# 666DZY666/micronet

Measured on NVIDIA H100. Metric: qat_step_images_per_sec, higher is better.
Workload: dtype f32 (bf16 tensor-core products of exact integer levels / exact bf16 pieces, fp32 accumulate)

## Files before the change

harness/step_profile.py:

```python
import argparse
import json
import os
import re
import subprocess
import sys

sys.path.insert(0, os.path.dirname(os.path.dirname(os.path.abspath(__file__))))

import torch

from harness import train as H

HEADLINE = "nin_gc_wbwtab_w3a2"


def card():
    try:
        return subprocess.run(["nvidia-smi", "--query-gpu=name,power.limit,clocks.max.sm", "--format=csv,noheader"],
                              capture_output=True, text=True, timeout=30).stdout.strip().splitlines()[0]
    except (OSError, subprocess.SubprocessError, IndexError) as e:
        return f"unknown ({type(e).__name__})"


def producer_bytes(rec, terms_dy):
    n, xb, pooled, plane_only, pk_conv = rec["n"], rec["xb"], rec["pool2"], rec["plane_only"], rec["pk_conv"]
    bits = n / 8
    out = {"channel_stats_kernel": n * xb}
    if pooled:
        out["bn_sign_pool_fwd_kernel"] = n * xb + n + n / 4 + bits
        out["bn_sign_pool_bwd_reduce_kernel"] = n * xb + n + n / 4 + bits
        if pk_conv:
            out["bn_sign_pool_bwd_pack_kernel"] = n * xb + n + n / 4 + bits + 2 * n * terms_dy
        else:
            out["bn_sign_pool_bwd_apply_kernel"] = n * xb + n + n / 4 + bits + 4 * n
    else:
        out["bn_sign_packed_fwd_kernel"] = n * xb + 2 * n + bits + (0 if plane_only else 4 * n)
        out["bn_sign_bwd_reduce_kernel"] = n * xb + 4 * n + bits
        if pk_conv:
            out["bn_sign_bwd_pack_kernel"] = n * xb + 4 * n + bits + 2 * n * terms_dy
        else:
            out["bn_sign_bwd_apply_kernel"] = n * xb + 4 * n + bits + 4 * n
    return out


def base_name(kernel):
    head = kernel.split("(")[0]
    head = re.sub(r"<.*$", "", head)
    return head.split("::")[-1].split(" ")[-1]


def main():
    ap = argparse.ArgumentParser()
    ap.add_argument("--out", required=True)
    ap.add_argument("--steps", type=int, default=5)
    ap.add_argument("--warmup", type=int, default=5)
    ap.add_argument("--batch", type=int, default=256)
    args = ap.parse_args()
    if not torch.cuda.is_available():
        raise SystemExit("step_profile: no CUDA device")
    os.makedirs(args.out, exist_ok=True)
    from micronet_b200 import _lib as L
    from micronet_b200.fused import BatchNormBinarize2d
    w = H.WORKLOADS[HEADLINE]
    dev = torch.device("cuda:0")
    model = H.prepare_engine(H.build_float_model(w["model"]), w["scheme"], **w["prepare"], **w.get("engine_extra", {})).to(dev)
    stepper = H.QatStepper(model, lr=0.01, wd=w["wd"], flat=True, graph=False)
    batches = [H.synthetic_batch(args.batch, w["hw"], seed=100 + i, device=dev) for i in range(2)]
    for i in range(args.warmup):
        stepper.step(*batches[i % 2])
    torch.cuda.synchronize()

    calls = []

    def hook(mod, inp):
        x = inp[0]
        calls.append({"n": x.numel(), "xb": 2 if getattr(x, "_mnb_codes", None) is not None else 4,
                      "pool2": bool(mod.pool2), "plane_only": bool(mod.plane_only) and not mod.pool2,
                      "pk_conv": getattr(x, "_mnb_pk_conv", None) is not None})

    handles = [m.register_forward_pre_hook(hook) for m in model.modules() if isinstance(m, BatchNormBinarize2d)]
    acts = [torch.profiler.ProfilerActivity.CPU, torch.profiler.ProfilerActivity.CUDA]
    with torch.profiler.profile(activities=acts) as prof:
        for i in range(args.steps):
            stepper.step(*batches[i % 2])
        torch.cuda.synchronize()
    for h in handles:
        h.remove()

    terms_dy = min(L.PK_TERMS, L.PK_TERMS_BWD)
    want = {}
    for rec in calls:
        for k, b in producer_bytes(rec, terms_dy).items():
            want[k] = want.get(k, 0.0) + b
    kern = {}
    for e in prof.events():
        if e.device_type != torch.autograd.DeviceType.CUDA:
            continue
        d = kern.setdefault(e.name, {"launches": 0, "us": 0.0})
        d["launches"] += 1
        d["us"] += e.device_time
    rows, total_us = [], sum(d["us"] for d in kern.values()) / args.steps
    for name, d in kern.items():
        row = {"kernel": name, "base": base_name(name), "launches_per_step": d["launches"] / args.steps,
               "us_per_step": d["us"] / args.steps}
        rows.append(row)
    by_base = {}
    for r in rows:
        by_base.setdefault(r["base"], []).append(r)
    for base, rs in by_base.items():
        if base not in want:
            continue
        launches = sum(r["launches_per_step"] for r in rs)
        bytes_step = want[base] / args.steps
        us = sum(r["us_per_step"] for r in rs)
        for r in rs:
            r["bytes_per_launch"] = bytes_step / launches
        rs[0]["group_bytes_per_step"] = bytes_step
        rs[0]["group_GBps"] = bytes_step / (us * 1e-6) / 1e9
    rows.sort(key=lambda r: -r["us_per_step"])
    res = {"card": card(), "workload": HEADLINE, "batch": args.batch, "steps": args.steps,
           "device_us_per_step": total_us, "kernels": rows}
    with open(os.path.join(args.out, "step_profile.json"), "w") as f:
        json.dump(res, f, indent=1)
    lines = [f"card: {res['card']}", f"{HEADLINE}, batch {args.batch}, eager step, {args.steps} profiled steps; "
             f"device time per step {total_us / 1e3:.3f} ms (sum of kernel times)", "",
             f"{'us/step':>9} {'share':>6} {'launch':>6} {'MB/launch':>9} {'GB/s':>7}  kernel"]
    for r in rows:
        mb = f"{r['bytes_per_launch'] / 1e6:9.1f}" if "bytes_per_launch" in r else " " * 9
        gbs = f"{r['group_GBps']:7.0f}" if "group_GBps" in r else " " * 7
        lines.append(f"{r['us_per_step']:9.1f} {r['us_per_step'] / total_us:6.1%} {r['launches_per_step']:6.1f} {mb} {gbs}  "
                     f"{r['kernel'][:110]}")
    txt = "\n".join(lines)
    with open(os.path.join(args.out, "step_profile.txt"), "w") as f:
        f.write(txt + "\n")
    print(txt)


if __name__ == "__main__":
    main()
```

include/micronet_b200.h:

```cpp
#ifndef MICRONET_B200_H
#define MICRONET_B200_H

#include <stdint.h>

#ifdef __cplusplus
extern "C" {
#endif

typedef void* mnb_stream_t;

#define MNB_E_ARG (-1)
#define MNB_E_UNSUPPORTED (-2)

int mnb_version(void);
const char* mnb_last_error(void);
int64_t mnb_launch_count(void);

typedef struct {
  int32_t batch, in_c, in_h, in_w;
  int32_t out_c, ker_h, ker_w;
  int32_t stride_h, stride_w, pad_h, pad_w, dil_h, dil_w, groups;
} mnb_conv_shape;

#define MNB_ACT_DOREFA 1
// ... 94 lines not shown
                          void* scratch, const int32_t* run_if_nonzero, mnb_stream_t stream);

int mnb_bn_batch_stats(const float* x, int32_t batch, int32_t channels, int32_t hw, double eps, double momentum,
                       float* running_mean, float* running_var, int64_t* num_batches_tracked, float* mean_invstd,
                       void* scratch, mnb_stream_t stream);
int mnb_bn_sign_fwd(const float* x, int32_t batch, int32_t channels, int32_t hw, const float* mean, const float* invstd,
                    const float* gamma, const float* beta, int32_t out_shuffle_groups, float* y, uint32_t* pass_bits,
                    mnb_stream_t stream);
int mnb_bn_sign_bwd(const float* g, const uint32_t* pass_bits, const float* x, int32_t batch, int32_t channels, int32_t hw,
                    const float* mean, const float* invstd, const float* gamma, int32_t training,
                    int32_t out_shuffle_groups, float* dx, float* dgamma, float* dbeta, float* dx_channel_sum,
                    void* scratch, mnb_stream_t stream);

int mnb_bn_sign_pool_fwd(const float* x, int32_t batch, int32_t channels, int32_t H, int32_t W, const float* mean,
                         const float* invstd, const float* gamma, const float* beta, int32_t out_shuffle_groups, float* y,
                         uint32_t* pass_bits, uint8_t* argmax, mnb_stream_t stream);
int mnb_bn_sign_pool_bwd(const float* g, const uint32_t* pass_bits, const uint8_t* argmax, const float* x, int32_t batch,
                         int32_t channels, int32_t H, int32_t W, const float* mean, const float* invstd, const float* gamma,
                         int32_t training, int32_t out_shuffle_groups, float* dx, float* dgamma, float* dbeta,
                         float* dx_channel_sum, void* scratch, mnb_stream_t stream);

int mnb_maxpool2d_fwd(const float* x, int32_t batch, int32_t channels, int32_t H, int32_t W, int32_t kernel, int32_t stride,
                      int32_t pad, int32_t out_shuffle_groups, float* y, uint8_t* argmax, mnb_stream_t stream);
int mnb_maxpool2d_bwd(const float* g, const uint8_t* argmax, int32_t batch, int32_t channels, int32_t H, int32_t W,
                      int32_t kernel, int32_t stride, int32_t pad, int32_t out_shuffle_groups, float* dx,
                      mnb_stream_t stream);

int mnb_bn_sign_fwd_packed(const float* x, int32_t batch, int32_t channels, int32_t hw, const float* mean,
                           const float* invstd, const float* gamma, const float* beta, int32_t out_shuffle_groups, float* y,
                           uint32_t* pass_bits, void* x_packed, mnb_stream_t stream);

int mnb_fconv2d_fwd_tc(const mnb_conv_shape* s, const float* x, const float* w, const float* bias, float* y,
                       int32_t* err_flag, mnb_stream_t stream);
int64_t mnb_fconv2d_wgrad_tc_scratch_bytes(const mnb_conv_shape* s);
int mnb_fconv2d_wgrad_tc(const mnb_conv_shape* s, const float* dy, const float* x, float* dw, void* scratch,
                         int32_t* err_flag, mnb_stream_t stream);

int64_t mnb_pk_act_bytes(int32_t batch, int32_t channels, int32_t h, int32_t w, int32_t terms);
int mnb_pk_pack_act(const float* x, int32_t batch, int32_t channels, int32_t h, int32_t w, const mnb_act_qparams* qp,
                    int32_t terms, const float* ch_scale, int32_t phase_split, void* out_pk, uint8_t* bits8,
                    mnb_stream_t stream);
int mnb_bn_relu_quant_pack_fwd(const float* x, int32_t batch, int32_t channels, int32_t hw, const float* mean,
                               const float* invstd, const float* gamma, const float* beta, const mnb_act_qparams* qp,
                               int32_t out_shuffle_groups, void* x_packed, uint32_t* pass_bits, mnb_stream_t stream);
int mnb_bn_sign_bwd_pack(const float* g, const uint32_t* pass_bits, const float* x, int32_t batch, int32_t channels, int32_t hw,
                         const float* mean, const float* invstd, const float* gamma, const float* dgamma, const float* dbeta,
                         int32_t out_shuffle_groups, const float* ch_scale, int32_t terms, float* dx, void* dy_packed,
                         mnb_stream_t stream);
int mnb_bn_sign_pool_bwd_pack(const float* g, const uint32_t* pass_bits, const uint8_t* argmax, const float* x, int32_t batch,
                              int32_t channels, int32_t H, int32_t W, const float* mean, const float* invstd,
                              const float* gamma, const float* dgamma, const float* dbeta, int32_t out_shuffle_groups,
                              const float* ch_scale, int32_t terms, void* dy_packed, mnb_stream_t stream);
int mnb_pk_conv_codes(const mnb_conv_shape* s, const void* a_pk, int32_t terms_a, const void* w_img, int32_t terms_w,
                      const float* n_scale, const float* a_scale, float a_scale_const, const float* bias, int32_t level_bound,
                      int16_t* codes, float* dec, int32_t* err_flag, mnb_stream_t stream);
int mnb_codes_decode(const int16_t* codes, const float* dec, int32_t batch, int32_t channels, int32_t hw, float* x,
                     mnb_stream_t stream);
int mnb_bn_batch_stats_codes(const int16_t* codes, const float* dec, int32_t batch, int32_t channels, int32_t hw, double eps,
                             double momentum, float* running_mean, float* running_var, int64_t* num_batches_tracked,
                             float* mean_invstd, void* scratch, mnb_stream_t stream);
int mnb_bn_sign_fwd_packed_codes(const int16_t* codes, const float* dec, int32_t batch, int32_t channels, int32_t hw,
                                 const float* mean, const float* invstd, const float* gamma, const float* beta,
                                 int32_t out_shuffle_groups, float* y, uint32_t* pass_bits, void* x_packed, mnb_stream_t stream);
int mnb_bn_sign_bwd_codes(const float* g, const uint32_t* pass_bits, const int16_t* codes, const float* dec, int32_t batch,
                          int32_t channels, int32_t hw, const float* mean, const float* invstd, const float* gamma,
                          int32_t training, int32_t out_shuffle_groups, float* dx, float* dgamma, float* dbeta,
                          float* dx_channel_sum, void* scratch, mnb_stream_t stream);
int mnb_bn_sign_pool_fwd_codes(const int16_t* codes, const float* dec, int32_t batch, int32_t channels, int32_t H, int32_t W,
                               const float* mean, const float* invstd, const float* gamma, const float* beta,
                               int32_t out_shuffle_groups, float* y, uint32_t* pass_bits, uint8_t* argmax, mnb_stream_t stream);
int mnb_bn_sign_pool_bwd_codes(const float* g, const uint32_t* pass_bits, const uint8_t* argmax, const int16_t* codes,
                               const float* dec, int32_t batch, int32_t channels, int32_t H, int32_t W, const float* mean,
                               const float* invstd, const float* gamma, int32_t training, int32_t out_shuffle_groups, float* dx,
                               float* dgamma, float* dbeta, float* dx_channel_sum, void* scratch, mnb_stream_t stream);
int mnb_bn_sign_bwd_pack_codes(const float* g, const uint32_t* pass_bits, const int16_t* codes, const float* dec, int32_t batch,
                               int32_t channels, int32_t hw, const float* mean, const float* invstd, const float* gamma,
                               const float* dgamma, const float* dbeta, int32_t out_shuffle_groups, const float* ch_scale,
                               int32_t terms, float* dx, void* dy_packed, mnb_stream_t stream);
int mnb_bn_sign_pool_bwd_pack_codes(const float* g, const uint32_t* pass_bits, const uint8_t* argmax, const int16_t* codes,
                                    const float* dec, int32_t batch, int32_t channels, int32_t H, int32_t W, const float* mean,
                                    const float* invstd, const float* gamma, const float* dgamma, const float* dbeta,
                                    int32_t out_shuffle_groups, const float* ch_scale, int32_t terms, void* dy_packed,
                                    mnb_stream_t stream);
int mnb_pk_pack_act_relu(const float* x, int32_t batch, int32_t channels, int32_t h, int32_t w, const mnb_act_qparams* qp,
                         int32_t terms, const float* ch_scale, int32_t phase_split, int32_t relu, void* out_pk,
                         uint8_t* bits8, mnb_stream_t stream);
int mnb_pk_conv_plan(const mnb_conv_shape* s, int32_t mode, int32_t terms_a, int32_t terms_w, int32_t* out16);
int mnb_pk_conv_plan_ex(const mnb_conv_shape* s, int32_t mode, int32_t terms_a, int32_t terms_w, int32_t* out, int32_t n);
int mnb_pk_wgrad_plan(const mnb_conv_shape* s, int32_t terms_dy, int32_t terms_x, int32_t* out, int32_t n);
int64_t mnb_pk_wimage_bytes(const mnb_conv_shape* s, int32_t mode, int32_t terms_a, int32_t terms_w);
int mnb_pk_pack_weight(const mnb_conv_shape* s, int32_t mode, int32_t terms_a, int32_t terms_w, const int16_t* w_int,
                       const float* w_f32, const float* kzero, void* w_img, mnb_stream_t stream);
int mnb_pk_conv(const mnb_conv_shape* s, int32_t mode, const void* a_pk, int32_t terms_a, const void* w_img, int32_t terms_w,
                const float* n_scale, const float* a_scale, float a_scale_const, const float* bias, const uint8_t* bits8,
                float gain, float* out, int32_t* err_flag, mnb_stream_t stream);
typedef struct mnb_pk_post {
  const mnb_act_qparams* q;
  int32_t relu;
  int32_t phase_split;
  void* out_pk;
  const float* bn_mean;
  const float* bn_invstd;
  const float* bn_gamma;
  const float* bn_beta;
  int32_t shuffle_groups;
} mnb_pk_post;
int mnb_pk_conv_post(const mnb_conv_shape* s, const void* a_pk, int32_t terms_a, const void* w_img, int32_t terms_w,
                     const float* n_scale, const float* a_scale, float a_scale_const, const float* bias, float* out,
                     const mnb_pk_post* post, int32_t* err_flag, mnb_stream_t stream);
int mnb_quant_add_pack_fwd(const float* a, const float* b, int32_t batch, int32_t channels, int32_t h, int32_t w,
                           const mnb_act_qparams* qp, int32_t relu, float* out, const mnb_pk_post* post, mnb_stream_t stream);
int64_t mnb_pk_i8_act_bytes(int32_t batch, int32_t channels, int32_t h, int32_t w);
int mnb_pk_i8_pack_act(const float* x, int32_t batch, int32_t channels, int32_t h, int32_t w, const mnb_act_qparams* qp,
                       int32_t phase_split, int32_t relu, void* out_pk, mnb_stream_t stream);
int mnb_pk_i8_conv_plan(const mnb_conv_shape* s, int32_t* out, int32_t n);
int64_t mnb_pk_i8_wimage_bytes(const mnb_conv_shape* s);
int mnb_pk_i8_pack_weight(const mnb_conv_shape* s, const int16_t* w_int, void* w_img, mnb_stream_t stream);
int mnb_pk_i8_conv(const mnb_conv_shape* s, const void* a_pk, const void* w_img, const float* n_scale, const float* a_scale,
                   float a_scale_const, const float* bias, float* out, const mnb_pk_post* post, int32_t* err_flag,
                   mnb_stream_t stream);
int mnb_quant_add_pack_i8_fwd(const float* a, const float* b, int32_t batch, int32_t channels, int32_t h, int32_t w,
                              const mnb_act_qparams* qp, int32_t relu, float* out, const mnb_pk_post* post, mnb_stream_t stream);
int mnb_bn_relu_quant_pack_i8_fwd(const float* x, int32_t batch, int32_t channels, int32_t hw, const float* mean,
                                  const float* invstd, const float* gamma, const float* beta, const mnb_act_qparams* qp,
                                  int32_t out_shuffle_groups, void* x_packed, mnb_stream_t stream);
int mnb_pk_plane_maxpool(const void* in_pk, int32_t batch, int32_t channels, int32_t h, int32_t w, int32_t k, int32_t s, int32_t p,
                         int32_t int8, void* out_pk, mnb_stream_t stream);
int64_t mnb_pk_wgrad_scratch_bytes(const mnb_conv_shape* s, int32_t terms_dy, int32_t terms_x);
int mnb_pk_wgrad(const mnb_conv_shape* s, const void* dy_pk, int32_t terms_dy, const void* x_pk, int32_t terms_x,
                 const float* a_scale, const float* kdiv, float* dw, void* scratch, int32_t* err_flag, mnb_stream_t stream);
int mnb_pk_wgrad_taps_plan(const mnb_conv_shape* s, int32_t terms_dy, int32_t terms_x, int32_t* out, int32_t n);
int mnb_pk_wgrad_taps(const mnb_conv_shape* s, const void* dy_pk, int32_t terms_dy, const void* x_pk, int32_t terms_x,
                      const float* a_scale, const float* kdiv, float* dw, void* scratch, int32_t* err_flag, mnb_stream_t stream);

int mnb_xnor_supported(const mnb_conv_shape* s);
int64_t mnb_xnor_act_bytes(int32_t batch, int32_t channels, int32_t h, int32_t w, int32_t groups);
int mnb_xnor_pack_act(const float* x, int32_t batch, int32_t channels, int32_t h, int32_t w, int32_t groups, void* out_bits,
                      mnb_stream_t stream);
int64_t mnb_xnor_wimage_bytes(const mnb_conv_shape* s);
int mnb_xnor_pack_weight(const mnb_conv_shape* s, const int16_t* w_int, void* w_img, mnb_stream_t stream);
int mnb_xnor_conv_fwd(const mnb_conv_shape* s, const void* a_bits, const void* w_img, const float* alpha, const float* bias,
                      float* y, mnb_stream_t stream);
#define MNB_XNOR_BITS 0
#define MNB_XNOR_PM1_BF16 1
typedef struct mnb_xnor_post {
  int32_t format;
  int32_t out_groups;
  int32_t shuffle_groups;
  int32_t pool2;
  const float* bn_mean;
  const float* bn_invstd;
  const float* bn_gamma;
  const float* bn_beta;
} mnb_xnor_post;
int64_t mnb_xnor_post_bytes(const mnb_conv_shape* s, const mnb_xnor_post* post);
int mnb_xnor_conv_post(const mnb_conv_shape* s, const void* a_bits, const void* w_img, const float* alpha, const float* bias,
                       const mnb_xnor_post* post, void* out, mnb_stream_t stream);
int mnb_xnor_pack_act_post(const float* x, int32_t batch, int32_t channels, int32_t h, int32_t w, const mnb_xnor_post* post,
                           void* out_bits, mnb_stream_t stream);

int mnb_adam_step(float* params, const float* grads, float* exp_avg, float* exp_avg_sq, int64_t n, float lr,
                  float beta1, float beta2, float eps, float weight_decay, int32_t step, mnb_stream_t stream);

void mnb_set_tc_profile_buffer(void* dev_int64x16);

int mnb_selftest_umma(const float* A, const float* B, float* D, int32_t N, int32_t K, int32_t int8,
// ... 12 lines not shown
```

micronet_b200/_lib.py:

```python
from __future__ import annotations

import ctypes as C
import os

import torch

_HERE = os.path.dirname(os.path.abspath(__file__))
LIB_PATH = os.path.join(_HERE, "lib", "libmicronet_b200.so")

ACT_DOREFA, ACT_IAO, ACT_SIGN = 1, 2, 3


class ConvShape(C.Structure):
    _fields_ = [(n, C.c_int32) for n in (
        "batch", "in_c", "in_h", "in_w", "out_c", "ker_h", "ker_w", "stride_h", "stride_w",
        "pad_h", "pad_w", "dil_h", "dil_w", "groups")]


class ActQParams(C.Structure):
    _fields_ = [("mode", C.c_int32), ("bits", C.c_int32), ("qmin", C.c_int32), ("qmax", C.c_int32),
                ("q_type", C.c_int32), ("scale", C.c_void_p), ("zero_point", C.c_void_p),
                ("obs_min", C.c_void_p), ("obs_max", C.c_void_p)]


# ... 6 lines not shown
XNOR_BITS, XNOR_PM1_BF16 = 0, 1


class XnorPost(C.Structure):
    _fields_ = [("format", C.c_int32), ("out_groups", C.c_int32), ("shuffle_groups", C.c_int32), ("pool2", C.c_int32),
                ("bn_mean", C.c_void_p), ("bn_invstd", C.c_void_p), ("bn_gamma", C.c_void_p), ("bn_beta", C.c_void_p)]


class ConvOperands(C.Structure):
    _fields_ = [("a_codes", C.c_void_p), ("a_f32", C.c_void_p), ("a_offset", C.c_int32),
                ("a_offset_zp", C.c_void_p), ("a_scale", C.c_void_p), ("w_int", C.c_void_p),
                ("w_scale", C.c_void_p), ("w_f32", C.c_void_p), ("bias", C.c_void_p)]


_P, _I, _L, _D = C.c_void_p, C.c_int32, C.c_int64, C.c_double
_SHAPE, _ACTQ, _OPS = C.POINTER(ConvShape), C.POINTER(ActQParams), C.POINTER(ConvOperands)

PROTOTYPES = {
    "mnb_version": (C.c_int, []),
    "mnb_last_error": (C.c_char_p, []),
    "mnb_launch_count": (_L, []),
    "mnb_act_quant_fwd": (C.c_int, [_P, _L, _ACTQ, _P, _P, _P, _P]),
    "mnb_act_quant_bwd": (C.c_int, [_P, _P, _L, _ACTQ, _P, _P]),
    "mnb_bn_fold_fwd": (C.c_int, [_P, _I, _I, _P, _P, _P, _P, _P, _D, _P, _P, _P]),
    "mnb_bn_fold_bwd": (C.c_int, [_P, _P, _P, _I, _I, _P, _P, _P, _P, _D, _P, _P, _P]),
    "mnb_bn_fold_running": (C.c_int, [_P, _P, _P, _P, _I, _D, _I, _P]),
    "mnb_quant_add_fwd": (C.c_int, [_P, _P, _L, _ACTQ, _P, _P, _P, _I, _P]),
    "mnb_quant_add_bwd": (C.c_int, [_P, _P, _P, _L, _ACTQ, _P, _P, _P]),
    "mnb_observe_scratch_bytes": (_L, [_L, _I]),
    "mnb_iao_observe": (C.c_int, [_P, _L, _I, _I, _I, _D, _D, _P, _P, _I, _I, _I, _I, _P, _P, _P, _P]),
    "mnb_iao_update_qparams": (C.c_int, [_P, _P, _I, _I, _I, _I, _P, _P, _P]),
    "mnb_dorefa_weight_fwd": (C.c_int, [_P, _L, _I, _I, _P, _P, _P, _P, _P, _P]),
    "mnb_dorefa_weight_bwd": (C.c_int, [_P, _P, _L, _I, _P, _P, _P]),
    "mnb_wb_weight_fwd": (C.c_int, [_P, _I, _I, _I, _I, _P, _P, _P, _P, _P]),
    "mnb_wb_weight_bwd": (C.c_int, [_P, _P, _P, _I, _I, _I, _I, _P, _P]),
    "mnb_iao_weight_fwd": (C.c_int, [_P, _L, _I, _I, _P, _P, _P, _P, _I, _I, _I, _P, _P, _P, _P, _P]),
    "mnb_iao_weight_bwd": (C.c_int, [_P, _P, _P, _L, _I, _I, _P, _P]),
    "mnb_conv2d_fwd": (C.c_int, [_SHAPE, _OPS, _P, _P]),
    "mnb_conv2d_dgrad": (C.c_int, [_SHAPE, _P, _P, _P, _ACTQ, _P, _P]),
    "mnb_wgrad_scratch_bytes": (_L, [_SHAPE]),
    "mnb_conv2d_wgrad": (C.c_int, [_SHAPE, _P, _OPS, _P, _P, _P]),
    "mnb_channel_stats": (C.c_int, [_P, _I, _I, _I, _I, _P, _P, _P]),
    "mnb_channel_stats_bwd": (C.c_int, [_P, _P, _P, _P, _I, _I, _I, _P, _P]),
    "mnb_fq_conv2d_fwd_tc": (C.c_int, [_SHAPE, _P, _ACTQ, _P, _P, _P, _P, _P, _P, _P, _P, _P]),
    "mnb_conv2d_dgrad_tc": (C.c_int, [_SHAPE, _P, _P, _P, _P, _ACTQ, _P, _P, _P, _P]),
    "mnb_wgrad_tc_scratch_bytes": (_L, [_SHAPE]),
    "mnb_conv2d_wgrad_tc": (C.c_int, [_SHAPE, _P, _P, _ACTQ, _P, _P, _P, _P, _P]),
    "mnb_conv2d_wgrad_cond": (C.c_int, [_SHAPE, _P, _OPS, _P, _P, _P, _P]),
    "mnb_bn_batch_stats": (C.c_int, [_P, _I, _I, _I, _D, _D, _P, _P, _P, _P, _P, _P]),
    "mnb_bn_sign_fwd": (C.c_int, [_P, _I, _I, _I, _P, _P, _P, _P, _I, _P, _P, _P]),
    "mnb_bn_sign_bwd": (C.c_int, [_P, _P, _P, _I, _I, _I, _P, _P, _P, _I, _I, _P, _P, _P, _P, _P, _P]),
    "mnb_bn_sign_pool_fwd": (C.c_int, [_P, _I, _I, _I, _I, _P, _P, _P, _P, _I, _P, _P, _P, _P]),
    "mnb_bn_sign_pool_bwd": (C.c_int, [_P, _P, _P, _P, _I, _I, _I, _I, _P, _P, _P, _I, _I, _P, _P, _P, _P, _P, _P]),
    "mnb_bn_sign_fwd_packed": (C.c_int, [_P, _I, _I, _I, _P, _P, _P, _P, _I, _P, _P, _P, _P]),
    "mnb_fconv2d_fwd_tc": (C.c_int, [_SHAPE, _P, _P, _P, _P, _P, _P]),
    "mnb_fconv2d_wgrad_tc_scratch_bytes": (_L, [_SHAPE]),
    "mnb_fconv2d_wgrad_tc": (C.c_int, [_SHAPE, _P, _P, _P, _P, _P, _P]),
    "mnb_maxpool2d_fwd": (C.c_int, [_P, _I, _I, _I, _I, _I, _I, _I, _I, _P, _P, _P]),
    "mnb_maxpool2d_bwd": (C.c_int, [_P, _P, _I, _I, _I, _I, _I, _I, _I, _I, _P, _P]),
    "mnb_adam_step": (C.c_int, [_P, _P, _P, _P, _L, C.c_float, C.c_float, C.c_float, C.c_float, C.c_float, _I, _P]),
    "mnb_pk_act_bytes": (_L, [_I, _I, _I, _I, _I]),
    "mnb_pk_pack_act": (C.c_int, [_P, _I, _I, _I, _I, _ACTQ, _I, _P, _I, _P, _P, _P]),
    "mnb_bn_relu_quant_pack_fwd": (C.c_int, [_P, _I, _I, _I, _P, _P, _P, _P, _ACTQ, _I, _P, _P, _P]),
    "mnb_pk_pack_act_relu": (C.c_int, [_P, _I, _I, _I, _I, _ACTQ, _I, _P, _I, _I, _P, _P, _P]),
    "mnb_pk_conv_plan": (C.c_int, [_SHAPE, _I, _I, _I, _P]),
    "mnb_pk_conv_plan_ex": (C.c_int, [_SHAPE, _I, _I, _I, _P, _I]),
    "mnb_pk_wgrad_plan": (C.c_int, [_SHAPE, _I, _I, _P, _I]),
    "mnb_pk_wimage_bytes": (_L, [_SHAPE, _I, _I, _I]),
    "mnb_pk_pack_weight": (C.c_int, [_SHAPE, _I, _I, _I, _P, _P, _P, _P, _P]),
    "mnb_pk_conv": (C.c_int, [_SHAPE, _I, _P, _I, _P, _I, _P, _P, C.c_float, _P, _P, C.c_float, _P, _P, _P]),
    "mnb_bn_sign_bwd_pack": (C.c_int, [_P, _P, _P, _I, _I, _I, _P, _P, _P, _P, _P, _I, _P, _I, _P, _P, _P]),
    "mnb_bn_sign_pool_bwd_pack": (C.c_int, [_P, _P, _P, _P, _I, _I, _I, _I, _P, _P, _P, _P, _P, _I, _P, _I, _P, _P]),
    "mnb_pk_conv_post": (C.c_int, [_SHAPE, _P, _I, _P, _I, _P, _P, C.c_float, _P, _P, C.POINTER(PkPost), _P, _P]),
    "mnb_pk_conv_codes": (C.c_int, [_SHAPE, _P, _I, _P, _I, _P, _P, C.c_float, _P, _I, _P, _P, _P, _P]),
    "mnb_codes_decode": (C.c_int, [_P, _P, _I, _I, _I, _P, _P]),
    "mnb_bn_batch_stats_codes": (C.c_int, [_P, _P, _I, _I, _I, _D, _D, _P, _P, _P, _P, _P, _P]),
    "mnb_bn_sign_fwd_packed_codes": (C.c_int, [_P, _P, _I, _I, _I, _P, _P, _P, _P, _I, _P, _P, _P, _P]),
    "mnb_bn_sign_bwd_codes": (C.c_int, [_P, _P, _P, _P, _I, _I, _I, _P, _P, _P, _I, _I, _P, _P, _P, _P, _P, _P]),
    "mnb_bn_sign_pool_fwd_codes": (C.c_int, [_P, _P, _I, _I, _I, _I, _P, _P, _P, _P, _I, _P, _P, _P, _P]),
    "mnb_bn_sign_pool_bwd_codes": (C.c_int, [_P, _P, _P, _P, _P, _I, _I, _I, _I, _P, _P, _P, _I, _I, _P, _P, _P, _P, _P, _P]),
    "mnb_bn_sign_bwd_pack_codes": (C.c_int, [_P, _P, _P, _P, _I, _I, _I, _P, _P, _P, _P, _P, _I, _P, _I, _P, _P, _P]),
    "mnb_bn_sign_pool_bwd_pack_codes": (C.c_int, [_P, _P, _P, _P, _P, _I, _I, _I, _I, _P, _P, _P, _P, _P, _I, _P, _I, _P,
                                                  _P]),
    "mnb_quant_add_pack_fwd": (C.c_int, [_P, _P, _I, _I, _I, _I, _ACTQ, _I, _P, C.POINTER(PkPost), _P]),
    "mnb_pk_i8_act_bytes": (_L, [_I, _I, _I, _I]),
    "mnb_pk_i8_pack_act": (C.c_int, [_P, _I, _I, _I, _I, _ACTQ, _I, _I, _P, _P]),
    "mnb_pk_i8_conv_plan": (C.c_int, [_SHAPE, _P, _I]),
    "mnb_pk_i8_wimage_bytes": (_L, [_SHAPE]),
    "mnb_pk_i8_pack_weight": (C.c_int, [_SHAPE, _P, _P, _P]),
    "mnb_pk_i8_conv": (C.c_int, [_SHAPE, _P, _P, _P, _P, C.c_float, _P, _P, C.POINTER(PkPost), _P, _P]),
    "mnb_quant_add_pack_i8_fwd": (C.c_int, [_P, _P, _I, _I, _I, _I, _ACTQ, _I, _P, C.POINTER(PkPost), _P]),
    "mnb_bn_relu_quant_pack_i8_fwd": (C.c_int, [_P, _I, _I, _I, _P, _P, _P, _P, _ACTQ, _I, _P, _P]),
    "mnb_pk_plane_maxpool": (C.c_int, [_P, _I, _I, _I, _I, _I, _I, _I, _I, _P, _P]),
    "mnb_pk_wgrad_scratch_bytes": (_L, [_SHAPE, _I, _I]),
    "mnb_pk_wgrad": (C.c_int, [_SHAPE, _P, _I, _P, _I, _P, _P, _P, _P, _P, _P]),
    "mnb_pk_wgrad_taps_plan": (C.c_int, [_SHAPE, _I, _I, _P, _I]),
    "mnb_pk_wgrad_taps": (C.c_int, [_SHAPE, _P, _I, _P, _I, _P, _P, _P, _P, _P, _P]),
    "mnb_xnor_supported": (C.c_int, [_SHAPE]),
    "mnb_xnor_act_bytes": (_L, [_I, _I, _I, _I, _I]),
    "mnb_xnor_pack_act": (C.c_int, [_P, _I, _I, _I, _I, _I, _P, _P]),
    "mnb_xnor_wimage_bytes": (_L, [_SHAPE]),
    "mnb_xnor_pack_weight": (C.c_int, [_SHAPE, _P, _P, _P]),
    "mnb_xnor_conv_fwd": (C.c_int, [_SHAPE, _P, _P, _P, _P, _P, _P]),
    "mnb_xnor_post_bytes": (_L, [_SHAPE, C.POINTER(XnorPost)]),
    "mnb_xnor_conv_post": (C.c_int, [_SHAPE, _P, _P, _P, _P, C.POINTER(XnorPost), _P, _P]),
    "mnb_xnor_pack_act_post": (C.c_int, [_P, _I, _I, _I, _I, C.POINTER(XnorPost), _P, _P]),
    "mnb_set_tc_profile_buffer": (None, [_P]),
    "mnb_selftest_mma_rate": (C.c_int, [_I, _I, _I, _I, _I, _P, _P, _P]),
    "mnb_selftest_umma": (C.c_int, [_P, _P, _P, _I, _I, _I, _P, _P]),
    "mnb_selftest_tma3d": (C.c_int, [_P, C.POINTER(C.c_int64), C.POINTER(C.c_int32), C.POINTER(C.c_int32), _P, _P, _P]),
}

_lib = None


def load():
    global _lib
    if _lib is not None:
        return _lib
    if not os.path.exists(LIB_PATH):
        raise RuntimeError(
            f"micronet_b200: {LIB_PATH} is missing - build it with `python -m micronet_b200.build` "
            "(there is no CPU / PyTorch fallback for the fake-quant hot path)")
    lib = C.CDLL(LIB_PATH)
    for name, (res, args) in PROTOTYPES.items():
        fn = getattr(lib, name)
        fn.restype, fn.argtypes = res, args
    _lib = lib
    return lib


def check(rc: int, what: str):
    if rc != 0:
        msg = load().mnb_last_error().decode(errors="replace")
        kind = ValueError if rc < 0 else RuntimeError
        raise kind(f"micronet_b200.{what} failed (code {rc}): {msg}")


def ptr(t):
    return None if t is None else t.data_ptr()


def stream():
    return torch.cuda.current_stream().cuda_stream


def require_cuda(*tensors):
    for t in tensors:
        if t is not None and not t.is_cuda:
            raise RuntimeError(
                "micronet_b200: the fake-quant engine runs on CUDA (sm_90a) tensors only; "
                "got a CPU tensor - there is deliberately no CPU fallback")


def require_f32(*tensors):
    for t in tensors:
        if t is not None and t.dtype != torch.float32:
            raise TypeError(f"micronet_b200: fp32 tensors only (the reference's QAT modules are fp32), got {t.dtype}")


def launch_count() -> int:
    return int(load().mnb_launch_count())


_errflags = {}

# ... 42 lines not shown
```

micronet_b200/csrc/mnb_common.cuh:

```cuda
#pragma once
#include <cuda_runtime.h>
#include <float.h>
#include <stdint.h>

#include "../../include/micronet_b200.h"

int mnb_fail(int code, const char* fmt, ...);
void mnb_count_launches(int n);

#define MNB_REQUIRE(cond, ...)                            \
  do {                                                    \
    if (!(cond)) return mnb_fail(MNB_E_ARG, __VA_ARGS__); \
  } while (0)

#define MNB_LAUNCHED(nlaunch)                                                        \
  do {                                                                               \
    mnb_count_launches(nlaunch);                                                     \
    cudaError_t e__ = cudaGetLastError();                                            \
    if (e__ != cudaSuccess) return mnb_fail((int)e__, "%s:%d launch failed: %s", __FILE__, __LINE__, \
                                            cudaGetErrorString(e__));                \
  } while (0)

static inline int mnb_ceil_div(int64_t a, int64_t b) { return (int)((a + b - 1) / b); }
constexpr int MNB_NUM_SMS = 132;


__device__ __forceinline__ float mnb_round_half_away(float v) {
  float r = floorf(__fadd_rn(fabsf(v), 0.5f));
  return v > 0.f ? r : (v < 0.f ? -r : 0.f);
}
__device__ __forceinline__ float mnb_sign0(float v) { return v > 0.f ? 1.f : (v < 0.f ? -1.f : 0.f); }

__device__ __forceinline__ uint32_t mnb_f2ord(float f) {
  uint32_t u = __float_as_uint(f);
  return (u & 0x80000000u) ? ~u : (u | 0x80000000u);
}
__device__ __forceinline__ float mnb_ord2f(uint32_t u) {
  return __uint_as_float((u & 0x80000000u) ? (u & 0x7fffffffu) : ~u);
}

template <typename T, typename Op>
__device__ __forceinline__ T mnb_warp_reduce(T v, Op op) {
#pragma unroll
  for (int o = 16; o > 0; o >>= 1) v = op(v, __shfl_xor_sync(0xffffffffu, v, o));
  return v;
}
template <typename T, typename Op>
__device__ __forceinline__ T mnb_block_reduce(T v, Op op, T identity, T* smem) {
  const int lane = threadIdx.x & 31, wid = threadIdx.x >> 5;
  v = mnb_warp_reduce(v, op);
  __syncthreads();
  if (lane == 0) smem[wid] = v;
  __syncthreads();
  const int nw = (blockDim.x + 31) >> 5;
  T r = (lane < nw) ? smem[lane] : identity;
  r = mnb_warp_reduce(r, op);
  return r;
}
struct MnbMin { template <typename T> __device__ T operator()(T a, T b) const { return a < b ? a : b; } };
struct MnbMax { template <typename T> __device__ T operator()(T a, T b) const { return a > b ? a : b; } };
struct MnbSum { template <typename T> __device__ T operator()(T a, T b) const { return a + b; } };

__device__ __forceinline__ float bn_bwd_centre(float g, float db, float xhat, float dg) {
  return fmaf(-xhat, dg, __fsub_rn(g, db));
}

struct XDec { float s, b; };
template <typename XT> struct XVec;
template <> struct XVec<float> { typedef float t1; typedef float2 t2; typedef float4 t4; };
template <> struct XVec<int16_t> { typedef short t1; typedef short2 t2; typedef short4 t4; };

template <typename XT>
__device__ __forceinline__ XDec x_dec(const float* dec, int channels, int c) {
  if constexpr (sizeof(XT) == 4) return XDec{1.f, 0.f};
  else return XDec{__ldg(dec + c), __ldg(dec + channels + c)};
}
template <typename XT>
__device__ __forceinline__ float x_val(XT q, XDec d) {
  if constexpr (sizeof(XT) == 4) return q;
  else return fmaf((float)q, d.s, d.b);
}
template <int VEC, typename XT>
__device__ __forceinline__ void x_load(const XT* p, XDec d, float (&v)[VEC]) {
  if constexpr (VEC == 1) {
    v[0] = x_val<XT>(__ldg(reinterpret_cast<const typename XVec<XT>::t1*>(p)), d);
  } else if constexpr (VEC == 2) {
    const typename XVec<XT>::t2 t = __ldg(reinterpret_cast<const typename XVec<XT>::t2*>(p));
    v[0] = x_val<XT>(t.x, d); v[1] = x_val<XT>(t.y, d);
  } else {
    static_assert(VEC == 4, "x_load: 1, 2 or 4 elements");
    const typename XVec<XT>::t4 t = __ldg(reinterpret_cast<const typename XVec<XT>::t4*>(p));
    v[0] = x_val<XT>(t.x, d); v[1] = x_val<XT>(t.y, d); v[2] = x_val<XT>(t.z, d); v[3] = x_val<XT>(t.w, d);
  }
}
template <typename XT>
__device__ __forceinline__ float4 x_load4(const XT* p, XDec d) {
  float v[4];
  x_load<4>(p, d, v);
  return make_float4(v[0], v[1], v[2], v[3]);
}

struct MnbActQ {
  int mode, qmin, qmax;
  float s, zp, lo, hi;
  float rinv;
};

__device__ __forceinline__ MnbActQ mnb_load_actq(const mnb_act_qparams& p) {
  MnbActQ q;
  q.mode = p.mode; q.qmin = p.qmin; q.qmax = p.qmax;
  q.s = 1.f; q.zp = 0.f; q.lo = 0.f; q.hi = 0.f; q.rinv = 1.f;
  if (p.mode == MNB_ACT_DOREFA) {
    q.s = (float)(1.0 / (double)((1 << p.bits) - 1));
  } else if (p.mode == MNB_ACT_IAO) {
    q.s = __ldg(p.scale);
    q.zp = __ldg(p.zero_point);
    float a = __fsub_rn(__fdiv_rn(__ldg(p.obs_min), q.s), q.zp);
    float b = __fsub_rn(__fdiv_rn(__ldg(p.obs_max), q.s), q.zp);
    if (p.q_type == 0) { q.hi = fmaxf(fabsf(a), fabsf(b)); q.lo = -q.hi; }
    else { q.lo = a; q.hi = b; }
  }
  q.rinv = __fdiv_rn(1.f, q.s);
  return q;
}

__device__ __forceinline__ int mnb_act_quantize_one(const MnbActQ& q, float x, bool& pass, float& xq) {
  if (q.mode == MNB_ACT_DOREFA) {
    float t = __fmul_rn(x, 0.1f);
    pass = (t >= 0.f) && (t <= 1.f);
    float c = fminf(fmaxf(t, 0.f), 1.f);
    float r = floorf(__fadd_rn(__fdiv_rn(c, q.s), 0.5f));
    xq = __fmul_rn(r, q.s);
    return (int)r;
  } else if (q.mode == MNB_ACT_IAO) {
    float v = __fsub_rn(__fdiv_rn(x, q.s), q.zp);
    float r = mnb_round_half_away(v);
    float c = fminf(fmaxf(r, (float)q.qmin), (float)q.qmax);
    pass = !(v > q.hi) && !(v < q.lo) && (r >= (float)q.qmin) && (r <= (float)q.qmax);
    xq = __fmul_rn(__fadd_rn(c, q.zp), q.s);
    return (int)c - q.qmin;
  } else {
    bool pos = !(x < 0.f);
    pass = !(x >= 1.0f) && !(x <= -1.0f);
    xq = pos ? 1.f : -1.f;
    return pos ? 2 : 0;
  }
}

__device__ __forceinline__ int mnb_act_code_certified(const MnbActQ& q, float x, bool& pass) {
  if (q.mode == MNB_ACT_DOREFA) {
    const float t = __fmul_rn(x, 0.1f);
    pass = (t >= 0.f) && (t <= 1.f);
    const float c = fminf(fmaxf(t, 0.f), 1.f);
    const float pa = c * q.rinv;
    const float f = pa + 0.5f;
    float r = floorf(f);
    const float d = f - r, delta = 4e-7f * (pa + 1.f);
    if (d < delta || d > 1.f - delta) r = floorf(__fadd_rn(__fdiv_rn(c, q.s), 0.5f));
    return (int)r;
  } else if (q.mode == MNB_ACT_IAO) {
    const float xa = x * q.rinv;
    float v = xa - q.zp;
    const float av = fabsf(v);
// ... 115 lines not shown
```

micronet_b200/csrc/mnb_conv_packed.cu:

```cuda
#include <cuda_bf16.h>

#include <algorithm>

#include "mnb_common.cuh"

namespace tcpacked {

template <int VEC> struct VecT;
template <> struct VecT<1> { typedef float type; };
template <> struct VecT<2> { typedef float2 type; };
template <> struct VecT<4> { typedef float4 type; };

template <int VEC>
__device__ __forceinline__ void store_vec(float* p, const float (&v)[VEC]) {
  typedef typename VecT<VEC>::type T;
  T t;
  float* f = reinterpret_cast<float*>(&t);
#pragma unroll
  for (int i = 0; i < VEC; ++i) f[i] = v[i];
  *reinterpret_cast<T*>(p) = t;
}

template <int VEC, typename XT>
__global__ void __launch_bounds__(256) bn_sign_packed_fwd_kernel(const XT* __restrict__ x, const float* __restrict__ dec,
// ... 11 lines not shown
    const int64_t t = w / chunks;
    const int oc8 = (int)(t % c8n), b = (int)(t / c8n);
    const int pos = (ch * 32 + lane) * VEC;
    float v[8][VEC];
    int cc[8];
#pragma unroll
    for (int j = 0; j < 8; ++j) {
      const int oc = oc8 * 8 + j;
      cc[j] = sg > 1 ? (oc % sg) * cpg + oc / sg : oc;
      x_load<VEC>(x + ((int64_t)b * channels + cc[j]) * hw + pos, x_dec<XT>(dec, channels, cc[j]), v[j]);
    }
    uint32_t h[VEC][8];
#pragma unroll
    for (int j = 0; j < 8; ++j) {
      const int c = cc[j];
      const float mu = __ldg(mean + c), k = __ldg(gamma + c) * __ldg(invstd + c), be = __ldg(beta + c);
      uint32_t pass = 0;
      float yv[VEC];
#pragma unroll
      for (int i = 0; i < VEC; ++i) {
        const float bn = fmaf(v[j][i] - mu, k, be);
        const bool neg = bn < 0.f;
        yv[i] = neg ? -1.f : 1.f;
        h[i][j] = neg ? 0xBF80u : 0x3F80u;
        pass |= (fabsf(bn) < 1.f ? 1u : 0u) << i;
      }
      if (y) store_vec<VEC>(y + ((int64_t)b * channels + oc8 * 8 + j) * hw + pos, yv);
      uint32_t word = pass << (VEC * (lane % LPW));
#pragma unroll
      for (int o = 1; o < LPW; o <<= 1) word |= __shfl_xor_sync(0xffffffffu, word, o);
      if (lane % LPW == 0) bits[(((int64_t)b * channels + c) * hw + pos) >> 5] = word;
    }
    uint4* dst = xp + ((int64_t)b * c8n + oc8) * hw + pos;
#pragma unroll
    for (int i = 0; i < VEC; ++i)
      dst[i] = make_uint4(h[i][0] | (h[i][1] << 16), h[i][2] | (h[i][3] << 16), h[i][4] | (h[i][5] << 16), h[i][6] | (h[i][7] << 16));
  }
}

}

template <typename XT>
static int bn_sign_fwd_packed(const XT* x, const float* dec, int32_t batch, int32_t channels, int32_t hw, const float* mean,
                              const float* invstd, const float* gamma, const float* beta, int32_t out_shuffle_groups, float* y,
                              uint32_t* pass_bits, void* x_packed, mnb_stream_t stream) {
  MNB_REQUIRE(x && mean && invstd && gamma && beta && pass_bits && x_packed, "NULL bn_sign_fwd_packed pointer");
  MNB_REQUIRE(batch > 0 && channels > 0 && hw > 0, "bad bn_sign_fwd_packed shape");
  MNB_REQUIRE(out_shuffle_groups >= 1 && channels % out_shuffle_groups == 0, "shuffle groups %d do not divide %d channels",
              out_shuffle_groups, channels);
  if (channels % 8 || hw % 32 || (reinterpret_cast<uintptr_t>(x_packed) & 15))
    return mnb_fail(MNB_E_UNSUPPORTED, "packed producer needs channels %% 8 == 0, H*W %% 32 == 0, 16-byte aligned output");
  constexpr uintptr_t xa4 = 4 * sizeof(XT) - 1, xa2 = 2 * sizeof(XT) - 1;
  const int vec = (hw % 128 == 0 && (reinterpret_cast<uintptr_t>(x) & xa4) == 0 && (!y || (reinterpret_cast<uintptr_t>(y) & 15) == 0)) ? 4
                  : ((hw % 64 == 0 && (reinterpret_cast<uintptr_t>(x) & xa2) == 0 && (!y || (reinterpret_cast<uintptr_t>(y) & 7) == 0)) ? 2 : 1);
  const int64_t warps = (int64_t)batch * (channels / 8) * (hw / (32 * vec));
  int blocks = (int)std::min<int64_t>(mnb_ceil_div(warps, 8), MNB_NUM_SMS * 8);
  uint4* xp = reinterpret_cast<uint4*>(x_packed);
  cudaStream_t st = (cudaStream_t)stream;
  if (vec == 4)
    tcpacked::bn_sign_packed_fwd_kernel<4, XT><<<blocks, 256, 0, st>>>(x, dec, batch, channels, hw, out_shuffle_groups, mean, invstd, gamma, beta, y, pass_bits, xp);
  else if (vec == 2)
    tcpacked::bn_sign_packed_fwd_kernel<2, XT><<<blocks, 256, 0, st>>>(x, dec, batch, channels, hw, out_shuffle_groups, mean, invstd, gamma, beta, y, pass_bits, xp);
  else
    tcpacked::bn_sign_packed_fwd_kernel<1, XT><<<blocks, 256, 0, st>>>(x, dec, batch, channels, hw, out_shuffle_groups, mean, invstd, gamma, beta, y, pass_bits, xp);
  MNB_LAUNCHED(1);
  return 0;
}

extern "C" int mnb_bn_sign_fwd_packed(const float* x, int32_t batch, int32_t channels, int32_t hw, const float* mean,
                                      const float* invstd, const float* gamma, const float* beta, int32_t out_shuffle_groups,
                                      float* y, uint32_t* pass_bits, void* x_packed, mnb_stream_t stream) {
  return bn_sign_fwd_packed<float>(x, nullptr, batch, channels, hw, mean, invstd, gamma, beta, out_shuffle_groups, y, pass_bits,
                                   x_packed, stream);
}

extern "C" int mnb_bn_sign_fwd_packed_codes(const int16_t* codes, const float* dec, int32_t batch, int32_t channels, int32_t hw,
                                            const float* mean, const float* invstd, const float* gamma, const float* beta,
                                            int32_t out_shuffle_groups, float* y, uint32_t* pass_bits, void* x_packed,
                                            mnb_stream_t stream) {
  MNB_REQUIRE(dec, "NULL decode pair");
  return bn_sign_fwd_packed<int16_t>(codes, dec, batch, channels, hw, mean, invstd, gamma, beta, out_shuffle_groups, y, pass_bits,
                                     x_packed, stream);
}
```

micronet_b200/csrc/mnb_fused.cu:

```cuda
#include <algorithm>

#include "mnb_common.cuh"

static inline cudaStream_t S(mnb_stream_t s) { return (cudaStream_t)s; }
constexpr int FUSED_SPLITS = 32;

__device__ __forceinline__ uint32_t shuffled_channel(uint32_t c, uint32_t sg, uint32_t cpg) {
  return sg > 1 ? (c % cpg) * sg + c / cpg : c;
}

__global__ void __launch_bounds__(256) bn_sign_fwd_v4_kernel(const float4* __restrict__ x, uint32_t n4, uint32_t channels,
                                                             uint32_t hw4, uint32_t sg, const float* __restrict__ mean,
                                                             const float* __restrict__ invstd, const float* __restrict__ gamma,
                                                             const float* __restrict__ beta, float4* __restrict__ y,
                                                             uint32_t* __restrict__ bits) {
  const uint32_t lane = threadIdx.x & 31;
  const uint32_t stride = gridDim.x * blockDim.x;
  const uint32_t n4_up = (n4 + 31u) & ~31u;
  const uint32_t cpg = channels / sg;
  for (uint32_t i = blockIdx.x * blockDim.x + threadIdx.x; i < n4_up; i += stride) {
    uint32_t nib = 0;
    if (i < n4) {
      const uint32_t plane = i / hw4, off = i - plane * hw4;
      const uint32_t b = plane / channels, c = plane - b * channels;
// ... 196 lines not shown

template <typename XT = float>
static bool planes_vectorizable(int64_t n, int hw, const void* a, const void* b, const void* c, const XT* x = nullptr) {
  return (hw & 3) == 0 && n < (1ll << 31) &&
         (((uintptr_t)a | (uintptr_t)b | (uintptr_t)c) & 15) == 0 && ((uintptr_t)x & (4 * sizeof(XT) - 1)) == 0;
}
static int plane_splits(int batch, int64_t per, int channels) {
  const int64_t want = (2 * 8 * MNB_NUM_SMS + channels - 1) / channels;
  return (int)std::max<int64_t>(1, std::min<int64_t>(std::min<int64_t>(std::min<int64_t>(FUSED_SPLITS, batch), per / 2048), want));
}

extern "C" int mnb_bn_sign_fwd(const float* x, int32_t batch, int32_t channels, int32_t hw, const float* mean,
                               const float* invstd, const float* gamma, const float* beta, int32_t out_shuffle_groups,
                               float* y, uint32_t* pass_bits, mnb_stream_t stream) {
  MNB_REQUIRE(x && mean && invstd && gamma && beta && y && pass_bits, "NULL bn_sign_fwd pointer");
  MNB_REQUIRE(batch > 0 && channels > 0 && hw > 0, "bad bn_sign_fwd shape");
  MNB_REQUIRE(out_shuffle_groups >= 1 && channels % out_shuffle_groups == 0, "shuffle groups %d do not divide %d channels",
              out_shuffle_groups, channels);
  const int64_t n = (int64_t)batch * channels * hw;
  int blocks = (int)std::min<int64_t>(mnb_ceil_div(n, 256 * 4), MNB_NUM_SMS * 8);
  if (planes_vectorizable(n, hw, x, y, nullptr))
    bn_sign_fwd_v4_kernel<<<blocks, 256, 0, S(stream)>>>(reinterpret_cast<const float4*>(x), (uint32_t)(n / 4),
                                                         (uint32_t)channels, (uint32_t)(hw / 4), (uint32_t)out_shuffle_groups,
                                                         mean, invstd, gamma, beta, reinterpret_cast<float4*>(y), pass_bits);
  else
    bn_sign_fwd_kernel<<<blocks, 256, 0, S(stream)>>>(x, n, channels, hw, out_shuffle_groups, mean, invstd, gamma, beta, y,
                                                      pass_bits);
  MNB_LAUNCHED(1);
  return 0;
}

template <typename XT>
static int bn_sign_bwd(const float* g, const uint32_t* pass_bits, const XT* x, const float* dec, int32_t batch, int32_t channels,
                       int32_t hw, const float* mean, const float* invstd, const float* gamma, int32_t training,
                       int32_t out_shuffle_groups, float* dx, float* dgamma, float* dbeta, float* dx_channel_sum, void* scratch,
                       mnb_stream_t stream) {
  MNB_REQUIRE(g && pass_bits && x && mean && invstd && gamma && dx && dgamma && dbeta && scratch, "NULL bn_sign_bwd pointer");
  MNB_REQUIRE(batch > 0 && channels > 0 && channels <= 8192 && hw > 0, "bad bn_sign_bwd shape");
  MNB_REQUIRE(out_shuffle_groups >= 1 && channels % out_shuffle_groups == 0, "shuffle groups %d do not divide %d channels",
              out_shuffle_groups, channels);
  const int64_t n = (int64_t)batch * channels * hw;
  const int64_t per = (int64_t)batch * hw;
  const int splits = plane_splits(batch, per, channels);
  uint32_t* counters = reinterpret_cast<uint32_t*>(reinterpret_cast<char*>(scratch) + 16384);
  double* partial = reinterpret_cast<double*>(reinterpret_cast<char*>(scratch) + 49152);
  const dim3 grid(channels, splits);
  const float inv_count = 1.f / (float)per;
  if (planes_vectorizable(n, hw, g, dx, nullptr, x)) {
    bn_sign_bwd_reduce_kernel<true, XT><<<grid, 256, 0, S(stream)>>>(g, pass_bits, x, dec, batch, channels, hw, out_shuffle_groups,
                                                                     mean, invstd, dgamma, dbeta, counters, partial);
    if (training == 2) { MNB_LAUNCHED(1); return 0; }
    bn_sign_bwd_apply_kernel<true, XT><<<grid, 256, 0, S(stream)>>>(g, pass_bits, x, dec, batch, channels, hw, out_shuffle_groups,
                                                                    inv_count, mean, invstd, gamma, dgamma, dbeta, training, dx,
                                                                    dx_channel_sum, counters, partial);
  } else {
    bn_sign_bwd_reduce_kernel<false, XT><<<grid, 256, 0, S(stream)>>>(g, pass_bits, x, dec, batch, channels, hw, out_shuffle_groups,
                                                                      mean, invstd, dgamma, dbeta, counters, partial);
    if (training == 2) { MNB_LAUNCHED(1); return 0; }
    bn_sign_bwd_apply_kernel<false, XT><<<grid, 256, 0, S(stream)>>>(g, pass_bits, x, dec, batch, channels, hw, out_shuffle_groups,
                                                                     inv_count, mean, invstd, gamma, dgamma, dbeta, training, dx,
                                                                     dx_channel_sum, counters, partial);
  }
  MNB_LAUNCHED(2);
  return 0;
}

extern "C" int mnb_bn_sign_bwd(const float* g, const uint32_t* pass_bits, const float* x, int32_t batch, int32_t channels,
                               int32_t hw, const float* mean, const float* invstd, const float* gamma, int32_t training,
                               int32_t out_shuffle_groups, float* dx, float* dgamma, float* dbeta, float* dx_channel_sum,
                               void* scratch, mnb_stream_t stream) {
  return bn_sign_bwd<float>(g, pass_bits, x, nullptr, batch, channels, hw, mean, invstd, gamma, training, out_shuffle_groups, dx,
                            dgamma, dbeta, dx_channel_sum, scratch, stream);
}

extern "C" int mnb_bn_sign_bwd_codes(const float* g, const uint32_t* pass_bits, const int16_t* codes, const float* dec,
                                     int32_t batch, int32_t channels, int32_t hw, const float* mean, const float* invstd,
                                     const float* gamma, int32_t training, int32_t out_shuffle_groups, float* dx, float* dgamma,
                                     float* dbeta, float* dx_channel_sum, void* scratch, mnb_stream_t stream) {
  MNB_REQUIRE(dec, "NULL decode pair");
  return bn_sign_bwd<int16_t>(g, pass_bits, codes, dec, batch, channels, hw, mean, invstd, gamma, training, out_shuffle_groups, dx,
                              dgamma, dbeta, dx_channel_sum, scratch, stream);
}

struct PoolGeom { uint32_t channels, H, W4, OH, OW2, sg; };

__device__ __forceinline__ uint32_t first_max_of_signs(bool p0, bool p1, bool p2, bool p3) {
  return p0 ? 0u : (p1 ? 1u : (p2 ? 2u : (p3 ? 3u : 0u)));
}

template <typename XT>
__global__ void __launch_bounds__(256) bn_sign_pool_fwd_kernel(const XT* __restrict__ x, const float* __restrict__ dec,
                                                               uint32_t n_pairs, PoolGeom gm,
                                                               const float* __restrict__ mean, const float* __restrict__ invstd,
                                                               const float* __restrict__ gamma, const float* __restrict__ beta,
                                                               float2* __restrict__ y, uchar2* __restrict__ arg,
                                                               uint8_t* __restrict__ bits8) {
  const uint32_t stride = gridDim.x * blockDim.x;
  const uint32_t n_up = (n_pairs + 31u) & ~31u;
  const uint32_t cpg = gm.channels / gm.sg;
  for (uint32_t o = blockIdx.x * blockDim.x + threadIdx.x; o < n_up; o += stride) {
    uint32_t nib = 0, i0 = 0;
    const bool live = o < n_pairs;
    if (live) {
      const uint32_t j = o % gm.OW2, t = o / gm.OW2;
      const uint32_t oh = t % gm.OH, plane = t / gm.OH;
      const uint32_t b = plane / gm.channels, c = plane - b * gm.channels;
      i0 = (plane * gm.H + 2 * oh) * gm.W4 + j;
      const float mu = __ldg(mean + c), sc = __ldg(gamma + c) * __ldg(invstd + c), be = __ldg(beta + c);
      const XDec d = x_dec<XT>(dec, (int)gm.channels, (int)c);
      const float4 r0 = x_load4(x + 4 * i0, d), r1 = x_load4(x + 4 * (i0 + gm.W4), d);
      const float v[8] = {fmaf(r0.x - mu, sc, be), fmaf(r0.y - mu, sc, be), fmaf(r0.z - mu, sc, be), fmaf(r0.w - mu, sc, be),
                          fmaf(r1.x - mu, sc, be), fmaf(r1.y - mu, sc, be), fmaf(r1.z - mu, sc, be), fmaf(r1.w - mu, sc, be)};
      bool pos[8];
#pragma unroll
      for (int e = 0; e < 8; ++e) { pos[e] = !(v[e] < 0.f); nib |= (uint32_t)(fabsf(v[e]) < 1.f) << e; }
      const uint32_t a0 = first_max_of_signs(pos[0], pos[1], pos[4], pos[5]);
      const uint32_t a1 = first_max_of_signs(pos[2], pos[3], pos[6], pos[7]);
      const float m0 = (pos[0] | pos[1] | pos[4] | pos[5]) ? 1.f : -1.f, m1 = (pos[2] | pos[3] | pos[6] | pos[7]) ? 1.f : -1.f;
      const uint32_t oplane = b * gm.channels + shuffled_channel(c, gm.sg, cpg);
      y[(oplane * gm.OH + oh) * gm.OW2 + j] = make_float2(m0, m1);
      arg[o] = make_uchar2((unsigned char)a0, (unsigned char)a1);
    }
    const uint32_t other = __shfl_xor_sync(0xffffffffu, nib, 1);
    if (live && (threadIdx.x & 1) == 0) {
      bits8[i0 >> 1] = (uint8_t)((nib & 15u) | ((other & 15u) << 4));
      bits8[(i0 + gm.W4) >> 1] = (uint8_t)((nib >> 4) | (other & 0xf0u));
    }
  }
}

template <typename XT>
__global__ void __launch_bounds__(256) bn_sign_pool_bwd_reduce_kernel(const float2* __restrict__ g, const uchar2* __restrict__ arg,
                                                                      const uint8_t* __restrict__ bits8, const XT* __restrict__ x,
                                                                      const float* __restrict__ dec, int batch, PoolGeom gm, const float* __restrict__ mean,
                                                                      const float* __restrict__ invstd, float* __restrict__ dgamma,
                                                                      float* __restrict__ dbeta, uint32_t* counters, double* partial) {
  __shared__ double red[32];
  __shared__ bool last;
  const uint32_t c = blockIdx.x, sp = blockIdx.y, nsp = gridDim.y;
  const uint32_t oc = shuffled_channel(c, gm.sg, gm.channels / gm.sg);
  const float mu = __ldg(mean + c), is = __ldg(invstd + c);
  const XDec d = x_dec<XT>(dec, (int)gm.channels, (int)c);
  const uint32_t b_lo = (uint32_t)((int64_t)batch * sp / nsp), b_hi = (uint32_t)((int64_t)batch * (sp + 1) / nsp);
  const uint32_t per_img = gm.OH * gm.OW2, total = (b_hi - b_lo) * per_img;
  float f1[2] = {0.f, 0.f}, f2[2] = {0.f, 0.f};
  for (uint32_t t0 = threadIdx.x; t0 < total; t0 += 2 * blockDim.x) {
#pragma unroll
    for (int u = 0; u < 2; ++u) {
      const uint32_t t = t0 + u * blockDim.x;
      if (t < total) {
        const uint32_t b = b_lo + t / per_img, rem = t % per_img;
        const uint32_t oh = rem / gm.OW2, j = rem - oh * gm.OW2;
        const uint32_t plane = b * gm.channels + c;
        const float2 gv = __ldg(g + ((b * gm.channels + oc) * gm.OH + oh) * gm.OW2 + j);
        const uchar2 a = arg[(plane * gm.OH + oh) * gm.OW2 + j];
        const uint32_t i0 = (plane * gm.H + 2 * oh) * gm.W4 + j;
#pragma unroll
        for (int w = 0; w < 2; ++w) {
          const uint32_t aw = w ? a.y : a.x;
          const uint32_t i4 = i0 + (aw >> 1) * gm.W4, col = 2u * w + (aw & 1u);
          const bool pass = (bits8[i4 >> 1] >> (4u * (i4 & 1u) + col)) & 1u;
          const float gmv = pass ? (w ? gv.y : gv.x) : 0.f;
          f1[u] += gmv;
          f2[u] += gmv * ((x_val<XT>(__ldg(x + 4u * i4 + col), d) - mu) * is);
        }
      }
// ... 44 lines not shown
    const uchar2 a = arg[(plane * gm.OH + oh) * gm.OW2 + j];
    const uint32_t i0 = (plane * gm.H + 2 * oh) * gm.W4 + j, i1 = i0 + gm.W4;
    const uint32_t n0 = (bits8[i0 >> 1] >> (4u * (i0 & 1u))) & 15u, n1 = (bits8[i1 >> 1] >> (4u * (i1 & 1u))) & 15u;
    float v[8] = {0.f, 0.f, 0.f, 0.f, 0.f, 0.f, 0.f, 0.f};
    {
      const uint32_t e0 = (a.x >> 1) * 4u + (a.x & 1u), e1 = (a.y >> 1) * 4u + 2u + (a.y & 1u);
      const uint32_t nib = n0 | (n1 << 4);
#pragma unroll
      for (int e = 0; e < 8; ++e) {
        if ((uint32_t)e == e0 && ((nib >> e) & 1u)) v[e] = gv.x;
        if ((uint32_t)e == e1 && ((nib >> e) & 1u)) v[e] = gv.y;
      }
    }
    if (training) {
      const float4 r0 = x_load4(x + 4 * i0, d), r1 = x_load4(x + 4 * i1, d);
      const float xs[8] = {r0.x, r0.y, r0.z, r0.w, r1.x, r1.y, r1.z, r1.w};
#pragma unroll
      for (int e = 0; e < 8; ++e) v[e] = bn_bwd_centre(v[e], db, (xs[e] - mu) * is, dg);
    }
    const float4 o0 = make_float4(k * v[0], k * v[1], k * v[2], k * v[3]), o1 = make_float4(k * v[4], k * v[5], k * v[6], k * v[7]);
    dx[i0] = o0;
    dx[i1] = o1;
    f += ((o0.x + o0.y) + (o0.z + o0.w)) + ((o1.x + o1.y) + (o1.z + o1.w));
  }
  if (!dx_sum) return;
  double s = mnb_block_reduce((double)f, MnbSum(), 0.0, red);
  if (threadIdx.x == 0) {
    partial[((int64_t)c * nsp + sp) * 2] = s;
    __threadfence();
    last = (atomicAdd(counters + c, 1u) == nsp - 1);
  }
  __syncthreads();
  if (!last || threadIdx.x != 0) return;
  __threadfence();
  s = 0.0;
  for (uint32_t j = 0; j < nsp; ++j) s += partial[((int64_t)c * nsp + j) * 2];
  dx_sum[c] = (float)s;
  counters[c] = 0;
}

template <typename XT>
static int pool_geom(int batch, int channels, int H, int W, int sg, const XT* x, const void* a, const void* b, PoolGeom& gm) {
  MNB_REQUIRE(batch > 0 && channels > 0 && channels <= 8192 && H > 0 && W > 0, "bad bn_sign_pool shape");
  MNB_REQUIRE(sg >= 1 && channels % sg == 0, "shuffle groups %d do not divide %d channels", sg, channels);
  if ((H & 1) || (W & 7) || (int64_t)batch * channels * H * W >= (1ll << 31) ||
      (((uintptr_t)a | (uintptr_t)b) & 15) || ((uintptr_t)x & (4 * sizeof(XT) - 1)))
    return mnb_fail(MNB_E_UNSUPPORTED, "bn_sign_pool needs even H, W %% 8 == 0, < 2^31 elements, 16-byte aligned tensors");
  gm = PoolGeom{(uint32_t)channels, (uint32_t)H, (uint32_t)(W / 4), (uint32_t)(H / 2), (uint32_t)(W / 4), (uint32_t)sg};
  return 0;
}

template <typename XT>
static int bn_sign_pool_fwd(const XT* x, const float* dec, int32_t batch, int32_t channels, int32_t H, int32_t W, const float* mean,
                            const float* invstd, const float* gamma, const float* beta, int32_t out_shuffle_groups, float* y,
                            uint32_t* pass_bits, uint8_t* argmax, mnb_stream_t stream) {
  MNB_REQUIRE(x && mean && invstd && gamma && beta && y && pass_bits && argmax, "NULL bn_sign_pool_fwd pointer");
  PoolGeom gm;
  if (int e = pool_geom(batch, channels, H, W, out_shuffle_groups, x, y, nullptr, gm)) return e;
  const uint32_t n_pairs = (uint32_t)((int64_t)batch * channels * gm.OH * gm.OW2);
  int blocks = (int)std::min<int64_t>(mnb_ceil_div(n_pairs, 256), MNB_NUM_SMS * 16);
  bn_sign_pool_fwd_kernel<XT><<<blocks, 256, 0, S(stream)>>>(x, dec, n_pairs, gm, mean, invstd, gamma, beta,
                                                             reinterpret_cast<float2*>(y), reinterpret_cast<uchar2*>(argmax),
                                                             reinterpret_cast<uint8_t*>(pass_bits));
  MNB_LAUNCHED(1);
  return 0;
}

extern "C" int mnb_bn_sign_pool_fwd(const float* x, int32_t batch, int32_t channels, int32_t H, int32_t W, const float* mean,
                                    const float* invstd, const float* gamma, const float* beta, int32_t out_shuffle_groups,
                                    float* y, uint32_t* pass_bits, uint8_t* argmax, mnb_stream_t stream) {
  return bn_sign_pool_fwd<float>(x, nullptr, batch, channels, H, W, mean, invstd, gamma, beta, out_shuffle_groups, y, pass_bits,
                                 argmax, stream);
}

extern "C" int mnb_bn_sign_pool_fwd_codes(const int16_t* codes, const float* dec, int32_t batch, int32_t channels, int32_t H,
                                          int32_t W, const float* mean, const float* invstd, const float* gamma, const float* beta,
                                          int32_t out_shuffle_groups, float* y, uint32_t* pass_bits, uint8_t* argmax,
                                          mnb_stream_t stream) {
  MNB_REQUIRE(dec, "NULL decode pair");
  return bn_sign_pool_fwd<int16_t>(codes, dec, batch, channels, H, W, mean, invstd, gamma, beta, out_shuffle_groups, y, pass_bits,
                                   argmax, stream);
}

template <typename XT>
static int bn_sign_pool_bwd(const float* g, const uint32_t* pass_bits, const uint8_t* argmax, const XT* x, const float* dec,
                            int32_t batch, int32_t channels, int32_t H, int32_t W, const float* mean, const float* invstd,
                            const float* gamma, int32_t training, int32_t out_shuffle_groups, float* dx, float* dgamma,
                            float* dbeta, float* dx_channel_sum, void* scratch, mnb_stream_t stream) {
  MNB_REQUIRE(g && pass_bits && argmax && x && mean && invstd && gamma && dx && dgamma && dbeta && scratch,
              "NULL bn_sign_pool_bwd pointer");
  PoolGeom gm;
  if (int e = pool_geom(batch, channels, H, W, out_shuffle_groups, x, dx, nullptr, gm)) return e;
  MNB_REQUIRE((reinterpret_cast<uintptr_t>(g) & 7) == 0, "pooled gradient must be 8-byte aligned");
  const int64_t per = (int64_t)batch * H * W;
  const int splits = plane_splits(batch, per, channels);
  uint32_t* counters = reinterpret_cast<uint32_t*>(reinterpret_cast<char*>(scratch) + 16384);
  double* partial = reinterpret_cast<double*>(reinterpret_cast<char*>(scratch) + 49152);
  const dim3 grid(channels, splits);
  const uint8_t* bits8 = reinterpret_cast<const uint8_t*>(pass_bits);
  bn_sign_pool_bwd_reduce_kernel<XT><<<grid, 256, 0, S(stream)>>>(reinterpret_cast<const float2*>(g),
                                                                  reinterpret_cast<const uchar2*>(argmax), bits8, x, dec, batch, gm,
                                                                  mean, invstd, dgamma, dbeta, counters, partial);
  if (training == 2) { MNB_LAUNCHED(1); return 0; }
  bn_sign_pool_bwd_apply_kernel<XT><<<grid, 256, 0, S(stream)>>>(reinterpret_cast<const float2*>(g),
                                                                 reinterpret_cast<const uchar2*>(argmax), bits8, x, dec, batch, gm,
                                                                 1.f / (float)per, mean, invstd, gamma, dgamma, dbeta, training,
                                                                 reinterpret_cast<float4*>(dx), dx_channel_sum, counters, partial);
  MNB_LAUNCHED(2);
  return 0;
}

extern "C" int mnb_bn_sign_pool_bwd(const float* g, const uint32_t* pass_bits, const uint8_t* argmax, const float* x, int32_t batch,
                                    int32_t channels, int32_t H, int32_t W, const float* mean, const float* invstd,
                                    const float* gamma, int32_t training, int32_t out_shuffle_groups, float* dx, float* dgamma,
                                    float* dbeta, float* dx_channel_sum, void* scratch, mnb_stream_t stream) {
  return bn_sign_pool_bwd<float>(g, pass_bits, argmax, x, nullptr, batch, channels, H, W, mean, invstd, gamma, training,
                                 out_shuffle_groups, dx, dgamma, dbeta, dx_channel_sum, scratch, stream);
}

extern "C" int mnb_bn_sign_pool_bwd_codes(const float* g, const uint32_t* pass_bits, const uint8_t* argmax, const int16_t* codes,
                                          const float* dec, int32_t batch, int32_t channels, int32_t H, int32_t W,
                                          const float* mean, const float* invstd, const float* gamma, int32_t training,
                                          int32_t out_shuffle_groups, float* dx, float* dgamma, float* dbeta,
                                          float* dx_channel_sum, void* scratch, mnb_stream_t stream) {
  MNB_REQUIRE(dec, "NULL decode pair");
  return bn_sign_pool_bwd<int16_t>(g, pass_bits, argmax, codes, dec, batch, channels, H, W, mean, invstd, gamma, training,
                                   out_shuffle_groups, dx, dgamma, dbeta, dx_channel_sum, scratch, stream);
}

__global__ void __launch_bounds__(256) maxpool_fwd_kernel(const float* __restrict__ x, int64_t n_out, int channels, int H, int W,
                                                          int OH, int OW, int k, int st, int pad, int sg,
                                                          float* __restrict__ y, uint8_t* __restrict__ arg) {
  const uint32_t cpg = (uint32_t)(channels / sg);
  const int64_t stride = (int64_t)gridDim.x * blockDim.x;
  for (int64_t o = (int64_t)blockIdx.x * blockDim.x + threadIdx.x; o < n_out; o += stride) {
    const int ow = (int)(o % OW);
    const int64_t t = o / OW;
    const int oh = (int)(t % OH);
    const int64_t plane = t / OH;
    const int c = (int)(plane % channels);
    const float* src = x + plane * H * W;
    const int h0 = oh * st - pad, w0 = ow * st - pad;
    float best = -INFINITY;
    int bi = -1;
    for (int r = 0; r < k; ++r) {
      const int h = h0 + r;
      if (h < 0 || h >= H) continue;
      for (int s = 0; s < k; ++s) {
        const int w = w0 + s;
        if (w < 0 || w >= W) continue;
        const float v = __ldg(src + h * W + w);
        if (bi < 0 || v > best || isnan(v)) { best = v; bi = r * k + s; }
      }
    }
    const int64_t oplane = plane - c + shuffled_channel((uint32_t)c, (uint32_t)sg, cpg);
    y[(oplane * OH + oh) * OW + ow] = best;
    arg[o] = (uint8_t)bi;
  }
}

__global__ void __launch_bounds__(256) maxpool2x2_fwd_kernel(const float4* __restrict__ x, uint32_t n_pairs, uint32_t channels,
                                                             uint32_t OH, uint32_t OW2, uint32_t W4, uint32_t H, uint32_t sg,
                                                             float2* __restrict__ y, uchar2* __restrict__ arg) {
  const uint32_t cpg = channels / sg;
  const uint32_t stride = gridDim.x * blockDim.x;
  for (uint32_t o = blockIdx.x * blockDim.x + threadIdx.x; o < n_pairs; o += stride) {
    const uint32_t j = o % OW2, t = o / OW2;
    const uint32_t oh = t % OH, plane = t / OH;
    const uint32_t b = plane / channels, c = plane - b * channels;
    const float4 r0 = __ldg(x + (plane * H + 2 * oh) * W4 + j), r1 = __ldg(x + (plane * H + 2 * oh + 1) * W4 + j);
    float m0 = r0.x; uint32_t a0 = 0;
    if (r0.y > m0 || isnan(r0.y)) { m0 = r0.y; a0 = 1; }
    if (r1.x > m0 || isnan(r1.x)) { m0 = r1.x; a0 = 2; }
    if (r1.y > m0 || isnan(r1.y)) { m0 = r1.y; a0 = 3; }
    float m1 = r0.z; uint32_t a1 = 0;
    if (r0.w > m1 || isnan(r0.w)) { m1 = r0.w; a1 = 1; }
    if (r1.z > m1 || isnan(r1.z)) { m1 = r1.z; a1 = 2; }
    if (r1.w > m1 || isnan(r1.w)) { m1 = r1.w; a1 = 3; }
    const uint32_t oplane = b * channels + shuffled_channel(c, sg, cpg);
    y[(oplane * OH + oh) * OW2 + j] = make_float2(m0, m1);
    arg[o] = make_uchar2((unsigned char)a0, (unsigned char)a1);
  }
}

__global__ void __launch_bounds__(256) maxpool_bwd_kernel(const float* __restrict__ g, const uint8_t* __restrict__ arg,
                                                          int64_t n_in, int channels, int H, int W, int OH, int OW, int k, int st,
                                                          int pad, int sg, float* __restrict__ dx) {
  const uint32_t cpg = (uint32_t)(channels / sg);
  const int64_t stride = (int64_t)gridDim.x * blockDim.x;
  for (int64_t i = (int64_t)blockIdx.x * blockDim.x + threadIdx.x; i < n_in; i += stride) {
    const int w = (int)(i % W);
    const int64_t t = i / W;
    const int h = (int)(t % H);
    const int64_t plane = t / H;
    const int c = (int)(plane % channels);
    const int64_t oplane = plane - c + shuffled_channel((uint32_t)c, (uint32_t)sg, cpg);
    const int oh_lo = (h + pad < k) ? 0 : (h + pad - k) / st + 1, oh_hi = min((h + pad) / st + 1, OH);
    const int ow_lo = (w + pad < k) ? 0 : (w + pad - k) / st + 1, ow_hi = min((w + pad) / st + 1, OW);
    float acc = 0.f;
    for (int oh = oh_lo; oh < oh_hi; ++oh)
      for (int ow = ow_lo; ow < ow_hi; ++ow) {
        const int r = h - (oh * st - pad), s = w - (ow * st - pad);
        if ((int)arg[(plane * OH + oh) * OW + ow] == r * k + s) acc += __ldg(g + (oplane * OH + oh) * OW + ow);
      }
    dx[i] = acc;
  }
}

__global__ void __launch_bounds__(256) maxpool2x2_bwd_kernel(const float2* __restrict__ g, const uchar2* __restrict__ arg,
                                                             uint32_t n_pairs, uint32_t channels, uint32_t OH, uint32_t OW2,
                                                             uint32_t W4, uint32_t H, uint32_t sg, float4* __restrict__ dx) {
  const uint32_t cpg = channels / sg;
  const uint32_t stride = gridDim.x * blockDim.x;
  for (uint32_t o = blockIdx.x * blockDim.x + threadIdx.x; o < n_pairs; o += stride) {
    const uint32_t j = o % OW2, t = o / OW2;
    const uint32_t oh = t % OH, plane = t / OH;
    const uint32_t b = plane / channels, c = plane - b * channels;
    const uint32_t oplane = b * channels + shuffled_channel(c, sg, cpg);
    const float2 gv = __ldg(g + (oplane * OH + oh) * OW2 + j);
    const uchar2 a = arg[o];
    dx[(plane * H + 2 * oh) * W4 + j] = make_float4(a.x == 0 ? gv.x : 0.f, a.x == 1 ? gv.x : 0.f, a.y == 0 ? gv.y : 0.f,
                                                    a.y == 1 ? gv.y : 0.f);
    dx[(plane * H + 2 * oh + 1) * W4 + j] = make_float4(a.x == 2 ? gv.x : 0.f, a.x == 3 ? gv.x : 0.f, a.y == 2 ? gv.y : 0.f,
                                                        a.y == 3 ? gv.y : 0.f);
  }
}

static int pool_out(int in, int k, int st, int pad) { return (in + 2 * pad - k) / st + 1; }
static bool pool_is_2x2(int H, int W, int k, int st, int pad, int64_t n_in, const void* a, const void* b) {
  return k == 2 && st == 2 && pad == 0 && (W & 3) == 0 && (H & 1) == 0 && n_in < (1ll << 31) &&
         (((uintptr_t)a | (uintptr_t)b) & 15) == 0;
}

extern "C" int mnb_maxpool2d_fwd(const float* x, int32_t batch, int32_t channels, int32_t H, int32_t W, int32_t kernel,
                                 int32_t stride, int32_t pad, int32_t out_shuffle_groups, float* y, uint8_t* argmax,
                                 mnb_stream_t stream) {
  MNB_REQUIRE(x && y && argmax && batch > 0 && channels > 0 && H > 0 && W > 0, "bad maxpool2d_fwd arguments");
  MNB_REQUIRE(kernel >= 1 && kernel <= 15 && stride >= 1 && pad >= 0 && 2 * pad <= kernel, "maxpool kernel %d stride %d pad %d",
              kernel, stride, pad);
  MNB_REQUIRE(out_shuffle_groups >= 1 && channels % out_shuffle_groups == 0, "shuffle groups %d do not divide %d channels",
              out_shuffle_groups, channels);
  const int OH = pool_out(H, kernel, stride, pad), OW = pool_out(W, kernel, stride, pad);
  MNB_REQUIRE(OH > 0 && OW > 0, "maxpool output is empty");
  const int64_t planes = (int64_t)batch * channels, n_out = planes * OH * OW;
  if (pool_is_2x2(H, W, kernel, stride, pad, planes * H * W, x, y)) {
    const uint32_t n_pairs = (uint32_t)(n_out / 2);
    int blocks = (int)std::min<int64_t>(mnb_ceil_div(n_pairs, 256), MNB_NUM_SMS * 16);
    maxpool2x2_fwd_kernel<<<blocks, 256, 0, S(stream)>>>(reinterpret_cast<const float4*>(x), n_pairs, (uint32_t)channels,
                                                         (uint32_t)OH, (uint32_t)(OW / 2), (uint32_t)(W / 4), (uint32_t)H,
                                                         (uint32_t)out_shuffle_groups, reinterpret_cast<float2*>(y),
                                                         reinterpret_cast<uchar2*>(argmax));
  } else {
    int blocks = (int)std::min<int64_t>(mnb_ceil_div(n_out, 256), MNB_NUM_SMS * 16);
    maxpool_fwd_kernel<<<blocks, 256, 0, S(stream)>>>(x, n_out, channels, H, W, OH, OW, kernel, stride, pad, out_shuffle_groups,
                                                      y, argmax);
  }
  MNB_LAUNCHED(1);
  return 0;
}

extern "C" int mnb_maxpool2d_bwd(const float* g, const uint8_t* argmax, int32_t batch, int32_t channels, int32_t H, int32_t W,
                                 int32_t kernel, int32_t stride, int32_t pad, int32_t out_shuffle_groups, float* dx,
                                 mnb_stream_t stream) {
  MNB_REQUIRE(g && dx && argmax && batch > 0 && channels > 0 && H > 0 && W > 0, "bad maxpool2d_bwd arguments");
  MNB_REQUIRE(kernel >= 1 && kernel <= 15 && stride >= 1 && pad >= 0 && 2 * pad <= kernel, "maxpool kernel %d stride %d pad %d",
              kernel, stride, pad);
  MNB_REQUIRE(out_shuffle_groups >= 1 && channels % out_shuffle_groups == 0, "shuffle groups %d do not divide %d channels",
              out_shuffle_groups, channels);
  const int OH = pool_out(H, kernel, stride, pad), OW = pool_out(W, kernel, stride, pad);
  MNB_REQUIRE(OH > 0 && OW > 0, "maxpool output is empty");
  const int64_t planes = (int64_t)batch * channels, n_in = planes * H * W;
  if (pool_is_2x2(H, W, kernel, stride, pad, n_in, g, dx) && (((uintptr_t)g) & 7) == 0) {
    const uint32_t n_pairs = (uint32_t)(planes * OH * OW / 2);
    int blocks = (int)std::min<int64_t>(mnb_ceil_div(n_pairs, 256), MNB_NUM_SMS * 16);
    maxpool2x2_bwd_kernel<<<blocks, 256, 0, S(stream)>>>(reinterpret_cast<const float2*>(g), reinterpret_cast<const uchar2*>(argmax),
                                                         n_pairs, (uint32_t)channels, (uint32_t)OH, (uint32_t)(OW / 2),
                                                         (uint32_t)(W / 4), (uint32_t)H, (uint32_t)out_shuffle_groups,
                                                         reinterpret_cast<float4*>(dx));
  } else {
    int blocks = (int)std::min<int64_t>(mnb_ceil_div(n_in, 256), MNB_NUM_SMS * 16);
    maxpool_bwd_kernel<<<blocks, 256, 0, S(stream)>>>(g, argmax, n_in, channels, H, W, OH, OW, kernel, stride, pad,
                                                      out_shuffle_groups, dx);
  }
  MNB_LAUNCHED(1);
  return 0;
}

__global__ void __launch_bounds__(256) codes_decode_kernel(const int16_t* __restrict__ codes, const float* __restrict__ dec,
                                                           int64_t n, int channels, int hw, float* __restrict__ x) {
  const int64_t stride = (int64_t)gridDim.x * blockDim.x;
  for (int64_t i = (int64_t)blockIdx.x * blockDim.x + threadIdx.x; i < n; i += stride) {
    const int c = (int)((i / hw) % channels);
    x[i] = x_val<int16_t>(__ldg(codes + i), x_dec<int16_t>(dec, channels, c));
  }
}

extern "C" int mnb_codes_decode(const int16_t* codes, const float* dec, int32_t batch, int32_t channels, int32_t hw, float* x,
                                mnb_stream_t stream) {
  MNB_REQUIRE(codes && dec && x && batch > 0 && channels > 0 && hw > 0, "bad codes_decode arguments");
  const int64_t n = (int64_t)batch * channels * hw;
  const int blocks = (int)std::min<int64_t>(mnb_ceil_div(n, 256), MNB_NUM_SMS * 8);
  codes_decode_kernel<<<blocks, 256, 0, S(stream)>>>(codes, dec, n, channels, hw, x);
  MNB_LAUNCHED(1);
  return 0;
}
```

micronet_b200/csrc/mnb_pk.cu:

```cuda
#include <cuda.h>
#include <cuda_bf16.h>

#include <algorithm>
#include <cstdlib>
#include <cstring>

#include "mnb_common.cuh"
#include "mnb_tc.cuh"

namespace pk {

constexpr int MAXST = 8;
constexpr int MAXTAP = 64, MAXTMPL = 16, MAXY = 4, MAXPAIR = 6, MAXPROG = 512;
constexpr int kSmemBudget = 227 * 1024 - 3072;
constexpr int kNtSizes[] = {16, 32, 48, 64, 96, 128};

struct Tmpl { int kph, tap0, ntap, blk_off, blk_bytes; };

struct Plan {
  int mode;
  int B, G, R, S, stride;
  int HA, WA, C8A, nkph;
  int kg, ng, NOUT;
  int OHr, OWr, OH, OW, omul, ny;
// ... 644 lines not shown
__global__ void __launch_bounds__(256) pack_weight_kernel(const __grid_constant__ PackWParams pp, uint4* __restrict__ out) {
  const Plan& p = pp.pl;
  const int64_t total = p.wimg_bytes / 16;
  const int RS = p.R * p.S;
  for (int64_t v = (int64_t)blockIdx.x * blockDim.x + threadIdx.x; v < total; v += (int64_t)gridDim.x * blockDim.x) {
    int64_t byte = v * 16;
    int y = 0;
    for (int yy = 1; yy < p.ny; ++yy) if (byte >= p.y_off[yy]) y = yy;
    byte -= p.y_off[y];
    if (p.img_bytes[y] == 0) continue;
    const int ntg = (int)(byte / p.img_bytes[y]);
    int rem = (int)(byte - (int64_t)ntg * p.img_bytes[y]);
    if (ntg >= p.n_ntiles * p.G) continue;
    const int nt = ntg / p.G, g = ntg - nt * p.G;
    int t = 0;
    for (int tt = 1; tt < p.ntmpl[y]; ++tt) if (rem >= p.tmpl[y][tt].blk_off) t = tt;
    const Tmpl tp = p.tmpl[y][t];
    rem -= tp.blk_off;
    const int cc = rem / tp.blk_bytes;
    rem -= cc * tp.blk_bytes;
    const int per_tap = (p.CC / CPU) * p.Nt * 16, per_term = tp.ntap * per_tap;
    const int term = rem / per_term;
    rem -= term * per_term;
    const int tapi = rem / per_tap;
    rem -= tapi * per_tap;
    const int c8l = rem / (p.Nt * 16), n = (rem - c8l * (p.Nt * 16)) / 16;
    const int r = p.tap_r[y][tp.tap0 + tapi], s = p.tap_s[y][tp.tap0 + tapi];
    const int nn = nt * p.Nt + n;
    float val[CPU];
#pragma unroll
    for (int e = 0; e < CPU; ++e) {
      const int kk = cc * p.CC + c8l * CPU + e;
      float x = 0.f;
      if (kk < p.kg && nn < p.ng) {
        int64_t src;
        int kout;
        if (p.mode == 0) { kout = g * pp.cout_g + nn; src = ((int64_t)kout * pp.cin_g + kk) * RS + r * p.S + s; }
        else { kout = g * pp.cout_g + kk; src = ((int64_t)kout * pp.cin_g + nn) * RS + r * p.S + s; }
        x = pp.w_int ? (float)__ldg(pp.w_int + src) : __ldg(pp.w_f32 + src);
        if (pp.kzero && __ldg(pp.kzero + kout) == 0.f) x = 0.f;
      }
      val[e] = x;
    }
    if constexpr (CPU == 16) {
      out[v] = pack16_s8(val);
    } else {
      uint32_t pk4[4];
      for (int tm = 0; tm <= term; ++tm) {
#pragma unroll
        for (int j = 0; j < 4; ++j) {
          pk4[j] = pack2(val[2 * j], val[2 * j + 1]);
          val[2 * j] -= __uint_as_float(pk4[j] << 16);
          val[2 * j + 1] -= __uint_as_float(pk4[j] & 0xffff0000u);
        }
      }
      out[v] = make_uint4(pk4[0], pk4[1], pk4[2], pk4[3]);
    }
  }
}

struct ConvParams {
  struct Mma {
    uint32_t n_items, chunks, ksteps, MT, Nt, npairs, st_mask, st_log2, stage16, a_mt16, a_term16, a_k16, b_off16,
        b_tap16, b_k16, a_lbo, b_lbo, seg_len;
    uint32_t ntmpl[MAXY];
    uint16_t tmpl_begin[MAXY][MAXTMPL], tmpl_cnt[MAXY][MAXTMPL];
    alignas(16) uint4 prog4[MAXPROG / 4];
  } m;
  int n_items, n_ntiles, G, MT, TA, chunks, CC8, C8A, kg8, stage_bytes, a_bytes, a_box_bytes, b_off, st_mask, st_log2;
  int Wt, TH, TB, wlo, hlo, col_tiles, row_tiles, n_mtiles;
  int ntmpl[MAXY], tmpl_kph[MAXY][MAXTMPL], tmpl_blk_off[MAXY][MAXTMPL], tmpl_blk_bytes[MAXY][MAXTMPL];
  int img_bytes[MAXY], y_off[MAXY];
  const uint8_t* w_img;
  int B, THH, BW, OHr, OWr, OH, OW, omul, ny, ng, Nt, NOUT, C8O, smem_bytes, off_stg, mode;
  int dbg;
  const float* n_scale;
  const float* a_scale;
  float a_scale_const;
  const float* bias;
  const uint8_t* bits8;
  float gain;
  float* out;
  int16_t* codes;
  float* dec;
  uint4* post_out;
  mnb_act_qparams post_q;
  int post_relu, post_split;
  const float *post_mean, *post_invstd, *post_gamma, *post_beta;
  int post_sg;
  int* err;
};

struct alignas(16) ConvShared {
  uint64_t full[MAXST], empty[MAXST];
  uint32_t abort;
  alignas(16) float epi_scale[256];
  alignas(16) float epi_bias[256];
  uint16_t epi_dst[256];
};

template <int NEPI>
__device__ __forceinline__ void epi_bar_sync() { asm volatile("bar.sync 1, %0;" ::"n"(NEPI) : "memory"); }

struct FastDiv {
  uint32_t d; float inv;
  __device__ __forceinline__ explicit FastDiv(int dd) : d((uint32_t)dd), inv(1.0f / (float)dd) {}
  __device__ __forceinline__ void divmod(uint32_t n, uint32_t& q, uint32_t& r) const {
    q = __float2uint_rz(__uint2float_rz(n) * inv);
    r = n - q * d;
    if ((int32_t)r < 0) { --q; r += d; } else if (r >= d) { ++q; r -= d; }
  }
};

constexpr int kConvThreads = 384;

template <bool SEG, int NT, bool I8 = false, bool XPOST = false>
__global__ void __launch_bounds__(kConvThreads, 1)
pk_conv_kernel(const __grid_constant__ CUtensorMap tmap0, const __grid_constant__ CUtensorMap tmap1,
               const __grid_constant__ CUtensorMap tmap2, const __grid_constant__ ConvParams p) {
  extern __shared__ __align__(1024) uint8_t smem[];
  __shared__ ConvShared sh;
  const int tid = threadIdx.x, warp = tid >> 5, lane = tid & 31;

  if (tid == 0) {
    for (int i = 0; i < MAXST; ++i) { tc::mbar_init(&sh.full[i], 1); tc::mbar_init(&sh.empty[i], 8); }
    sh.abort = 0;
    tc::fence_barrier_init();
    tc::prefetch_tmap(&tmap0);
    if (p.TA > 1) tc::prefetch_tmap(&tmap1);
    if (p.TA > 2) tc::prefetch_tmap(&tmap2);
  }
  for (int i = tid; i < p.smem_bytes / 16; i += kConvThreads) reinterpret_cast<uint4*>(smem)[i] = make_uint4(0, 0, 0, 0);
  tc::fence_proxy_async_smem();
  __syncthreads();

  if (warp == 0) {
    if (lane == 0) {
      const int y = blockIdx.y;
      uint32_t sc = 0;
      const FastDiv d_nt(p.n_ntiles), d_g(p.G), d_ct(p.col_tiles), d_rt(p.row_tiles);
      for (int it = blockIdx.x; it < p.n_items; it += gridDim.x) {
        uint32_t nt, r1, g, mg;
        d_nt.divmod((uint32_t)it, r1, nt);
        d_g.divmod(r1, mg, g);
        const uint8_t* wsrc = p.w_img + (size_t)p.y_off[y] + (size_t)(nt * p.G + g) * (size_t)p.img_bytes[y];
        for (int t = 0; t < p.ntmpl[y]; ++t) {
          const int kph = p.tmpl_kph[y][t];
          const uint32_t blk = (uint32_t)p.tmpl_blk_bytes[y][t];
          const uint8_t* bsrc = wsrc + p.tmpl_blk_off[y][t];
          for (int cc = 0; cc < p.chunks; ++cc, ++sc) {
            const uint32_t slot = sc & (uint32_t)p.st_mask, ph = (sc >> p.st_log2) & 1u;
            if (!tc::mbar_wait(&sh.empty[slot], ph ^ 1u, p.err, 701)) goto done;
            const bool ld_a = !(p.dbg & 8), ld_b = !(p.dbg & 16);
            tc::mbar_arrive_expect_tx(&sh.full[slot], (ld_a ? (uint32_t)(p.MT * p.TA * p.a_box_bytes) : 0u) + (ld_b ? blk : 0u));
            uint8_t* sbase = smem + (size_t)slot * p.stage_bytes;
            const int c8 = kph * p.C8A + g * p.kg8 + cc * p.CC8;
            for (int mt = 0; mt < (ld_a ? p.MT : 0); ++mt) {
              const uint32_t tile = mg * (uint32_t)p.MT + (uint32_t)mt;
              uint32_t ct, r2, rt, bt;
              d_ct.divmod(tile, r2, ct);
              d_rt.divmod(r2, bt, rt);
              const int cw = (int)ct * p.Wt - p.wlo, chh = (int)rt * p.TH - p.hlo, cb = (int)bt * p.TB;
              tc::tma_load_4d(sbase + (size_t)(mt * p.TA) * p.a_bytes, &tmap0, &sh.full[slot], 2 * cw, chh, cb, c8);
              if (p.TA > 1) tc::tma_load_4d(sbase + (size_t)(mt * p.TA + 1) * p.a_bytes, &tmap1, &sh.full[slot], 2 * cw, chh, cb, c8);
              if (p.TA > 2) tc::tma_load_4d(sbase + (size_t)(mt * p.TA + 2) * p.a_bytes, &tmap2, &sh.full[slot], 2 * cw, chh, cb, c8);
            }
// ... 39 lines not shown
          scv = p.n_scale ? __fmul_rn(a_sc, __ldg(p.n_scale + n_base + n)) : a_sc;
          if (p.bias) bs = __ldg(p.bias + n_base + n);
        }
        sh.epi_scale[n] = scv; sh.epi_bias[n] = bs;
        if constexpr (XPOST) {
          if (p.post_sg > 1 && n < n_cnt) {
            const int c = n_base + n, cpg = p.NOUT / p.post_sg;
            sh.epi_dst[n] = (uint16_t)((c % cpg) * p.post_sg + c / cpg);
          }
        }
        if constexpr (!SEG && !I8) {
          if (p.dec && mg == 0 && y == 0 && n < n_cnt) { p.dec[n_base + n] = scv; p.dec[p.NOUT + n_base + n] = bs; }
        }
      }
      float acc[MAXMT][NR];
      float rs[SEG ? MAXMT : 1][SEG ? NR : 1];
#pragma unroll
      for (int mt = 0; mt < MAXMT; ++mt) tc::zero_acc(acc[mt]);
      if (SEG) {
#pragma unroll
        for (int mt = 0; mt < MAXMT; ++mt) tc::zero_acc(rs[mt]);
      }
      uint32_t seg_pos = 0;
      for (uint32_t t = 0; t < p.m.ntmpl[y]; ++t) {
        const uint32_t pb = p.m.tmpl_begin[y][t], pc = p.m.tmpl_cnt[y][t];
        for (uint32_t cc = 0; cc < p.m.chunks; ++cc, ++sc) {
          const uint32_t slot = sc & p.m.st_mask, ph = (sc >> p.m.st_log2) & 1u;
          tc::mbar_wait_soft(&sh.full[slot], ph, p.err, 703, &sh.abort);
          const uint32_t s16 = slot * p.m.stage16;
          tc::wg_fence();
#pragma unroll
          for (int mt = 0; mt < MAXMT; ++mt) tc::fence_acc(acc[mt]);
          if (!(p.dbg & 2)) {
#pragma unroll
            for (int mt = 0; mt < MAXMT; ++mt) {
              if (mt >= (int)p.m.MT) break;
              const uint32_t a_base = a_lo0 + s16 + (uint32_t)mt * p.m.a_mt16, b_base = b_lo0 + s16;
              for (uint32_t e = 0; e < pc; ++e) {
                const uint4 w4 = p.m.prog4[pb + e];
                const uint32_t w[4] = {w4.x, w4.y, w4.z, w4.w};
#pragma unroll
                for (int k = 0; k < 4; ++k) {
                  if (w[k] == 0xffffffffu) continue;
                  if constexpr (I8)
                    tc::Mma<NT>::s8(reinterpret_cast<int32_t(&)[NR]>(acc[mt]), a_hi | (uint64_t)(a_base + (w[k] & 0xffffu)),
                                    b_hi | (uint64_t)(b_base + (w[k] >> 16)), 1);
                  else
                    tc::Mma<NT>::template bf16<0, 0>(acc[mt], a_hi | (uint64_t)(a_base + (w[k] & 0xffffu)),
                                                      b_hi | (uint64_t)(b_base + (w[k] >> 16)), 1);
                }
              }
            }
          }
          tc::wg_commit();
          tc::wg_wait<0>();
#pragma unroll
          for (int mt = 0; mt < MAXMT; ++mt) tc::fence_acc(acc[mt]);
          __syncwarp();
          if (lane == 0) tc::mbar_arrive(&sh.empty[slot]);
          if (SEG && ++seg_pos == p.m.seg_len) {
            seg_pos = 0;
#pragma unroll
            for (int mt = 0; mt < MAXMT; ++mt) {
#pragma unroll
              for (int i = 0; i < NR; ++i) { rs[SEG ? mt : 0][SEG ? i : 0] = __fadd_rn(rs[SEG ? mt : 0][SEG ? i : 0], acc[mt][i]); acc[mt][i] = 0.f; }
            }
          }
        }
      }
      if (SEG) {
#pragma unroll
        for (int mt = 0; mt < MAXMT; ++mt) {
#pragma unroll
          for (int i = 0; i < NR; ++i) rs[SEG ? mt : 0][SEG ? i : 0] = __fadd_rn(rs[SEG ? mt : 0][SEG ? i : 0], acc[mt][i]);
        }
      }
      if constexpr (I8) {
#pragma unroll
        for (int mt = 0; mt < MAXMT; ++mt) {
#pragma unroll
          for (int i = 0; i < NR; ++i) acc[mt][i] = __int2float_rn(__float_as_int(acc[mt][i]));
        }
      }
      int mt_cur = -1;
      bool valid = false;
      int64_t orow = 0;
      const uint8_t* brow = nullptr;
      int64_t prow = 0;
      auto do_slot = [&](const int mt, const int c16, const float (&r)[16]) {
        const int n0 = c16 * 16;
        if (mt != mt_cur) {
          mt_cur = mt;
          const int tile = mg * p.MT + mt;
          uint32_t ct_u, r2_u, rt_u, bt_u;
          e_ct.divmod((uint32_t)tile, r2_u, ct_u);
          e_rt.divmod(r2_u, bt_u, rt_u);
          const int ct = (int)ct_u, rt = (int)rt_u, bt = (int)bt_u;
          const int b = bt * p.TB + tb, i = rt * p.TH + th, j = ct * p.Wt + wc;
          valid = row_ok && tile < p.n_mtiles && b < p.B && i < p.OHr && j < p.OWr;
          const int oh = i * p.omul + ya, ow = j * p.omul + yb;
          orow = ((int64_t)b * p.NOUT + n_base) * plane + (int64_t)oh * p.OW + ow;
          brow = p.bits8 ? p.bits8 + (int64_t)b * p.C8O * plane + (int64_t)oh * p.OW + ow : nullptr;
          if (p.post_out) {
            if (p.post_split)
              prow = (((int64_t)b * 4 * p.C8O + ((oh & 1) * 2 + (ow & 1)) * p.C8O) * (p.OH >> 1) + (oh >> 1)) * (p.OW >> 1) + (ow >> 1);
            else
              prow = ((int64_t)b * p.C8O * p.OH + oh) * p.OW + ow;
          }
        }
        if (!valid || n0 >= n_cnt || (p.dbg & 1)) return;
        if (!SEG && !I8 && p.codes) {
          int16_t* cp = p.codes + orow + (int64_t)n0 * plane;
#pragma unroll
          for (int k = 0; k < 16; ++k, cp += plane)
            if (n0 + k < n_cnt) *cp = (int16_t)__float2int_rn(r[k]);
          return;
        }
        if constexpr (XPOST) {
          float* op0 = p.out + orow + (int64_t)n0 * plane;
          const int64_t oct_stride = p.post_split ? (int64_t)(p.OH >> 1) * (p.OW >> 1) : plane;
          uint32_t pw[4];
#pragma unroll
          for (int qc = 0; qc < 4; ++qc) {
            if (!I8 && qc >= 2 && n0 + 8 >= n_cnt) break;
            float lev[4], yv[4];
            const float4 sc4 = *reinterpret_cast<const float4*>(&sh.epi_scale[n0 + 4 * qc]);
            const float4 bs4 = *reinterpret_cast<const float4*>(&sh.epi_bias[n0 + 4 * qc]);
            const float scv[4] = {sc4.x, sc4.y, sc4.z, sc4.w}, bsv[4] = {bs4.x, bs4.y, bs4.z, bs4.w};
            float mu[4] = {0.f, 0.f, 0.f, 0.f}, gs[4] = {0.f, 0.f, 0.f, 0.f}, be[4] = {0.f, 0.f, 0.f, 0.f};
            if (p.post_mean) {
              const int c0 = n_base + n0 + (n0 + 4 * qc < n_cnt ? 4 * qc : 0);
              const float4 m4 = __ldg(reinterpret_cast<const float4*>(p.post_mean + c0));
              const float4 g4 = __ldg(reinterpret_cast<const float4*>(p.post_gamma + c0));
              const float4 i4 = __ldg(reinterpret_cast<const float4*>(p.post_invstd + c0));
              const float4 b4 = __ldg(reinterpret_cast<const float4*>(p.post_beta + c0));
              mu[0] = m4.x; mu[1] = m4.y; mu[2] = m4.z; mu[3] = m4.w;
              gs[0] = __fmul_rn(g4.x, i4.x); gs[1] = __fmul_rn(g4.y, i4.y); gs[2] = __fmul_rn(g4.z, i4.z); gs[3] = __fmul_rn(g4.w, i4.w);
              be[0] = b4.x; be[1] = b4.y; be[2] = b4.z; be[3] = b4.w;
            }
#pragma unroll
            for (int j = 0; j < 4; ++j) {
              const int k = 4 * qc + j;
              float v = fmaf(r[k], scv[j], bsv[j]);
              if (p.out && n0 + k < n_cnt) op0[(int64_t)k * plane] = v;
              if (p.post_mean) v = fmaf(__fsub_rn(v, mu[j]), gs[j], be[j]);
              yv[j] = p.post_relu ? fmaxf(v, 0.f) : v;
            }
            uint32_t passbits;
            mnb_act_levels<4>(pq, yv, lev, passbits);
#pragma unroll
            for (int j = 0; j < 4; ++j) lev[j] = n0 + 4 * qc + j < n_cnt ? lev[j] + pzp : 0.f;
            if (p.post_sg > 1) {
#pragma unroll
              for (int j = 0; j < 4; ++j) {
                if (n0 + 4 * qc + j >= n_cnt) continue;
                const int oc = sh.epi_dst[n0 + 4 * qc + j];
                if constexpr (I8)
                  reinterpret_cast<int8_t*>(p.post_out)[(prow + (int64_t)(oc >> 4) * oct_stride) * 16 + (oc & 15)] =
                      (int8_t)__float2int_rn(lev[j]);
                else
                  reinterpret_cast<__nv_bfloat16*>(p.post_out)[(prow + (int64_t)(oc >> 3) * oct_stride) * 8 + (oc & 7)] =
                      __float2bfloat16_rn(lev[j]);
              }
            } else if constexpr (I8) {
              pw[qc] = pack4_s8(lev[0], lev[1], lev[2], lev[3]);
              if (qc == 3) p.post_out[prow + (int64_t)((n_base + n0) >> 4) * oct_stride] = make_uint4(pw[0], pw[1], pw[2], pw[3]);
            } else {
              pw[2 * (qc & 1)] = pack2(lev[0], lev[1]);
              pw[2 * (qc & 1) + 1] = pack2(lev[2], lev[3]);
              if (qc & 1)
                p.post_out[prow + (int64_t)(((n_base + n0) >> 3) + (qc >> 1)) * oct_stride] = make_uint4(pw[0], pw[1], pw[2], pw[3]);
            }
          }
          return;
        }
        float sc[16], bs[16];
#pragma unroll
        for (int v = 0; v < 4; ++v) {
          const float4 a = *reinterpret_cast<const float4*>(&sh.epi_scale[n0 + 4 * v]);
          const float4 c = *reinterpret_cast<const float4*>(&sh.epi_bias[n0 + 4 * v]);
          sc[4 * v] = a.x; sc[4 * v + 1] = a.y; sc[4 * v + 2] = a.z; sc[4 * v + 3] = a.w;
          bs[4 * v] = c.x; bs[4 * v + 1] = c.y; bs[4 * v + 2] = c.z; bs[4 * v + 3] = c.w;
        }
        float* op = p.out + orow + (int64_t)n0 * plane;
        if (!SEG && p.post_out) {
          float lev[16], yv[16];
#pragma unroll
          for (int k = 0; k < 16; ++k) {
            const float v = fmaf(r[k], sc[k], bs[k]);
            if (p.out && n0 + k < n_cnt) op[(int64_t)k * plane] = v;
            yv[k] = p.post_relu ? fmaxf(v, 0.f) : v;
          }
          uint32_t passbits;
// ... 555 lines not shown
                               void* out_pk, uint8_t* bits8, mnb_stream_t stream) {
  return mnb_pk_pack_act_relu(x, batch, channels, h, w, qp, terms, ch_scale, phase_split, 0, out_pk, bits8, stream);
}

extern "C" int mnb_pk_pack_act_relu(const float* x, int32_t batch, int32_t channels, int32_t h, int32_t w,
                                    const mnb_act_qparams* qp, int32_t terms, const float* ch_scale, int32_t phase_split,
                                    int32_t relu, void* out_pk, uint8_t* bits8, mnb_stream_t stream) {
  MNB_REQUIRE(x && out_pk, "NULL pk_pack_act pointer");
  MNB_REQUIRE(batch > 0 && channels > 0 && h > 0 && w > 0 && terms >= 1 && terms <= 3, "bad pk_pack_act arguments");
  MNB_REQUIRE((reinterpret_cast<uintptr_t>(out_pk) & 15) == 0, "packed tensor must be 16-byte aligned");
  if (phase_split) MNB_REQUIRE(((h | w) & 1) == 0, "phase split needs even H and W");
  const int C8 = (channels + 7) / 8;
  const int64_t plane_vecs = (int64_t)batch * C8 * h * w;
  MNB_REQUIRE((int64_t)batch * C8 <= 65535 * 8 && (int64_t)h * w < (1ll << 31), "pk_pack_act: too many (image, octet) planes");
  dim3 blocks, threads;
  if (!unit_grid(batch, C8, h * w, blocks, threads))
    return mnb_fail(MNB_E_UNSUPPORTED, "pk_pack_act: %d (image, octet) planes exceed the grid", batch * C8);
  cudaStream_t st = (cudaStream_t)stream;
  if (qp) {
    MNB_REQUIRE(qp->mode == MNB_ACT_DOREFA || qp->mode == MNB_ACT_IAO || qp->mode == MNB_ACT_SIGN, "unknown activation quantizer");
    if (qp->mode == MNB_ACT_DOREFA) MNB_REQUIRE(qp->bits >= 2 && qp->bits <= 8, "DoReFa a_bits must be in [2,8]");
    const int a_off = qp->mode == MNB_ACT_IAO ? qp->qmin : (qp->mode == MNB_ACT_SIGN ? -1 : 0);
    pk::pack_act_kernel<1><<<blocks, threads, 0, st>>>(x, batch, channels, h, w, C8, terms, nullptr, *qp, a_off, phase_split,
                                                   reinterpret_cast<uint4*>(out_pk), plane_vecs, bits8, relu);
  } else {
    mnb_act_qparams none{};
    pk::pack_act_kernel<0><<<blocks, threads, 0, st>>>(x, batch, channels, h, w, C8, terms, ch_scale, none, 0, phase_split,
                                                   reinterpret_cast<uint4*>(out_pk), plane_vecs, nullptr, relu);
  }
  MNB_LAUNCHED(1);
  return 0;
}

template <typename XT>
static int bn_sign_bwd_pack(const float* g, const uint32_t* pass_bits, const XT* x, const float* dec, int32_t batch,
                            int32_t channels, int32_t hw, const float* mean, const float* invstd, const float* gamma,
                            const float* dgamma, const float* dbeta, int32_t out_shuffle_groups, const float* ch_scale,
                            int32_t terms, float* dx, void* dy_packed, mnb_stream_t stream) {
  MNB_REQUIRE(g && pass_bits && x && mean && invstd && gamma && dgamma && dbeta && dy_packed, "NULL bn_sign_bwd_pack pointer");
  MNB_REQUIRE(batch > 0 && channels > 0 && hw > 0 && terms >= 1 && terms <= 3, "bad bn_sign_bwd_pack arguments");
  MNB_REQUIRE(out_shuffle_groups >= 1 && channels % out_shuffle_groups == 0, "shuffle groups %d do not divide %d channels",
              out_shuffle_groups, channels);
  if (channels % 8 || (reinterpret_cast<uintptr_t>(dy_packed) & 15))
    return mnb_fail(MNB_E_UNSUPPORTED, "packed BatchNorm backward needs channels %% 8 == 0 and a 16-byte aligned output");
  if (hw % 32) return mnb_fail(MNB_E_UNSUPPORTED, "packed BatchNorm backward needs H*W %% 32 == 0");
  const int c8n = channels / 8;
  auto al = [](const void* p, int a) { return p == nullptr || (reinterpret_cast<uintptr_t>(p) & (uintptr_t)(a - 1)) == 0; };
  constexpr int xs = (int)sizeof(XT);
  const int vec = (hw % 128 == 0 && al(g, 16) && al(x, 4 * xs) && al(dx, 16)) ? 4
                  : ((hw % 64 == 0 && al(g, 8) && al(x, 2 * xs) && al(dx, 8)) ? 2 : 1);
  const int64_t warps = (int64_t)batch * c8n * (hw / (32 * vec));
  const int blocks = (int)std::min<int64_t>(mnb_ceil_div(warps, 8), (int64_t)MNB_NUM_SMS * 8);
  const float inv_count = 1.f / (float)((int64_t)batch * hw);
  uint4* outp = reinterpret_cast<uint4*>(dy_packed);
  const int64_t plane_vecs = (int64_t)batch * c8n * hw;
  cudaStream_t st = (cudaStream_t)stream;
#define MNB_BWD_PACK(V)                                                                                                          \
  pk::bn_sign_bwd_pack_kernel<V, XT><<<blocks, 256, 0, st>>>(g, pass_bits, x, dec, batch, channels, hw, out_shuffle_groups,     \
                                                             inv_count, mean, invstd, gamma, dgamma, dbeta, ch_scale, terms, dx, \
                                                             outp, plane_vecs)
  if (vec == 4) MNB_BWD_PACK(4); else if (vec == 2) MNB_BWD_PACK(2); else MNB_BWD_PACK(1);
#undef MNB_BWD_PACK
  MNB_LAUNCHED(1);
  return 0;
}

extern "C" int mnb_bn_sign_bwd_pack(const float* g, const uint32_t* pass_bits, const float* x, int32_t batch, int32_t channels,
                                    int32_t hw, const float* mean, const float* invstd, const float* gamma, const float* dgamma,
                                    const float* dbeta, int32_t out_shuffle_groups, const float* ch_scale, int32_t terms,
                                    float* dx, void* dy_packed, mnb_stream_t stream) {
  return bn_sign_bwd_pack<float>(g, pass_bits, x, nullptr, batch, channels, hw, mean, invstd, gamma, dgamma, dbeta,
                                 out_shuffle_groups, ch_scale, terms, dx, dy_packed, stream);
}

extern "C" int mnb_bn_sign_bwd_pack_codes(const float* g, const uint32_t* pass_bits, const int16_t* codes, const float* dec,
                                          int32_t batch, int32_t channels, int32_t hw, const float* mean, const float* invstd,
                                          const float* gamma, const float* dgamma, const float* dbeta, int32_t out_shuffle_groups,
                                          const float* ch_scale, int32_t terms, float* dx, void* dy_packed, mnb_stream_t stream) {
  MNB_REQUIRE(dec, "NULL decode pair");
  return bn_sign_bwd_pack<int16_t>(g, pass_bits, codes, dec, batch, channels, hw, mean, invstd, gamma, dgamma, dbeta,
                                   out_shuffle_groups, ch_scale, terms, dx, dy_packed, stream);
}

template <typename XT>
static int bn_sign_pool_bwd_pack(const float* g, const uint32_t* pass_bits, const uint8_t* argmax, const XT* x, const float* dec,
                                 int32_t batch, int32_t channels, int32_t H, int32_t W, const float* mean, const float* invstd,
                                 const float* gamma, const float* dgamma, const float* dbeta, int32_t out_shuffle_groups,
                                 const float* ch_scale, int32_t terms, void* dy_packed, mnb_stream_t stream) {
  MNB_REQUIRE(g && pass_bits && argmax && x && mean && invstd && gamma && dgamma && dbeta && dy_packed, "NULL bn_sign_pool_bwd_pack pointer");
  MNB_REQUIRE(batch > 0 && channels > 0 && H > 0 && W > 0 && terms >= 1 && terms <= 3, "bad bn_sign_pool_bwd_pack arguments");
  MNB_REQUIRE(out_shuffle_groups >= 1 && channels % out_shuffle_groups == 0, "shuffle groups %d do not divide %d channels",
              out_shuffle_groups, channels);
  if ((H & 1) || (W & 7) || channels % 8 || (int64_t)batch * channels * H * W >= (1ll << 31) ||
      (reinterpret_cast<uintptr_t>(x) & (4 * sizeof(XT) - 1)) || (reinterpret_cast<uintptr_t>(dy_packed) & 15) ||
      (reinterpret_cast<uintptr_t>(g) & 7))
    return mnb_fail(MNB_E_UNSUPPORTED, "packed pooled BatchNorm backward needs even H, W %% 8 == 0, channels %% 8 == 0, aligned tensors");
  const int c8n = channels / 8;
  const int64_t total = (int64_t)batch * c8n * (H / 2) * (W / 4);
  const int blocks = (int)std::min<int64_t>(mnb_ceil_div(total, 256), (int64_t)MNB_NUM_SMS * 8);
  pk::bn_sign_pool_bwd_pack_kernel<XT><<<blocks, 256, 0, (cudaStream_t)stream>>>(
      reinterpret_cast<const float2*>(g), reinterpret_cast<const uchar2*>(argmax), reinterpret_cast<const uint8_t*>(pass_bits),
      x, dec, batch, channels, H, W / 4, out_shuffle_groups, 1.f / (float)((int64_t)batch * H * W), mean,
      invstd, gamma, dgamma, dbeta, ch_scale, terms, reinterpret_cast<uint4*>(dy_packed), (int64_t)batch * c8n * H * W);
  MNB_LAUNCHED(1);
  return 0;
}

extern "C" int mnb_bn_sign_pool_bwd_pack(const float* g, const uint32_t* pass_bits, const uint8_t* argmax, const float* x,
                                         int32_t batch, int32_t channels, int32_t H, int32_t W, const float* mean,
                                         const float* invstd, const float* gamma, const float* dgamma, const float* dbeta,
                                         int32_t out_shuffle_groups, const float* ch_scale, int32_t terms, void* dy_packed,
                                         mnb_stream_t stream) {
  return bn_sign_pool_bwd_pack<float>(g, pass_bits, argmax, x, nullptr, batch, channels, H, W, mean, invstd, gamma, dgamma, dbeta,
                                      out_shuffle_groups, ch_scale, terms, dy_packed, stream);
}

extern "C" int mnb_bn_sign_pool_bwd_pack_codes(const float* g, const uint32_t* pass_bits, const uint8_t* argmax,
                                               const int16_t* codes, const float* dec, int32_t batch, int32_t channels, int32_t H,
                                               int32_t W, const float* mean, const float* invstd, const float* gamma,
                                               const float* dgamma, const float* dbeta, int32_t out_shuffle_groups,
                                               const float* ch_scale, int32_t terms, void* dy_packed, mnb_stream_t stream) {
  MNB_REQUIRE(dec, "NULL decode pair");
  return bn_sign_pool_bwd_pack<int16_t>(g, pass_bits, argmax, codes, dec, batch, channels, H, W, mean, invstd, gamma, dgamma,
                                        dbeta, out_shuffle_groups, ch_scale, terms, dy_packed, stream);
}

extern "C" int mnb_quant_add_pack_fwd(const float* a, const float* b, int32_t batch, int32_t channels, int32_t h, int32_t w,
                                      const mnb_act_qparams* qp, int32_t relu, float* out, const mnb_pk_post* post,
                                      mnb_stream_t stream) {
  return quant_add_pack<8>(a, b, batch, channels, h, w, qp, relu, out, post, stream);
}

extern "C" int mnb_bn_relu_quant_pack_fwd(const float* x, int32_t batch, int32_t channels, int32_t hw, const float* mean,
                                          const float* invstd, const float* gamma, const float* beta,
                                          const mnb_act_qparams* qp, int32_t out_shuffle_groups, void* x_packed,
                                          uint32_t* pass_bits, mnb_stream_t stream) {
  MNB_REQUIRE(x && mean && invstd && gamma && beta && qp && x_packed && pass_bits, "NULL bn_relu_quant_pack pointer");
  MNB_REQUIRE(batch > 0 && channels > 0 && hw > 0, "bad bn_relu_quant_pack shape");
  MNB_REQUIRE(qp->mode == MNB_ACT_DOREFA && qp->bits >= 2 && qp->bits <= 8, "the fused producer takes a DoReFa quantizer with 2..8 bits");
  MNB_REQUIRE(out_shuffle_groups >= 1 && channels % out_shuffle_groups == 0, "shuffle groups %d do not divide %d channels",
              out_shuffle_groups, channels);
  if (channels % 8 || hw % 32 || (reinterpret_cast<uintptr_t>(x_packed) & 15))
    return mnb_fail(MNB_E_UNSUPPORTED, "fused producer needs channels %% 8 == 0, H*W %% 32 == 0, 16-byte aligned output");
  const int64_t warps = (int64_t)batch * (channels / 8) * (hw / 32);
  const int blocks = (int)std::min<int64_t>(mnb_ceil_div(warps, 8), (int64_t)MNB_NUM_SMS * 16);
  pk::bn_relu_quant_pack_kernel<<<blocks, 256, 0, (cudaStream_t)stream>>>(x, batch, channels, hw, out_shuffle_groups, mean, invstd,
                                                                       gamma, beta, *qp, pass_bits,
                                                                       reinterpret_cast<uint4*>(x_packed));
  MNB_LAUNCHED(1);
  return 0;
}

extern "C" int mnb_bn_relu_quant_pack_i8_fwd(const float* x, int32_t batch, int32_t channels, int32_t hw, const float* mean,
                                             const float* invstd, const float* gamma, const float* beta,
                                             const mnb_act_qparams* qp, int32_t out_shuffle_groups, void* x_packed,
                                             mnb_stream_t stream) {
  MNB_REQUIRE(x && mean && invstd && gamma && beta && qp && x_packed, "NULL bn_relu_quant_pack_i8 pointer");
  MNB_REQUIRE(batch > 0 && channels > 0 && hw > 0, "bad bn_relu_quant_pack_i8 shape");
  MNB_REQUIRE(out_shuffle_groups >= 1 && channels % out_shuffle_groups == 0, "shuffle groups %d do not divide %d channels",
              out_shuffle_groups, channels);
  if (qp->mode != MNB_ACT_DOREFA || !i8_quantizer(qp))
    return mnb_fail(MNB_E_UNSUPPORTED, "bn_relu_quant_pack_i8: the int8 producer takes a DoReFa quantizer with 2..7 bits");
  if (channels % 16 || hw % 32 || (reinterpret_cast<uintptr_t>(x_packed) & 15))
    return mnb_fail(MNB_E_UNSUPPORTED, "int8 producer needs channels %% 16 == 0, H*W %% 32 == 0, 16-byte aligned output");
  const int64_t warps = (int64_t)batch * (channels / 16) * (hw / 32);
  const int blocks = (int)std::min<int64_t>(mnb_ceil_div(warps, 8), (int64_t)MNB_NUM_SMS * 16);
  pk::bn_relu_quant_pack_i8_kernel<<<blocks, 256, 0, (cudaStream_t)stream>>>(x, batch, channels, hw, out_shuffle_groups, mean,
                                                                          invstd, gamma, beta, *qp,
                                                                          reinterpret_cast<uint4*>(x_packed));
  MNB_LAUNCHED(1);
  return 0;
}

extern "C" int mnb_pk_plane_maxpool(const void* in_pk, int32_t batch, int32_t channels, int32_t h, int32_t w, int32_t k,
                                    int32_t s, int32_t p, int32_t int8, void* out_pk, mnb_stream_t stream) {
  MNB_REQUIRE(in_pk && out_pk && in_pk != out_pk, "NULL or aliased pk_plane_maxpool pointer");
  MNB_REQUIRE(batch > 0 && channels > 0 && h > 0 && w > 0, "bad pk_plane_maxpool shape");
  MNB_REQUIRE(((reinterpret_cast<uintptr_t>(in_pk) | reinterpret_cast<uintptr_t>(out_pk)) & 15) == 0,
              "packed tensors must be 16-byte aligned");
  if (k < 1 || s < 1 || p < 0 || 2 * p > k || h + 2 * p < k || w + 2 * p < k)
    return mnb_fail(MNB_E_UNSUPPORTED, "pk_plane_maxpool: kernel %d, stride %d, padding %d on %d x %d (needs 2 * p <= k)", k, s,
                    p, h, w);
  const int oh = (h + 2 * p - k) / s + 1, ow = (w + 2 * p - k) / s + 1;
  const int64_t planes = (int64_t)batch * ((channels + (int8 ? 15 : 7)) / (int8 ? 16 : 8));
  const int64_t total = planes * oh * ow;
  const int blocks = (int)std::min<int64_t>(mnb_ceil_div(total, 256), (int64_t)MNB_NUM_SMS * 16);
  auto kern = int8 ? pk::plane_maxpool_kernel<true> : pk::plane_maxpool_kernel<false>;
  kern<<<blocks, 256, 0, (cudaStream_t)stream>>>(reinterpret_cast<const uint4*>(in_pk), planes, h, w, k, s, p, oh, ow,
                                                 reinterpret_cast<uint4*>(out_pk));
  MNB_LAUNCHED(1);
  return 0;
}

extern "C" int mnb_pk_conv_plan_ex(const mnb_conv_shape* s, int32_t mode, int32_t terms_a, int32_t terms_w, int32_t* out,
                                   int32_t n) {
  pk::Plan p;
  if (int e = pk::make_plan(s, mode, terms_a, terms_w, p)) return e;
  if (out) plan_fields(p, out, n);
  return 0;
}

extern "C" int mnb_pk_conv_plan(const mnb_conv_shape* s, int32_t mode, int32_t terms_a, int32_t terms_w, int32_t* out16) {
  return mnb_pk_conv_plan_ex(s, mode, terms_a, terms_w, out16, 16);
}

extern "C" int64_t mnb_pk_wimage_bytes(const mnb_conv_shape* s, int32_t mode, int32_t terms_a, int32_t terms_w) {
  pk::Plan p;
  if (pk::make_plan(s, mode, terms_a, terms_w, p)) return -1;
  return p.wimg_bytes;
}

extern "C" int mnb_pk_pack_weight(const mnb_conv_shape* s, int32_t mode, int32_t terms_a, int32_t terms_w,
                                  const int16_t* w_int, const float* w_f32, const float* kzero, void* w_img,
                                  mnb_stream_t stream) {
  MNB_REQUIRE((w_int != nullptr) != (w_f32 != nullptr), "exactly one of w_int / w_f32");
  MNB_REQUIRE(w_img && (reinterpret_cast<uintptr_t>(w_img) & 15) == 0, "weight image must be 16-byte aligned");
  pk::PackWParams pp;
  if (int e = pk::make_plan(s, mode, terms_a, terms_w, pp.pl)) return e;
  pp.w_int = w_int; pp.w_f32 = w_f32; pp.kzero = kzero;
  pp.cin_g = s->in_c / s->groups; pp.cout_g = s->out_c / s->groups;
  const int64_t vecs = pp.pl.wimg_bytes / 16;
  const int blocks = (int)std::min<int64_t>((vecs + 255) / 256, (int64_t)MNB_NUM_SMS * 8);
  pk::pack_weight_kernel<8><<<blocks, 256, 0, (cudaStream_t)stream>>>(pp, reinterpret_cast<uint4*>(w_img));
  MNB_LAUNCHED(1);
  return 0;
}

static int pk_conv_impl(const mnb_conv_shape* s, int32_t mode, const void* a_pk, int32_t terms_a, const void* w_img,
                        int32_t terms_w, const float* n_scale, const float* a_scale, float a_scale_const,
                        const float* bias, const uint8_t* bits8, float gain, float* out, const mnb_pk_post* post,
                        int32_t* err_flag, mnb_stream_t stream, int cpu = 8, int16_t* codes = nullptr, float* dec = nullptr) {
  using namespace pk;
  MNB_REQUIRE(s && a_pk && w_img && (out || post || codes) && err_flag, "NULL pk_conv pointer");
  Plan pl;
  if (int e = make_plan(s, mode, terms_a, terms_w, pl, cpu)) return e;
  if (codes) {
    MNB_REQUIRE(mode == 0 && cpu == 8 && !out && !post && !bits8 && dec, "pk conv: int16 codes are a plain forward output");
    if (pl.segmented || terms_a != 1 || terms_w != 1)
      return unsupported("int16 codes need one activation piece, one weight piece and a non-segmented plan");
  }
  if (post) {
    const int nbn = (post->bn_mean != nullptr) + (post->bn_invstd != nullptr) + (post->bn_gamma != nullptr) + (post->bn_beta != nullptr);
    MNB_REQUIRE(nbn == 0 || nbn == 4, "pk conv: the consumer's BatchNorm needs all four of mean, invstd, gamma, beta");
    if (nbn) {
      MNB_REQUIRE(((reinterpret_cast<uintptr_t>(post->bn_mean) | reinterpret_cast<uintptr_t>(post->bn_invstd) |
                    reinterpret_cast<uintptr_t>(post->bn_gamma) | reinterpret_cast<uintptr_t>(post->bn_beta)) & 15) == 0,
                  "pk conv: the consumer's BatchNorm arrays must be 16-byte aligned");
      if (pl.NOUT % 4) return unsupported("the consumer's BatchNorm needs output channels % 4 == 0");
    }
    MNB_REQUIRE(post->shuffle_groups >= 0, "pk conv: shuffle groups %d", post->shuffle_groups);
    if (post->shuffle_groups > 1) {
      if (pl.NOUT % post->shuffle_groups) return unsupported("shuffle groups do not divide the output channels");
      if (post->phase_split) return unsupported("channel shuffle in front of a stride-2 consumer");
      if (pl.NOUT % cpu) return unsupported("shuffled consumer plane needs output channels % channels per unit == 0");
    }
  }
  if (post && cpu == 16) {
    MNB_REQUIRE(post->q && post->out_pk && (reinterpret_cast<uintptr_t>(post->out_pk) & 15) == 0, "pk conv: consumer plane / quantizer");
    if (!i8_quantizer(post->q)) return unsupported(kI8QuantizerRule);
    if (pl.G > 1 && (pl.ng % 16)) return unsupported("int8 consumer plane of a grouped conv needs channels per group % 16 == 0");
  }
  if (post) {
    MNB_REQUIRE(mode == 0 && !bits8, "pk conv: a fused consumer is a forward-only (inference) option");
    MNB_REQUIRE(post->q && post->out_pk && (reinterpret_cast<uintptr_t>(post->out_pk) & 15) == 0, "pk conv: consumer plane / quantizer");
    MNB_REQUIRE(post->q->mode == MNB_ACT_DOREFA || post->q->mode == MNB_ACT_IAO, "pk conv: consumer quantizer must be DoReFa or IAO");
    MNB_REQUIRE(post->q->bits >= 2 && post->q->bits <= 8, "pk conv: consumer levels must fit one bf16 piece (2..8 bits)");
    if (pl.G > 1 && (pl.ng % 8)) return unsupported("fused consumer of a grouped conv needs channels per group % 8 == 0");
    if (post->phase_split && ((pl.OH | pl.OW) & 1)) return unsupported("stride-2 consumer of an odd-sized plane");
    if (pl.segmented) return unsupported("fused consumer of a segmented (multi-piece) plan");
  }
  if (bits8 && pl.G > 1 && (pl.ng % 8)) return unsupported("STE mask of a grouped conv needs channels per group % 8 == 0");
  static ConvParams p;
  memset(&p, 0, sizeof(p));
  ConvParams::Mma& m = p.m;
  m.n_items = pl.n_items; m.chunks = pl.chunks; m.ksteps = pl.ksteps; m.MT = pl.MT; m.Nt = pl.Nt; m.npairs = pl.npairs;
  m.st_mask = pl.nstage - 1; m.st_log2 = pl.st_log2; m.stage16 = pl.stage_bytes >> 4;
  m.a_term16 = pl.a_bytes >> 4; m.a_mt16 = (pl.TA * pl.a_bytes) >> 4; m.a_k16 = 2 * pl.npos;
  m.b_off16 = pl.b_off >> 4; m.b_tap16 = (pl.CC / cpu) * pl.Nt; m.b_k16 = 2 * pl.Nt;
  m.a_lbo = (uint32_t)pl.npos * 16u; m.b_lbo = (uint32_t)pl.Nt * 16u;
  m.seg_len = (uint32_t)pl.seg_len;
  int nprog = 0;
  uint32_t* prog = reinterpret_cast<uint32_t*>(m.prog4);
  for (int i = 0; i < MAXPROG; ++i) prog[i] = 0xffffffffu;
  for (int y = 0; y < pl.ny; ++y) {
    m.ntmpl[y] = pl.ntmpl[y]; p.ntmpl[y] = pl.ntmpl[y];
    for (int t = 0; t < pl.ntmpl[y]; ++t) {
      const Tmpl& tp = pl.tmpl[y][t];
      p.tmpl_kph[y][t] = tp.kph; p.tmpl_blk_off[y][t] = tp.blk_off; p.tmpl_blk_bytes[y][t] = tp.blk_bytes;
      const int cnt = tp.ntap * pl.npairs * pl.ksteps;
      nprog = (nprog + 3) & ~3;
      m.tmpl_begin[y][t] = (uint16_t)(nprog / 4); m.tmpl_cnt[y][t] = (uint16_t)((cnt + 3) / 4);
      if (nprog + ((cnt + 3) & ~3) > MAXPROG) return unsupported("MMA program longer than 512 entries");
      for (int pr = 0; pr < pl.npairs; ++pr)
        for (int i = 0; i < tp.ntap; ++i)
          for (int j = 0; j < pl.ksteps; ++j) {
            const uint32_t a16 = (uint32_t)pl.tap_aoff[y][tp.tap0 + i] + (uint32_t)pl.pair_a[pr] * m.a_term16 + (uint32_t)j * m.a_k16;
            const uint32_t b16 = (uint32_t)i * m.b_tap16 + (uint32_t)pl.pair_b[pr] * (uint32_t)tp.ntap * m.b_tap16 + (uint32_t)j * m.b_k16;
            if (a16 > 0xffffu || b16 > 0xffffu) return mnb_fail(MNB_E_ARG, "pk conv: MMA program offset overflow");
            prog[nprog++] = a16 | (b16 << 16);
          }
    }
    p.img_bytes[y] = pl.img_bytes[y]; p.y_off[y] = pl.y_off[y];
  }
  p.n_items = pl.n_items; p.n_ntiles = pl.n_ntiles; p.G = pl.G; p.MT = pl.MT; p.TA = pl.TA; p.chunks = pl.chunks;
  p.CC8 = pl.CC / cpu; p.C8A = pl.C8A; p.kg8 = pl.kg / cpu; p.stage_bytes = pl.stage_bytes; p.a_bytes = pl.a_bytes;
  p.a_box_bytes = pl.a_box_bytes; p.b_off = pl.b_off; p.st_mask = pl.nstage - 1; p.st_log2 = pl.st_log2;
  p.Wt = pl.Wt; p.TH = pl.TH; p.TB = pl.TB; p.wlo = pl.wlo; p.hlo = pl.hlo; p.col_tiles = pl.col_tiles; p.row_tiles = pl.row_tiles;
  p.n_mtiles = pl.n_mtiles;
  p.w_img = reinterpret_cast<const uint8_t*>(w_img);
  p.B = pl.B; p.THH = pl.THH; p.BW = pl.BW; p.OHr = pl.OHr; p.OWr = pl.OWr; p.OH = pl.OH; p.OW = pl.OW; p.omul = pl.omul; p.ny = pl.ny;
  p.ng = pl.ng; p.Nt = pl.Nt; p.NOUT = pl.NOUT; p.C8O = ceil_div(pl.NOUT, cpu); p.smem_bytes = pl.smem_bytes; p.off_stg = pl.off_stg;
  p.mode = mode;
  p.n_scale = n_scale; p.a_scale = a_scale; p.a_scale_const = a_scale_const; p.bias = bias; p.bits8 = bits8; p.gain = gain;
  p.out = out; p.err = err_flag; p.codes = codes; p.dec = dec;
  if (post) {
    p.post_out = reinterpret_cast<uint4*>(post->out_pk); p.post_q = *post->q; p.post_relu = post->relu; p.post_split = post->phase_split;
    p.post_mean = post->bn_mean; p.post_invstd = post->bn_invstd; p.post_gamma = post->bn_gamma; p.post_beta = post->bn_beta;
    p.post_sg = post->shuffle_groups;
  }
  { static const int dbg = [] { const char* e = getenv("MNB_PK_DEBUG"); return e ? atoi(e) : 0; }(); p.dbg = dbg; }
  CUtensorMap tm[3];
  const int C8tot = pl.nkph * pl.C8A;
  const int64_t plane_bytes = (int64_t)pl.B * C8tot * pl.HA * pl.WA * 16;
  for (int t = 0; t < 3; ++t) {
    const int tt = t < pl.TA ? t : 0;
    if (int e = make_pk_tmap(&tm[t], a_pk, plane_bytes, tt, pl.B, C8tot, pl.HA, pl.WA, pl.BW, pl.THH, pl.TB, pl.CC / cpu)) return e;
  }
  if (pl.n_items >= (1 << 22) || pl.n_mtiles >= (1 << 22))
    return mnb_fail(MNB_E_UNSUPPORTED, "pk conv: %d work items / %d M tiles exceed the index arithmetic of the kernel", pl.n_items, pl.n_mtiles);
  const int gx = std::max(1, std::min(pl.n_items, MNB_NUM_SMS / pl.ny));
  using ConvFn = void (*)(const CUtensorMap, const CUtensorMap, const CUtensorMap, const ConvParams);
#define MNB_PK_CONV_FNS(SEG, I8, X) {pk_conv_kernel<SEG, 16, I8, X>, pk_conv_kernel<SEG, 32, I8, X>, pk_conv_kernel<SEG, 48, I8, X>, \
                                     pk_conv_kernel<SEG, 64, I8, X>, pk_conv_kernel<SEG, 96, I8, X>, pk_conv_kernel<SEG, 128, I8, X>}
  static const ConvFn fns[5][6] = {MNB_PK_CONV_FNS(false, false, false), MNB_PK_CONV_FNS(true, false, false),
                                   MNB_PK_CONV_FNS(false, true, false), MNB_PK_CONV_FNS(false, false, true),
                                   MNB_PK_CONV_FNS(false, true, true)};
#undef MNB_PK_CONV_FNS
  int ki = -1;
  for (int i = 0; i < 6; ++i) if (kNtSizes[i] == pl.Nt) ki = i;
  if (ki < 0 || pl.MT * pl.Nt > 128) return mnb_fail(MNB_E_ARG, "pk conv: plan with Nt %d, MT %d", pl.Nt, pl.MT);
  const bool xpost = post && (post->bn_mean || post->shuffle_groups > 1);
  const ConvFn fn = fns[cpu == 16 ? (xpost ? 4 : 2) : (pl.segmented ? 1 : (xpost ? 3 : 0))][ki];
  if (int e = set_max_smem(fn, kSmemBudget)) return e;
  fn<<<dim3(gx, pl.ny), kConvThreads, pl.smem_bytes, (cudaStream_t)stream>>>(tm[0], tm[1], tm[2], p);
  MNB_LAUNCHED(1);
  return 0;
}

extern "C" int mnb_pk_conv(const mnb_conv_shape* s, int32_t mode, const void* a_pk, int32_t terms_a, const void* w_img,
                           int32_t terms_w, const float* n_scale, const float* a_scale, float a_scale_const,
                           const float* bias, const uint8_t* bits8, float gain, float* out, int32_t* err_flag,
                           mnb_stream_t stream) {
  MNB_REQUIRE(out, "NULL pk_conv output");
  return pk_conv_impl(s, mode, a_pk, terms_a, w_img, terms_w, n_scale, a_scale, a_scale_const, bias, bits8, gain, out, nullptr,
                      err_flag, stream);
}

extern "C" int mnb_pk_conv_post(const mnb_conv_shape* s, const void* a_pk, int32_t terms_a, const void* w_img, int32_t terms_w,
                                const float* n_scale, const float* a_scale, float a_scale_const, const float* bias,
                                float* out, const mnb_pk_post* post, int32_t* err_flag, mnb_stream_t stream) {
  MNB_REQUIRE(post, "NULL consumer description");
  return pk_conv_impl(s, 0, a_pk, terms_a, w_img, terms_w, n_scale, a_scale, a_scale_const, bias, nullptr, 1.f, out, post,
                      err_flag, stream);
}

extern "C" int mnb_pk_conv_codes(const mnb_conv_shape* s, const void* a_pk, int32_t terms_a, const void* w_img, int32_t terms_w,
                                 const float* n_scale, const float* a_scale, float a_scale_const, const float* bias,
                                 int32_t level_bound, int16_t* codes, float* dec, int32_t* err_flag, mnb_stream_t stream) {
  MNB_REQUIRE(s && codes && dec, "NULL pk_conv_codes pointer");
  MNB_REQUIRE(level_bound >= 1 && s->groups >= 1, "pk_conv_codes: level bound %d", level_bound);
  if ((int64_t)(s->in_c / s->groups) * s->ker_h * s->ker_w * level_bound > 32767)
    return mnb_fail(MNB_E_UNSUPPORTED, "pk_conv_codes: sums of %d x %d x %d terms of level %d may exceed int16", s->in_c / s->groups,
                    s->ker_h, s->ker_w, level_bound);
  return pk_conv_impl(s, 0, a_pk, terms_a, w_img, terms_w, n_scale, a_scale, a_scale_const, bias, nullptr, 1.f, nullptr, nullptr,
                      err_flag, stream, 8, codes, dec);
}


extern "C" int64_t mnb_pk_i8_act_bytes(int32_t batch, int32_t channels, int32_t h, int32_t w) {
  return (int64_t)batch * ((channels + 15) / 16) * h * w * 16;
}

extern "C" int mnb_pk_i8_pack_act(const float* x, int32_t batch, int32_t channels, int32_t h, int32_t w, const mnb_act_qparams* qp,
                                  int32_t phase_split, int32_t relu, void* out_pk, mnb_stream_t stream) {
  MNB_REQUIRE(x && qp && out_pk, "NULL pk_i8_pack_act pointer");
  MNB_REQUIRE(batch > 0 && channels > 0 && h > 0 && w > 0, "bad pk_i8_pack_act arguments");
  MNB_REQUIRE((reinterpret_cast<uintptr_t>(out_pk) & 15) == 0, "packed tensor must be 16-byte aligned");
  if (!i8_quantizer(qp)) return mnb_fail(MNB_E_UNSUPPORTED, "pk_i8_pack_act: %s", kI8QuantizerRule);
  if (phase_split) MNB_REQUIRE(((h | w) & 1) == 0, "phase split needs even H and W");
  MNB_REQUIRE((int64_t)h * w < (1ll << 31), "pk_i8_pack_act: plane too large");
  const int C16 = (channels + 15) / 16;
  dim3 blocks, threads;
  if (!unit_grid(batch, C16, h * w, blocks, threads))
    return mnb_fail(MNB_E_UNSUPPORTED, "pk_i8_pack_act: %d (image, unit) planes exceed the grid", batch * C16);
  pk::pack_act_i8_kernel<<<blocks, threads, 0, (cudaStream_t)stream>>>(x, batch, channels, h, w, C16, *qp, phase_split,
                                                                               relu, reinterpret_cast<uint4*>(out_pk));
  MNB_LAUNCHED(1);
  return 0;
}

extern "C" int mnb_pk_i8_conv_plan(const mnb_conv_shape* s, int32_t* out, int32_t n) {
  pk::Plan p;
  if (int e = pk::make_plan(s, 0, 1, 1, p, 16)) return e;
  if (out) plan_fields(p, out, n);
  return 0;
}

extern "C" int64_t mnb_pk_i8_wimage_bytes(const mnb_conv_shape* s) {
  pk::Plan p;
  if (pk::make_plan(s, 0, 1, 1, p, 16)) return -1;
  return p.wimg_bytes;
}

extern "C" int mnb_pk_i8_pack_weight(const mnb_conv_shape* s, const int16_t* w_int, void* w_img, mnb_stream_t stream) {
  MNB_REQUIRE(w_int, "NULL pk_i8_pack_weight levels");
  MNB_REQUIRE(w_img && (reinterpret_cast<uintptr_t>(w_img) & 15) == 0, "weight image must be 16-byte aligned");
  pk::PackWParams pp;
  if (int e = pk::make_plan(s, 0, 1, 1, pp.pl, 16)) return e;
  pp.w_int = w_int; pp.w_f32 = nullptr; pp.kzero = nullptr;
  pp.cin_g = s->in_c / s->groups; pp.cout_g = s->out_c / s->groups;
  const int64_t vecs = pp.pl.wimg_bytes / 16;
  const int blocks = (int)std::min<int64_t>((vecs + 255) / 256, (int64_t)MNB_NUM_SMS * 8);
  pk::pack_weight_kernel<16><<<blocks, 256, 0, (cudaStream_t)stream>>>(pp, reinterpret_cast<uint4*>(w_img));
  MNB_LAUNCHED(1);
  return 0;
}

extern "C" int mnb_pk_i8_conv(const mnb_conv_shape* s, const void* a_pk, const void* w_img, const float* n_scale,
                              const float* a_scale, float a_scale_const, const float* bias, float* out, const mnb_pk_post* post,
                              int32_t* err_flag, mnb_stream_t stream) {
  MNB_REQUIRE(out || post, "pk_i8_conv: NULL out needs a consumer plane (post)");
  return pk_conv_impl(s, 0, a_pk, 1, w_img, 1, n_scale, a_scale, a_scale_const, bias, nullptr, 1.f, out, post, err_flag, stream, 16);
}

extern "C" int mnb_quant_add_pack_i8_fwd(const float* a, const float* b, int32_t batch, int32_t channels, int32_t h, int32_t w,
                                         const mnb_act_qparams* qp, int32_t relu, float* out, const mnb_pk_post* post,
                                         mnb_stream_t stream) {
  return quant_add_pack<16>(a, b, batch, channels, h, w, qp, relu, out, post, stream);
}

extern "C" int64_t mnb_pk_wgrad_scratch_bytes(const mnb_conv_shape* s, int32_t terms_dy, int32_t terms_x) {
  pk::WgPlan p;
  if (pk::make_wg_plan(s, terms_dy, terms_x, p)) return -1;
  return p.partial_floats * 4;
}

extern "C" int mnb_pk_wgrad_plan(const mnb_conv_shape* s, int32_t terms_dy, int32_t terms_x, int32_t* out, int32_t n) {
  pk::WgPlan p;
  if (int e = pk::make_wg_plan(s, terms_dy, terms_x, p)) return e;
  if (out) {
    const int v[10] = {p.Nc, p.n_ctiles, p.tpg, p.n_tg, p.gm, p.splits, p.NI, p.nstage, p.BW, p.TH};
    for (int i = 0; i < std::min(n, 10); ++i) out[i] = v[i];
  }
  return 0;
}

extern "C" int mnb_pk_wgrad(const mnb_conv_shape* s, const void* dy_pk, int32_t terms_dy, const void* x_pk, int32_t terms_x,
                            const float* a_scale, const float* kdiv, float* dw, void* scratch, int32_t* err_flag,
// ... 113 lines not shown
```

micronet_b200/csrc/mnb_quant.cu:

```cuda
#include <math.h>
#include <stdarg.h>
#include <stdio.h>

#include <atomic>

#include "mnb_common.cuh"

static thread_local char g_mnb_err[512] = "";
static std::atomic<int64_t> g_mnb_launches{0};

int mnb_fail(int code, const char* fmt, ...) {
  va_list ap;
  va_start(ap, fmt);
  vsnprintf(g_mnb_err, sizeof(g_mnb_err), fmt, ap);
  va_end(ap);
  return code;
}
void mnb_count_launches(int n) { g_mnb_launches.fetch_add(n, std::memory_order_relaxed); }

extern "C" int mnb_version(void) { return 100; }
extern "C" const char* mnb_last_error(void) { return g_mnb_err; }
extern "C" int64_t mnb_launch_count(void) { return g_mnb_launches.load(); }

static inline cudaStream_t S(mnb_stream_t s) { return (cudaStream_t)s; }
// ... 642 lines not shown
      stats[channels + c] = (float)(1.0 / sqrt(ss / (double)per + bn.eps));
      const float m = bn.momentum;
      bn.running_mean[c] = __fadd_rn(__fmul_rn(1.f - m, bn.running_mean[c]), __fmul_rn(m, (float)mean));
      bn.running_var[c] = __fadd_rn(__fmul_rn(1.f - m, bn.running_var[c]), __fmul_rn(m, (float)var));
      if (c == 0 && bn.num_batches_tracked) *bn.num_batches_tracked += 1;
    } else {
      stats[channels + c] = (float)var;
    }
  } else {
    stats[c] = (float)s1;
    stats[channels + c] = (float)s2;
  }
  counters[c] = 0;
}

__global__ void __launch_bounds__(256) channel_stats_bwd_kernel(const float* __restrict__ x,
                                                                const float* __restrict__ mean,
                                                                const float* __restrict__ dmean,
                                                                const float* __restrict__ dvar, int batch,
                                                                int channels, int hw, float* __restrict__ dx) {
  const int64_t n = (int64_t)batch * channels * hw;
  const float N = (float)((int64_t)batch * hw);
  int64_t i = (int64_t)blockIdx.x * blockDim.x + threadIdx.x;
  const int64_t stride = (int64_t)gridDim.x * blockDim.x;
  for (; i < n; i += stride) {
    int c = (int)((i / hw) % channels);
    float a = __fdiv_rn(__ldg(dmean + c), N);
    float b = __fmul_rn(__ldg(dvar + c), __fdiv_rn(2.f, N - 1.f));
    dx[i] = __fadd_rn(a, __fmul_rn(b, __fsub_rn(__ldg(x + i), __ldg(mean + c))));
  }
}

extern "C" int mnb_channel_stats(const float* x, int32_t batch, int32_t channels, int32_t hw,
                                 int32_t as_mean_var, float* stats, void* scratch, mnb_stream_t stream) {
  MNB_REQUIRE(x && stats && scratch && batch > 0 && channels > 0 && hw > 0, "bad channel_stats arguments");
  MNB_REQUIRE(channels <= 8192, "channel_stats supports at most 8192 channels, got %d", channels);
  int64_t per = (int64_t)batch * hw;
  int splits = (int)std::max<int64_t>(1, std::min<int64_t>(std::min<int64_t>(STATS_SPLITS, batch), per / 2048));
  splits = std::max(1, std::min(splits, (2 * 8 * MNB_NUM_SMS + channels - 1) / channels));
  uint32_t* counters = reinterpret_cast<uint32_t*>(reinterpret_cast<char*>(scratch) + 16384);
  double* partial = reinterpret_cast<double*>(reinterpret_cast<char*>(scratch) + 49152);
  MNB_REQUIRE(as_mean_var >= 0 && as_mean_var <= 2, "as_mean_var must be 0, 1 or 2");
  channel_stats_kernel<float><<<dim3(channels, splits), 256, 0, S(stream)>>>(x, nullptr, batch, channels, hw, as_mean_var,
                                                                              stats, counters, partial, MnbBnUpdate{});
  MNB_LAUNCHED(1);
  return 0;
}

template <typename XT>
static int bn_batch_stats(const XT* x, const float* dec, int32_t batch, int32_t channels, int32_t hw, double eps, double momentum,
                          float* running_mean, float* running_var, int64_t* num_batches_tracked, float* mean_invstd,
                          void* scratch, mnb_stream_t stream) {
  MNB_REQUIRE(x && running_mean && running_var && mean_invstd && scratch && batch > 0 && channels > 0 && hw > 0,
              "bad bn_batch_stats arguments");
  MNB_REQUIRE(channels <= 8192, "bn_batch_stats supports at most 8192 channels, got %d", channels);
  MNB_REQUIRE((int64_t)batch * hw > 1, "batch statistics need more than one value per channel");
  int64_t per = (int64_t)batch * hw;
  int splits = (int)std::max<int64_t>(1, std::min<int64_t>(std::min<int64_t>(STATS_SPLITS, batch), per / 2048));
  splits = std::max(1, std::min(splits, (2 * 8 * MNB_NUM_SMS + channels - 1) / channels));
  uint32_t* counters = reinterpret_cast<uint32_t*>(reinterpret_cast<char*>(scratch) + 16384);
  double* partial = reinterpret_cast<double*>(reinterpret_cast<char*>(scratch) + 49152);
  MnbBnUpdate bn{eps, (float)momentum, running_mean, running_var, reinterpret_cast<long long*>(num_batches_tracked)};
  channel_stats_kernel<XT><<<dim3(channels, splits), 256, 0, S(stream)>>>(x, dec, batch, channels, hw, 3, mean_invstd, counters,
                                                                           partial, bn);
  MNB_LAUNCHED(1);
  return 0;
}

extern "C" int mnb_bn_batch_stats(const float* x, int32_t batch, int32_t channels, int32_t hw, double eps, double momentum,
                                  float* running_mean, float* running_var, int64_t* num_batches_tracked,
                                  float* mean_invstd, void* scratch, mnb_stream_t stream) {
  return bn_batch_stats<float>(x, nullptr, batch, channels, hw, eps, momentum, running_mean, running_var, num_batches_tracked,
                               mean_invstd, scratch, stream);
}

extern "C" int mnb_bn_batch_stats_codes(const int16_t* codes, const float* dec, int32_t batch, int32_t channels, int32_t hw,
                                        double eps, double momentum, float* running_mean, float* running_var,
                                        int64_t* num_batches_tracked, float* mean_invstd, void* scratch, mnb_stream_t stream) {
  MNB_REQUIRE(dec, "NULL decode pair");
  return bn_batch_stats<int16_t>(codes, dec, batch, channels, hw, eps, momentum, running_mean, running_var, num_batches_tracked,
                                 mean_invstd, scratch, stream);
}

extern "C" int mnb_channel_stats_bwd(const float* x, const float* mean, const float* dmean, const float* dvar,
                                     int32_t batch, int32_t channels, int32_t hw, float* dx,
                                     mnb_stream_t stream) {
  MNB_REQUIRE(x && mean && dmean && dvar && dx && batch > 0 && channels > 0 && hw > 0, "bad channel_stats_bwd arguments");
  int64_t n = (int64_t)batch * channels * hw;
  int blocks = (int)std::min<int64_t>(mnb_ceil_div(n, 256 * 4), MNB_NUM_SMS * 8);
  channel_stats_bwd_kernel<<<blocks, 256, 0, S(stream)>>>(x, mean, dmean, dvar, batch, channels, hw, dx);
  MNB_LAUNCHED(1);
  return 0;
}

__global__ void __launch_bounds__(256) adam_step_kernel(float* __restrict__ p, const float* __restrict__ g,
                                                        float* __restrict__ m, float* __restrict__ v, int64_t n,
                                                        float lr, float b1, float b2, float eps, float wd,
                                                        float bc1, float sqrt_bc2) {
  int64_t i = (int64_t)blockIdx.x * blockDim.x + threadIdx.x;
  const int64_t stride = (int64_t)gridDim.x * blockDim.x;
  const float step_size = lr / bc1;
  for (; i < n; i += stride) {
    float gi = g[i];
    const float pi = p[i];
    if (wd != 0.f) gi = fmaf(wd, pi, gi);
    const float mi = m[i] + (gi - m[i]) * (1.f - b1);
    const float vi = fmaf(1.f - b2, gi * gi, v[i] * b2);
    const float denom = sqrtf(vi) / sqrt_bc2 + eps;
    m[i] = mi; v[i] = vi;
    p[i] = pi - step_size * (mi / denom);
  }
}

extern "C" int mnb_adam_step(float* p, const float* g, float* m, float* v, int64_t n, float lr, float beta1,
                             float beta2, float eps, float weight_decay, int32_t step, mnb_stream_t stream) {
  MNB_REQUIRE(p && g && m && v && n >= 0 && step >= 1, "bad Adam arguments");
  if (n == 0) return 0;
  const float bc1 = (float)(1.0 - pow((double)beta1, (double)step));
  const float sqrt_bc2 = (float)sqrt(1.0 - pow((double)beta2, (double)step));
  int blocks = (int)std::min<int64_t>(mnb_ceil_div(n, 256), MNB_NUM_SMS * 8);
  adam_step_kernel<<<blocks, 256, 0, S(stream)>>>(p, g, m, v, n, lr, beta1, beta2, eps, weight_decay, bc1, sqrt_bc2);
  MNB_LAUNCHED(1);
  return 0;
}

__global__ void __launch_bounds__(256) quant_add_fwd_kernel(const float* __restrict__ a, const float* __restrict__ b,
                                                            int64_t n, mnb_act_qparams p, float* __restrict__ out,
                                                            uint32_t* __restrict__ bits_a, uint32_t* __restrict__ bits_b,
                                                            int relu) {
  const MnbActQ q = mnb_load_actq(p);
  const int lane = threadIdx.x & 31;
  const int64_t warp = ((int64_t)blockIdx.x * blockDim.x + threadIdx.x) >> 5;
  const int64_t nwarps = ((int64_t)gridDim.x * blockDim.x) >> 5;
  for (int64_t base = warp * 128; base < n; base += nwarps * 128) {
    float va[4], vb[4];
#pragma unroll
    for (int j = 0; j < 4; ++j) {
      const int64_t i = base + lane + 32 * j;
      va[j] = (i < n) ? __ldg(a + i) : 0.f;
      vb[j] = (i < n) ? __ldg(b + i) : 0.f;
    }
#pragma unroll
    for (int j = 0; j < 4; ++j) {
      const int64_t i = base + lane + 32 * j;
      bool pa, pb;
      const int ca = mnb_act_code_certified(q, va[j], pa), cb = mnb_act_code_certified(q, vb[j], pb);
      float oa, ob;
      if (q.mode == MNB_ACT_DOREFA) { oa = __fmul_rn((float)ca, q.s); ob = __fmul_rn((float)cb, q.s); }
      else {
        oa = __fmul_rn(__fadd_rn((float)(ca + q.qmin), q.zp), q.s);
        ob = __fmul_rn(__fadd_rn((float)(cb + q.qmin), q.zp), q.s);
      }
      const bool live = i < n;
      const uint32_t wa = __ballot_sync(0xffffffffu, live && pa), wb = __ballot_sync(0xffffffffu, live && pb);
      if (live) { const float sum = __fadd_rn(oa, ob); out[i] = relu ? fmaxf(sum, 0.f) : sum; }
      if (lane == 0 && (base + 32 * j) < n) {
        if (bits_a) bits_a[(base >> 5) + j] = wa;
        if (bits_b) bits_b[(base >> 5) + j] = wb;
      }
    }
  }
}

__global__ void __launch_bounds__(256) quant_add_bwd_kernel(const float* __restrict__ g, const uint32_t* __restrict__ bits_a,
                                                            const uint32_t* __restrict__ bits_b, int64_t n,
                                                            mnb_act_qparams p, float* __restrict__ da, float* __restrict__ db) {
// ... 124 lines not shown
```

micronet_b200/functional.py:

```python
from __future__ import annotations

import ctypes as C

import torch
from torch.autograd import Function

from . import _lib as L


class KernelTimer:

    def __init__(self):
        self.records = []

    def run(self, kind, sh, fn):
        a, b = torch.cuda.Event(enable_timing=True), torch.cuda.Event(enable_timing=True)
        a.record()
        rc = fn()
        b.record()
        self.records.append((kind, tuple(getattr(sh, f) for f, _ in sh._fields_), a, b))
        return rc

    def summary(self):
        out = {}
# ... 151 lines not shown
        w_scale = torch.empty(k, dtype=torch.float32, device=w.device)
        aux = torch.empty(3 * k, dtype=torch.float32, device=w.device)
        L.check(lib.mnb_wb_weight_fwd(w.data_ptr(), k, cpg, khw, W, w_int.data_ptr(), w_scale.data_ptr(),
                                      wq.data_ptr(), aux.data_ptr(), L.stream()), "wb_weight_fwd")
        ctx.w, ctx.aux, ctx.W = w.detach(), aux, W
        ctx.mark_non_differentiable(w_int, w_scale)
        return wq, w_int, w_scale

    @staticmethod
    def backward(ctx, g, _gi, _gs):
        lib = L.load()
        g = g.contiguous()
        w = ctx.w
        dw = torch.empty_like(g)
        L.check(lib.mnb_wb_weight_bwd(g.data_ptr(), w.data_ptr(), ctx.aux.data_ptr(), w.shape[0], w.shape[1],
                                      w.shape[2] * w.shape[3], ctx.W, dw.data_ptr(), L.stream()),
                "wb_weight_bwd")
        return dw, None


class IaoWeightFn(Function):

    @staticmethod
    def forward(ctx, w, scale, zero_point, obs_min, obs_max, q_type, qmin, qmax):
        L.require_cuda(w)
        lib = L.load()
        w = w.contiguous()
        n, k, rows = w.numel(), w.shape[0], scale.numel()
        wq = torch.empty_like(w)
        w_int = torch.empty(w.shape, dtype=torch.int16, device=w.device)
        w_scale = torch.empty(k, dtype=torch.float32, device=w.device)
        keep = torch.empty(w.shape, dtype=torch.uint8, device=w.device)
        L.check(lib.mnb_iao_weight_fwd(w.data_ptr(), n, k, rows, scale.data_ptr(), zero_point.data_ptr(),
                                       obs_min.data_ptr(), obs_max.data_ptr(), q_type, qmin, qmax,
                                       w_int.data_ptr(), w_scale.data_ptr(), wq.data_ptr(), keep.data_ptr(),
                                       L.stream()), "iao_weight_fwd")
        ctx.keep, ctx.scale, ctx.k, ctx.rows = keep, scale, k, rows
        ctx.mark_non_differentiable(w_int, w_scale)
        return wq, w_int, w_scale

    @staticmethod
    def backward(ctx, g, _gi, _gs):
        lib = L.load()
        g = g.contiguous()
        dw = torch.empty_like(g)
        L.check(lib.mnb_iao_weight_bwd(g.data_ptr(), ctx.keep.data_ptr(), ctx.scale.data_ptr(), g.numel(),
                                       ctx.k, ctx.rows, dw.data_ptr(), L.stream()), "iao_weight_bwd")
        return (dw,) + (None,) * 7


def _shape_struct(x_shape, w_shape, stride, padding, dilation, groups):
    b, c, h, w = x_shape
    k, _, r, s = w_shape
    return L.ConvShape(b, c, h, w, k, r, s, stride[0], stride[1], padding[0], padding[1],
                       dilation[0], dilation[1], groups)


def _out_hw(sh: L.ConvShape):
    p = (sh.in_h + 2 * sh.pad_h - sh.dil_h * (sh.ker_h - 1) - 1) // sh.stride_h + 1
    q = (sh.in_w + 2 * sh.pad_w - sh.dil_w * (sh.ker_w - 1) - 1) // sh.stride_w + 1
    return p, q


def channel_sums(x4):
    lib = L.load()
    b, c = x4.shape[0], x4.shape[1]
    hw = x4.numel() // (b * c)
    out = torch.empty(2 * c, dtype=torch.float32, device=x4.device)
    L.check(lib.mnb_channel_stats(x4.data_ptr(), b, c, hw, 0, out.data_ptr(),
                                  L.scratch(x4.device, c).data_ptr(), L.stream()), "channel_stats")
    return out[:c]



def materialized(t):
    xbits = getattr(t, "_mnb_xbits", None)
    if xbits is not None:
        from . import xnor as XN
        return XN.unpack(xbits[1], t.shape, xbits[3])
    codes = getattr(t, "_mnb_codes", None)
    if codes is not None:
        b, c = t.shape[0], t.shape[1]
        out = torch.empty(t.shape, dtype=torch.float32, device=t.device)
        L.check(L.load().mnb_codes_decode(codes[0].data_ptr(), codes[1].data_ptr(), b, c, t.numel() // (b * c), out.data_ptr(),
                                          L.stream()), "codes_decode")
        return out
    if not getattr(t, "_mnb_plane_only", False):
        return t
    b, c, h, w = t.shape
    plane = t._mnb_pk_pm1.view(torch.bfloat16).view(b, c // 8, h, w, 8)
    return plane.permute(0, 1, 4, 2, 3).reshape(b, c, h, w).float()


def xnor_preferred(sh, has_plane):
    return not has_plane


def _pk_terms(spec, w_int, pm1=False):
    T = L.PK_TERMS
    if spec is None:
        ta = 1 if pm1 else T
    else:
        ta = 2 if (spec.mode == L.ACT_IAO and spec.q_type == 1) else 1
    return ta, (1 if w_int is not None else T)


def _pk_forward(ctx, x, wq, bias, w_int, w_scale, spec, sh, y, need_dx, prepacked=None, pre_relu=False, pm1=False,
                codes_out=False):
    from . import pk as PK
    ta, tw = _pk_terms(spec, w_int, pm1)
    if not PK.supported(sh, 0, ta, tw):
        return False
    Tb = min(L.PK_TERMS, L.PK_TERMS_BWD)
    if need_dx and not PK.supported(sh, 1, Tb, 1 if w_int is not None else Tb):
        return False
    if ctx.needs_input_grad[1] and not PK.wgrad_supported(sh, Tb, min(ta, Tb)):
        return False
    qp = spec.struct() if spec is not None else None
    split = sh.stride_h == 2
    if prepacked is not None:
        x_pk, bits8 = prepacked, None
    else:
        x_pk, bits8 = PK.pack_act(x, qp, ta, phase_split=split, want_bits=need_dx, relu=pre_relu)
    src = w_int if w_int is not None else wq
    cache = getattr(src, "_mnb_pk_cache", None)
    ckey = (PK._key(sh), ta, tw)
    w_img = cache.get(ckey) if cache is not None else None
    if w_img is None:
        w_img = PK.pack_weight(sh, 0, ta, tw, w_int=w_int, w_f32=None if w_int is not None else wq)
        if cache is not None:
            cache[ckey] = w_img
    a_scale, a_const = None, 1.0
    if spec is not None:
        if spec.mode == L.ACT_IAO:
            a_scale = spec.scale.clone() if (need_dx or ctx.needs_input_grad[1]) else spec.scale
        elif spec.mode == L.ACT_DOREFA:
            a_const = 1.0 / float(2 ** spec.bits - 1)
    rc = L.E_UNSUPPORTED
    if codes_out and w_int is not None and ta == 1 and tw == 1:
        codes = torch.empty(y.shape, dtype=torch.int16, device=y.device)
        dec = torch.empty(2 * y.shape[1], dtype=torch.float32, device=y.device)
        rc = _timed("fwd_pk", sh, lambda: PK.conv_codes(sh, x_pk, w_img, codes, dec, n_scale=w_scale, a_scale=a_scale,
                                                        a_scale_const=a_const, bias=bias))
        if rc == 0:
            y._mnb_codes = (codes, dec)
    if rc == L.E_UNSUPPORTED:
        rc = _timed("fwd_pk", sh, lambda: PK.conv(sh, 0, x_pk, ta, w_img, tw, y,
                                                  n_scale=w_scale if w_int is not None else None,
                                                  a_scale=a_scale, a_scale_const=a_const, bias=bias))
    if rc == L.E_UNSUPPORTED:
        return False
    L.check(rc, "pk_conv fwd")
    ctx.pk = True
    ctx.pk_x, ctx.pk_ta, ctx.pk_bits8, ctx.pk_a_scale, ctx.pk_prepacked = x_pk, ta, bits8, a_scale, prepacked is not None
    return True


def _pk_backward(ctx, dy):
    from . import pk as PK
    sh, spec = ctx.sh, ctx.spec
    T = min(L.PK_TERMS, L.PK_TERMS_BWD)
    int_w = ctx.w_int is not None
    need_dx, need_dw = ctx.needs_input_grad[0], ctx.needs_input_grad[1]
    fold = int_w and need_dx
    pre = getattr(dy, "_mnb_pk_dy", None)
    if pre is not None:
        if pre[1] != T or (pre[2] is not None) != fold:
            raise RuntimeError("micronet_b200: packed gradient operand does not match this layer's backward configuration")
        dy_pk = pre[0]
    else:
        dy_pk, _ = PK.pack_act(dy, None, T, ch_scale=ctx.w_scale if fold else None)
    dx = dwq = None
    if need_dx:
        tw = 1 if int_w else T
        w_img = PK.pack_weight(sh, 1, T, tw, w_int=ctx.w_int, w_f32=None if int_w else ctx.wq,
                               kzero=ctx.w_scale if int_w else None)
        dx = torch.empty((sh.batch, sh.in_c, sh.in_h, sh.in_w), dtype=torch.float32, device=dy.device)
        gain = 0.1 if (spec is not None and spec.mode == L.ACT_DOREFA) else 1.0
        plain_gain = gain if ctx.pk_prepacked else 1.0
        L.check(_timed("dgrad_pk", sh, lambda: PK.conv(sh, 1, dy_pk, T, w_img, tw, dx, bits8=ctx.pk_bits8, gain=gain,
                                                       a_scale_const=plain_gain)), "pk_conv dgrad")
    if need_dw:
        dwq = torch.empty_like(ctx.wq)
        a_scale = None
        if spec is not None:
            a_scale = ctx.pk_a_scale if spec.mode == L.ACT_IAO else _dorefa_scale_tensor(spec.bits, dy.device)
        tx = min(ctx.pk_ta, T)
        kdiv = ctx.w_scale if fold else None
        fn = PK.wgrad_taps if L.PK_WG_TAPS and PK.wgrad_taps_plan(sh, T, tx) is not None else PK.wgrad
        L.check(_timed("wgrad_pk", sh, lambda: fn(sh, dy_pk, T, ctx.pk_x, tx, dwq, a_scale=a_scale, kdiv=kdiv)), "pk_wgrad")
    return dx, dwq


class QuantConv2dFn(Function):

    @staticmethod
    def forward(ctx, x, wq, bias, w_int, w_scale, spec, stride, padding, dilation, groups, pre_relu=False, no_grad=False,
                codes_out=False):
        L.require_cuda(x, wq)
        assert not (pre_relu and any(ctx.needs_input_grad)), "the folded ReLU is an inference-only fusion"
        lib = L.load()
        packed = getattr(x, "_mnb_packed", None) if L.USE_PACKED else None
        x = x.contiguous()
        wq = wq.contiguous()
        sh = _shape_struct(x.shape, wq.shape, stride, padding, dilation, groups)
        p, q = _out_hw(sh)
        y = torch.empty((x.shape[0], wq.shape[0], p, q), dtype=torch.float32, device=x.device)
        codes = bits = None
        a_scale = None
        if spec is not None and spec.mode != L.ACT_SIGN:
            a_scale = spec.scale if spec.mode == L.ACT_IAO else _dorefa_scale_tensor(spec.bits, x.device)
        done = False
        ctx.pk = False
        if (L.XNOR_MODE != "off" and spec is None and w_int is not None and getattr(x, "_mnb_pm1", False)
                and (no_grad or not any(ctx.needs_input_grad[:3])) and x.dtype == torch.float32 and not pre_relu):
            from . import xnor as XN
            if XN.supported(sh) and (L.XNOR_MODE == "all" or xnor_preferred(sh, getattr(x, "_mnb_pk_pm1", None) is not None)):
                a_bits = XN.pack_act(materialized(x), groups)
                rc = _timed("fwd_xnor", sh, lambda: XN.conv(sh, a_bits, XN.pack_weight(sh, w_int), y, alpha=w_scale, bias=bias))
                if rc == 0:
                    done = True
                elif rc != L.E_UNSUPPORTED:
                    L.check(rc, "xnor_conv_fwd")
        pkq = getattr(x, "_mnb_pk_q", None)
        if pkq is not None and not done:
            if spec is None or spec.mode != L.ACT_DOREFA or spec.bits != pkq[1] or w_int is None:
# ... 505 lines not shown
```

micronet_b200/fused.py:

```python
from __future__ import annotations

import torch
import torch.nn as nn
from torch.autograd import Function

import ctypes as C

import torch.nn.functional as TF

from . import _lib as L


def _xargs(lib, name, x, codes):
    if codes is None:
        return getattr(lib, name), (x.data_ptr(),)
    return getattr(lib, name + "_codes"), (codes[0].data_ptr(), codes[1].data_ptr())


class BNSignFn(Function):

    @staticmethod
    def forward(ctx, x, gamma, beta, mean, invstd, training, shuffle_groups, pool, plane_only=False):
        from . import functional as F_
        lib = L.load()
        x = x.contiguous()
        b, c = x.shape[0], x.shape[1]
        hw = x.numel() // (b * c)
        pk_conv = getattr(x, "_mnb_pk_conv", None)
        codes = getattr(x, "_mnb_codes", None)
        if codes is not None and not pool and (L.USE_PACKED or not (L.PK_WBWTAB and c % 8 == 0 and hw % 32 == 0
                                                                    and x.dim() == 4 and L.PK_MODE != "off")):
            x, codes = F_.materialized(x), None
        bits = torch.empty((x.numel() + 31) // 32, dtype=torch.int32, device=x.device)
        arg = None
        if pool:
            h, w = x.shape[2], x.shape[3]
            y = torch.empty((b, c, h // 2, w // 2), dtype=x.dtype, device=x.device)
            arg = torch.empty(y.numel(), dtype=torch.uint8, device=x.device)
            fn, xa = _xargs(lib, "mnb_bn_sign_pool_fwd", x, codes)
            L.check(fn(*xa, b, c, h, w, mean.data_ptr(), invstd.data_ptr(), gamma.data_ptr(), beta.data_ptr(), shuffle_groups,
                       y.data_ptr(), bits.data_ptr(), arg.data_ptr(), L.stream()), "bn_sign_pool_fwd")
        else:
            y = torch.empty_like(x)
            packed = None
            if L.PK_WBWTAB and not L.USE_PACKED and c % 8 == 0 and hw % 32 == 0 and x.dim() == 4 and L.PK_MODE != "off":
                plane = torch.empty(x.numel() * 2, dtype=torch.uint8, device=x.device)
                skip_y = bool(plane_only) and L.PLANE_ONLY
                fn, xa = _xargs(lib, "mnb_bn_sign_fwd_packed", x, codes)
                rc = fn(*xa, b, c, hw, mean.data_ptr(), invstd.data_ptr(), gamma.data_ptr(), beta.data_ptr(), shuffle_groups,
                        None if skip_y else y.data_ptr(), bits.data_ptr(), plane.data_ptr(), L.stream())
                if rc == 0:
                    y._mnb_pk_pm1 = plane
                    if skip_y:
                        y._mnb_plane_only = True
                    packed = False
                elif rc != L.E_UNSUPPORTED:
                    L.check(rc, "bn_sign_fwd_packed")
                elif codes is not None:
                    x, codes = F_.materialized(x), None
            if packed is None and L.USE_PACKED and c % 8 == 0 and hw % 32 == 0:
                packed = torch.empty(x.numel(), dtype=torch.bfloat16, device=x.device)
                rc = lib.mnb_bn_sign_fwd_packed(x.data_ptr(), b, c, hw, mean.data_ptr(), invstd.data_ptr(), gamma.data_ptr(),
                                                beta.data_ptr(), shuffle_groups, y.data_ptr(), bits.data_ptr(),
                                                packed.data_ptr(), L.stream())
                if rc == L.E_UNSUPPORTED:
                    packed = None
                else:
                    L.check(rc, "bn_sign_fwd_packed")
            if packed is None:
                L.check(lib.mnb_bn_sign_fwd(x.data_ptr(), b, c, hw, mean.data_ptr(), invstd.data_ptr(), gamma.data_ptr(),
                                            beta.data_ptr(), shuffle_groups, y.data_ptr(), bits.data_ptr(), L.stream()),
                        "bn_sign_fwd")
            elif packed is not False:
                y._mnb_packed = packed
        y._mnb_pm1 = True
        ctx.save_for_backward(x, gamma, mean, invstd)
        ctx.bits, ctx.arg, ctx.training, ctx.shuffle_groups = bits, arg, training, shuffle_groups
        ctx.pk_conv, ctx.codes = pk_conv, codes
        return y

    @staticmethod
    def backward(ctx, g):
        lib = L.load()
        x, gamma, mean, invstd = ctx.saved_tensors
        g = g.contiguous()
        b, c = x.shape[0], x.shape[1]
        hw = x.numel() // (b * c)
        dx = torch.empty_like(x)
        out = torch.empty(3 * c, dtype=torch.float32, device=x.device)
        dgamma, dbeta, dx_sum = out[:c], out[c:2 * c], out[2 * c:]
        scratch = L.scratch(x.device, c)
        if (ctx.arg is not None and ctx.pk_conv is not None and ctx.training and c % 8 == 0 and x.shape[3] % 8 == 0
                and x.shape[2] % 2 == 0 and "mnb_bn_sign_pool_bwd_pack" in L.PROTOTYPES):
            w_scale, T = ctx.pk_conv
            fn, xa = _xargs(lib, "mnb_bn_sign_pool_bwd", x, ctx.codes)
            L.check(fn(g.data_ptr(), ctx.bits.data_ptr(), ctx.arg.data_ptr(), *xa, b, c, x.shape[2], x.shape[3],
                       mean.data_ptr(), invstd.data_ptr(), gamma.data_ptr(), 2, ctx.shuffle_groups, dx.data_ptr(),
                       dgamma.data_ptr(), dbeta.data_ptr(), None, scratch.data_ptr(), L.stream()), "bn_sign_pool_bwd (reduce)")
            dy_pk = torch.empty(T * x.numel() * 2, dtype=torch.uint8, device=x.device)
# ... 444 lines not shown
```

micronet_b200/pk.py:

```python
from __future__ import annotations

import ctypes as C

import torch

from . import _lib as L

_plan_cache = {}


def _key(sh):
    return tuple(getattr(sh, f) for f, _ in sh._fields_)


def supported(sh, mode, terms_a, terms_w):
    k = ("c", _key(sh), mode, terms_a, terms_w)
    if k not in _plan_cache:
        _plan_cache[k] = L.load().mnb_pk_conv_plan(C.byref(sh), mode, terms_a, terms_w, None) == 0
    return _plan_cache[k]


def segmented(sh, mode, terms_a, terms_w):
    k = ("s", _key(sh), mode, terms_a, terms_w)
    if k not in _plan_cache:
        out = (C.c_int32 * 17)()
        _plan_cache[k] = L.load().mnb_pk_conv_plan_ex(C.byref(sh), mode, terms_a, terms_w, out, 17) == 0 and out[16] != 0
    return _plan_cache[k]


def wgrad_supported(sh, terms_dy, terms_x):
    k = ("w", _key(sh), terms_dy, terms_x)
    if k not in _plan_cache:
        _plan_cache[k] = int(L.load().mnb_pk_wgrad_scratch_bytes(C.byref(sh), terms_dy, terms_x))
    return _plan_cache[k] >= 0


def pack_act(x, qp, terms, ch_scale=None, phase_split=False, want_bits=False, relu=False):
    lib = L.load()
    b, c, h, w = x.shape
    nbytes = int(lib.mnb_pk_act_bytes(b, c, h, w, terms))
    out = torch.empty(nbytes, dtype=torch.uint8, device=x.device)
    bits = None
    if qp is not None and want_bits:
        bits = torch.empty((b, (c + 7) // 8, h, w), dtype=torch.uint8, device=x.device)
    L.check(lib.mnb_pk_pack_act_relu(x.data_ptr(), b, c, h, w, None if qp is None else C.byref(qp), terms, L.ptr(ch_scale),
                                     1 if phase_split else 0, 1 if relu else 0, out.data_ptr(), L.ptr(bits), L.stream()),
            "pk_pack_act")
    return out, bits


def pack_weight(sh, mode, terms_a, terms_w, w_int=None, w_f32=None, kzero=None):
    lib = L.load()
    nbytes = int(lib.mnb_pk_wimage_bytes(C.byref(sh), mode, terms_a, terms_w))
    if nbytes < 0:
        raise ValueError("micronet_b200.pk: shape outside the cover of the packed-operand convolution")
    dev = (w_int if w_int is not None else w_f32).device
    img = torch.empty(nbytes, dtype=torch.uint8, device=dev)
    L.check(lib.mnb_pk_pack_weight(C.byref(sh), mode, terms_a, terms_w, L.ptr(w_int), L.ptr(w_f32), L.ptr(kzero),
                                   img.data_ptr(), L.stream()), "pk_pack_weight")
    return img


def conv(sh, mode, a_pk, terms_a, w_img, terms_w, out, n_scale=None, a_scale=None, a_scale_const=1.0, bias=None,
         bits8=None, gain=1.0):
    lib = L.load()
    return lib.mnb_pk_conv(C.byref(sh), mode, a_pk.data_ptr(), terms_a, w_img.data_ptr(), terms_w, L.ptr(n_scale),
                           L.ptr(a_scale), float(a_scale_const), L.ptr(bias), L.ptr(bits8), float(gain), out.data_ptr(),
                           L.tc_err_flag(out.device).data_ptr(), L.stream())


def conv_codes(sh, a_pk, w_img, codes, dec, n_scale=None, a_scale=None, a_scale_const=1.0, bias=None, level_bound=1):
    return L.load().mnb_pk_conv_codes(C.byref(sh), a_pk.data_ptr(), 1, w_img.data_ptr(), 1, L.ptr(n_scale), L.ptr(a_scale),
                                      float(a_scale_const), L.ptr(bias), int(level_bound), codes.data_ptr(), dec.data_ptr(),
                                      L.tc_err_flag(codes.device).data_ptr(), L.stream())


def codes_fit(in_channels, groups, kernel_size, level_bound=1):
    r, s = (kernel_size, kernel_size) if isinstance(kernel_size, int) else kernel_size
    return (in_channels // groups) * r * s * level_bound <= 32767


def consumer_plane(b, c, h, w, device):
    return torch.empty(int(L.load().mnb_pk_act_bytes(b, c, h, w, 1)), dtype=torch.uint8, device=device)


def post_struct(qp, plane, relu, split, bn=None, shuffle_groups=1):
    post = L.PkPost(C.pointer(qp), 1 if relu else 0, 1 if split else 0, plane.data_ptr())
    if bn is not None:
        post.bn_mean, post.bn_invstd, post.bn_gamma, post.bn_beta = (t.data_ptr() for t in bn)
    post.shuffle_groups = int(shuffle_groups)
    return post


def conv_post(sh, a_pk, terms_a, w_img, terms_w, out, post_qp, post_plane, post_relu, post_split, n_scale=None, a_scale=None,
              a_scale_const=1.0, bias=None, bn=None, shuffle_groups=1):
    lib = L.load()
    post = post_struct(post_qp, post_plane, post_relu, post_split, bn, shuffle_groups)
    return lib.mnb_pk_conv_post(C.byref(sh), a_pk.data_ptr(), terms_a, w_img.data_ptr(), terms_w, L.ptr(n_scale), L.ptr(a_scale),
                                float(a_scale_const), L.ptr(bias), L.ptr(out), C.byref(post),
                                L.tc_err_flag(a_pk.device).data_ptr(), L.stream())


def i8_plan(sh):
    out = (C.c_int32 * 21)()
    return list(out) if L.load().mnb_pk_i8_conv_plan(C.byref(sh), out, 21) == 0 else None


def i8_supported(sh):
    k = ("i8", _key(sh))
    if k not in _plan_cache:
        _plan_cache[k] = L.load().mnb_pk_i8_conv_plan(C.byref(sh), None, 0) == 0
    return _plan_cache[k]


def consumer_plane_i8(b, c, h, w, device):
    return torch.empty(int(L.load().mnb_pk_i8_act_bytes(b, c, h, w)), dtype=torch.uint8, device=device)


def pack_act_i8(x, qp, phase_split=False, relu=False):
    b, c, h, w = x.shape
    out = consumer_plane_i8(b, c, h, w, x.device)
    L.check(L.load().mnb_pk_i8_pack_act(x.data_ptr(), b, c, h, w, C.byref(qp), 1 if phase_split else 0, 1 if relu else 0,
                                        out.data_ptr(), L.stream()), "pk_i8_pack_act")
    return out


def plane_maxpool(plane, b, c, h, w, k, s, p, int8=False):
    oh, ow = (h + 2 * p - k) // s + 1, (w + 2 * p - k) // s + 1
    out = (consumer_plane_i8 if int8 else consumer_plane)(b, c, oh, ow, plane.device)
    L.check(L.load().mnb_pk_plane_maxpool(plane.data_ptr(), b, c, h, w, k, s, p, 1 if int8 else 0, out.data_ptr(), L.stream()),
            "pk_plane_maxpool")
    return out


def pack_weight_i8(sh, w_int):
    nbytes = int(L.load().mnb_pk_i8_wimage_bytes(C.byref(sh)))
    if nbytes < 0:
        raise ValueError("micronet_b200.pk: shape outside the cover of the int8 convolution")
    img = torch.empty(nbytes, dtype=torch.uint8, device=w_int.device)
    L.check(L.load().mnb_pk_i8_pack_weight(C.byref(sh), w_int.data_ptr(), img.data_ptr(), L.stream()), "pk_i8_pack_weight")
    return img


def conv_i8(sh, a_pk, w_img, out, n_scale=None, a_scale=None, a_scale_const=1.0, bias=None, post=None):
    pp = None
    if post is not None:
        pp = C.byref(post_struct(*post))
    return L.load().mnb_pk_i8_conv(C.byref(sh), a_pk.data_ptr(), w_img.data_ptr(), L.ptr(n_scale), L.ptr(a_scale),
                                   float(a_scale_const), L.ptr(bias), L.ptr(out), pp, L.tc_err_flag(a_pk.device).data_ptr(),
                                   L.stream())


def wgrad(sh, dy_pk, terms_dy, x_pk, terms_x, dw, a_scale=None, kdiv=None):
    lib = L.load()
    nbytes = int(lib.mnb_pk_wgrad_scratch_bytes(C.byref(sh), terms_dy, terms_x))
    if nbytes < 0:
        return L.E_UNSUPPORTED
    ws = torch.empty(max(nbytes, 16), dtype=torch.uint8, device=dw.device)
    return lib.mnb_pk_wgrad(C.byref(sh), dy_pk.data_ptr(), terms_dy, x_pk.data_ptr(), terms_x, L.ptr(a_scale),
                            L.ptr(kdiv), dw.data_ptr(), ws.data_ptr(), L.tc_err_flag(dw.device).data_ptr(), L.stream())


# ... 23 lines not shown
```

Before: 38130.

## Store conv outputs as int8 codes with per-channel parity for BN consumers

Adds an int8 code path for the packed convolution's output. When padding is zero, weights are ternary and the reduction length is at most 255, all sums in a channel share one parity, so the code stores the value shifted right by one plus a per-channel parity in a third decode row. All BN/sign consumer kernels are instantiated for int8 to read half the bytes of the int16 codes. The parity is taken from a single lane's accumulator, which adds an assumption about how each channel is produced.

```diff
diff --git a/harness/step_profile.py b/harness/step_profile.py
--- a/harness/step_profile.py
+++ b/harness/step_profile.py
@@ -74,7 +74,8 @@
 
     def hook(mod, inp):
         x = inp[0]
-        calls.append({"n": x.numel(), "xb": 2 if getattr(x, "_mnb_codes", None) is not None else 4,
+        codes = getattr(x, "_mnb_codes", None)
+        calls.append({"n": x.numel(), "xb": codes[0].element_size() if codes is not None else 4,
                       "pool2": bool(mod.pool2), "plane_only": bool(mod.plane_only) and not mod.pool2,
                       "pk_conv": getattr(x, "_mnb_pk_conv", None) is not None})
 
diff --git a/include/micronet_b200.h b/include/micronet_b200.h
--- a/include/micronet_b200.h
+++ b/include/micronet_b200.h
@@ -200,6 +200,37 @@
                                     const float* invstd, const float* gamma, const float* dgamma, const float* dbeta,
                                     int32_t out_shuffle_groups, const float* ch_scale, int32_t terms, void* dy_packed,
                                     mnb_stream_t stream);
+int mnb_pk_conv_codes8(const mnb_conv_shape* s, const void* a_pk, int32_t terms_a, const void* w_img, int32_t terms_w,
+                       const float* n_scale, const float* a_scale, float a_scale_const, const float* bias, int32_t level_bound,
+                       int8_t* codes, float* dec, int32_t* err_flag, mnb_stream_t stream);
+int mnb_codes_decode8(const int8_t* codes, const float* dec, int32_t batch, int32_t channels, int32_t hw, float* x,
+                      mnb_stream_t stream);
+int mnb_bn_batch_stats_codes8(const int8_t* codes, const float* dec, int32_t batch, int32_t channels, int32_t hw, double eps,
+                              double momentum, float* running_mean, float* running_var, int64_t* num_batches_tracked,
+                              float* mean_invstd, void* scratch, mnb_stream_t stream);
+int mnb_bn_sign_fwd_packed_codes8(const int8_t* codes, const float* dec, int32_t batch, int32_t channels, int32_t hw,
+                                  const float* mean, const float* invstd, const float* gamma, const float* beta,
+                                  int32_t out_shuffle_groups, float* y, uint32_t* pass_bits, void* x_packed, mnb_stream_t stream);
+int mnb_bn_sign_bwd_codes8(const float* g, const uint32_t* pass_bits, const int8_t* codes, const float* dec, int32_t batch,
+                           int32_t channels, int32_t hw, const float* mean, const float* invstd, const float* gamma,
+                           int32_t training, int32_t out_shuffle_groups, float* dx, float* dgamma, float* dbeta,
+                           float* dx_channel_sum, void* scratch, mnb_stream_t stream);
+int mnb_bn_sign_pool_fwd_codes8(const int8_t* codes, const float* dec, int32_t batch, int32_t channels, int32_t H, int32_t W,
+                                const float* mean, const float* invstd, const float* gamma, const float* beta,
+                                int32_t out_shuffle_groups, float* y, uint32_t* pass_bits, uint8_t* argmax, mnb_stream_t stream);
+int mnb_bn_sign_pool_bwd_codes8(const float* g, const uint32_t* pass_bits, const uint8_t* argmax, const int8_t* codes,
+                                const float* dec, int32_t batch, int32_t channels, int32_t H, int32_t W, const float* mean,
+                                const float* invstd, const float* gamma, int32_t training, int32_t out_shuffle_groups, float* dx,
+                                float* dgamma, float* dbeta, float* dx_channel_sum, void* scratch, mnb_stream_t stream);
+int mnb_bn_sign_bwd_pack_codes8(const float* g, const uint32_t* pass_bits, const int8_t* codes, const float* dec, int32_t batch,
+                                int32_t channels, int32_t hw, const float* mean, const float* invstd, const float* gamma,
+                                const float* dgamma, const float* dbeta, int32_t out_shuffle_groups, const float* ch_scale,
+                                int32_t terms, float* dx, void* dy_packed, mnb_stream_t stream);
+int mnb_bn_sign_pool_bwd_pack_codes8(const float* g, const uint32_t* pass_bits, const uint8_t* argmax, const int8_t* codes,
+                                     const float* dec, int32_t batch, int32_t channels, int32_t H, int32_t W, const float* mean,
+                                     const float* invstd, const float* gamma, const float* dgamma, const float* dbeta,
+                                     int32_t out_shuffle_groups, const float* ch_scale, int32_t terms, void* dy_packed,
+                                     mnb_stream_t stream);
 int mnb_pk_pack_act_relu(const float* x, int32_t batch, int32_t channels, int32_t h, int32_t w, const mnb_act_qparams* qp,
                          int32_t terms, const float* ch_scale, int32_t phase_split, int32_t relu, void* out_pk,
                          uint8_t* bits8, mnb_stream_t stream);
diff --git a/micronet_b200/_lib.py b/micronet_b200/_lib.py
--- a/micronet_b200/_lib.py
+++ b/micronet_b200/_lib.py
@@ -112,6 +112,16 @@
     "mnb_bn_sign_bwd_pack_codes": (C.c_int, [_P, _P, _P, _P, _I, _I, _I, _P, _P, _P, _P, _P, _I, _P, _I, _P, _P, _P]),
     "mnb_bn_sign_pool_bwd_pack_codes": (C.c_int, [_P, _P, _P, _P, _P, _I, _I, _I, _I, _P, _P, _P, _P, _P, _I, _P, _I, _P,
                                                   _P]),
+    "mnb_pk_conv_codes8": (C.c_int, [_SHAPE, _P, _I, _P, _I, _P, _P, C.c_float, _P, _I, _P, _P, _P, _P]),
+    "mnb_codes_decode8": (C.c_int, [_P, _P, _I, _I, _I, _P, _P]),
+    "mnb_bn_batch_stats_codes8": (C.c_int, [_P, _P, _I, _I, _I, _D, _D, _P, _P, _P, _P, _P, _P]),
+    "mnb_bn_sign_fwd_packed_codes8": (C.c_int, [_P, _P, _I, _I, _I, _P, _P, _P, _P, _I, _P, _P, _P, _P]),
+    "mnb_bn_sign_bwd_codes8": (C.c_int, [_P, _P, _P, _P, _I, _I, _I, _P, _P, _P, _I, _I, _P, _P, _P, _P, _P, _P]),
+    "mnb_bn_sign_pool_fwd_codes8": (C.c_int, [_P, _P, _I, _I, _I, _I, _P, _P, _P, _P, _I, _P, _P, _P, _P]),
+    "mnb_bn_sign_pool_bwd_codes8": (C.c_int, [_P, _P, _P, _P, _P, _I, _I, _I, _I, _P, _P, _P, _I, _I, _P, _P, _P, _P, _P, _P]),
+    "mnb_bn_sign_bwd_pack_codes8": (C.c_int, [_P, _P, _P, _P, _I, _I, _I, _P, _P, _P, _P, _P, _I, _P, _I, _P, _P, _P]),
+    "mnb_bn_sign_pool_bwd_pack_codes8": (C.c_int, [_P, _P, _P, _P, _P, _I, _I, _I, _I, _P, _P, _P, _P, _P, _I, _P, _I, _P,
+                                                   _P]),
     "mnb_quant_add_pack_fwd": (C.c_int, [_P, _P, _I, _I, _I, _I, _ACTQ, _I, _P, C.POINTER(PkPost), _P]),
     "mnb_pk_i8_act_bytes": (_L, [_I, _I, _I, _I]),
     "mnb_pk_i8_pack_act": (C.c_int, [_P, _I, _I, _I, _I, _ACTQ, _I, _I, _P, _P]),
diff --git a/micronet_b200/csrc/mnb_common.cuh b/micronet_b200/csrc/mnb_common.cuh
--- a/micronet_b200/csrc/mnb_common.cuh
+++ b/micronet_b200/csrc/mnb_common.cuh
@@ -65,20 +65,23 @@
   return fmaf(-xhat, dg, __fsub_rn(g, db));
 }
 
-struct XDec { float s, b; };
+struct XDec { float s, b, p; };
 template <typename XT> struct XVec;
 template <> struct XVec<float> { typedef float t1; typedef float2 t2; typedef float4 t4; };
 template <> struct XVec<int16_t> { typedef short t1; typedef short2 t2; typedef short4 t4; };
+template <> struct XVec<int8_t> { typedef signed char t1; typedef char2 t2; typedef char4 t4; };
 
 template <typename XT>
 __device__ __forceinline__ XDec x_dec(const float* dec, int channels, int c) {
-  if constexpr (sizeof(XT) == 4) return XDec{1.f, 0.f};
-  else return XDec{__ldg(dec + c), __ldg(dec + channels + c)};
+  if constexpr (sizeof(XT) == 4) return XDec{1.f, 0.f, 0.f};
+  else if constexpr (sizeof(XT) == 2) return XDec{__ldg(dec + c), __ldg(dec + channels + c), 0.f};
+  else return XDec{__ldg(dec + c), __ldg(dec + channels + c), __ldg(dec + 2 * channels + c)};
 }
 template <typename XT>
 __device__ __forceinline__ float x_val(XT q, XDec d) {
   if constexpr (sizeof(XT) == 4) return q;
-  else return fmaf((float)q, d.s, d.b);
+  else if constexpr (sizeof(XT) == 2) return fmaf((float)q, d.s, d.b);
+  else return fmaf(fmaf(2.f, (float)q, d.p), d.s, d.b);
 }
 template <int VEC, typename XT>
 __device__ __forceinline__ void x_load(const XT* p, XDec d, float (&v)[VEC]) {
diff --git a/micronet_b200/csrc/mnb_conv_packed.cu b/micronet_b200/csrc/mnb_conv_packed.cu
--- a/micronet_b200/csrc/mnb_conv_packed.cu
+++ b/micronet_b200/csrc/mnb_conv_packed.cu
@@ -117,3 +117,12 @@
   return bn_sign_fwd_packed<int16_t>(codes, dec, batch, channels, hw, mean, invstd, gamma, beta, out_shuffle_groups, y, pass_bits,
                                      x_packed, stream);
 }
+
+extern "C" int mnb_bn_sign_fwd_packed_codes8(const int8_t* codes, const float* dec, int32_t batch, int32_t channels, int32_t hw,
+                                             const float* mean, const float* invstd, const float* gamma, const float* beta,
+                                             int32_t out_shuffle_groups, float* y, uint32_t* pass_bits, void* x_packed,
+                                             mnb_stream_t stream) {
+  MNB_REQUIRE(dec, "NULL decode triple");
+  return bn_sign_fwd_packed<int8_t>(codes, dec, batch, channels, hw, mean, invstd, gamma, beta, out_shuffle_groups, y, pass_bits,
+                                    x_packed, stream);
+}
diff --git a/micronet_b200/csrc/mnb_fused.cu b/micronet_b200/csrc/mnb_fused.cu
--- a/micronet_b200/csrc/mnb_fused.cu
+++ b/micronet_b200/csrc/mnb_fused.cu
@@ -302,6 +302,15 @@
                               dgamma, dbeta, dx_channel_sum, scratch, stream);
 }
 
+extern "C" int mnb_bn_sign_bwd_codes8(const float* g, const uint32_t* pass_bits, const int8_t* codes, const float* dec,
+                                      int32_t batch, int32_t channels, int32_t hw, const float* mean, const float* invstd,
+                                      const float* gamma, int32_t training, int32_t out_shuffle_groups, float* dx, float* dgamma,
+                                      float* dbeta, float* dx_channel_sum, void* scratch, mnb_stream_t stream) {
+  MNB_REQUIRE(dec, "NULL decode triple");
+  return bn_sign_bwd<int8_t>(g, pass_bits, codes, dec, batch, channels, hw, mean, invstd, gamma, training, out_shuffle_groups, dx,
+                             dgamma, dbeta, dx_channel_sum, scratch, stream);
+}
+
 struct PoolGeom { uint32_t channels, H, W4, OH, OW2, sg; };
 
 __device__ __forceinline__ uint32_t first_max_of_signs(bool p0, bool p1, bool p2, bool p3) {
@@ -512,6 +521,15 @@
                                    argmax, stream);
 }
 
+extern "C" int mnb_bn_sign_pool_fwd_codes8(const int8_t* codes, const float* dec, int32_t batch, int32_t channels, int32_t H,
+                                           int32_t W, const float* mean, const float* invstd, const float* gamma, const float* beta,
+                                           int32_t out_shuffle_groups, float* y, uint32_t* pass_bits, uint8_t* argmax,
+                                           mnb_stream_t stream) {
+  MNB_REQUIRE(dec, "NULL decode triple");
+  return bn_sign_pool_fwd<int8_t>(codes, dec, batch, channels, H, W, mean, invstd, gamma, beta, out_shuffle_groups, y, pass_bits,
+                                  argmax, stream);
+}
+
 template <typename XT>
 static int bn_sign_pool_bwd(const float* g, const uint32_t* pass_bits, const uint8_t* argmax, const XT* x, const float* dec,
                             int32_t batch, int32_t channels, int32_t H, int32_t W, const float* mean, const float* invstd,
@@ -558,6 +576,16 @@
                                    out_shuffle_groups, dx, dgamma, dbeta, dx_channel_sum, scratch, stream);
 }
 
+extern "C" int mnb_bn_sign_pool_bwd_codes8(const float* g, const uint32_t* pass_bits, const uint8_t* argmax, const int8_t* codes,
+                                           const float* dec, int32_t batch, int32_t channels, int32_t H, int32_t W,
+                                           const float* mean, const float* invstd, const float* gamma, int32_t training,
+                                           int32_t out_shuffle_groups, float* dx, float* dgamma, float* dbeta,
+                                           float* dx_channel_sum, void* scratch, mnb_stream_t stream) {
+  MNB_REQUIRE(dec, "NULL decode triple");
+  return bn_sign_pool_bwd<int8_t>(g, pass_bits, argmax, codes, dec, batch, channels, H, W, mean, invstd, gamma, training,
+                                  out_shuffle_groups, dx, dgamma, dbeta, dx_channel_sum, scratch, stream);
+}
+
 __global__ void __launch_bounds__(256) maxpool_fwd_kernel(const float* __restrict__ x, int64_t n_out, int channels, int H, int W,
                                                           int OH, int OW, int k, int st, int pad, int sg,
                                                           float* __restrict__ y, uint8_t* __restrict__ arg) {
@@ -716,21 +744,33 @@
   return 0;
 }
 
-__global__ void __launch_bounds__(256) codes_decode_kernel(const int16_t* __restrict__ codes, const float* __restrict__ dec,
+template <typename XT>
+__global__ void __launch_bounds__(256) codes_decode_kernel(const XT* __restrict__ codes, const float* __restrict__ dec,
                                                            int64_t n, int channels, int hw, float* __restrict__ x) {
   const int64_t stride = (int64_t)gridDim.x * blockDim.x;
   for (int64_t i = (int64_t)blockIdx.x * blockDim.x + threadIdx.x; i < n; i += stride) {
     const int c = (int)((i / hw) % channels);
-    x[i] = x_val<int16_t>(__ldg(codes + i), x_dec<int16_t>(dec, channels, c));
-  }
-}
-
-extern "C" int mnb_codes_decode(const int16_t* codes, const float* dec, int32_t batch, int32_t channels, int32_t hw, float* x,
-                                mnb_stream_t stream) {
+    x[i] = x_val<XT>(__ldg(codes + i), x_dec<XT>(dec, channels, c));
+  }
+}
+
+template <typename XT>
+static int codes_decode(const XT* codes, const float* dec, int32_t batch, int32_t channels, int32_t hw, float* x,
+                        mnb_stream_t stream) {
   MNB_REQUIRE(codes && dec && x && batch > 0 && channels > 0 && hw > 0, "bad codes_decode arguments");
   const int64_t n = (int64_t)batch * channels * hw;
   const int blocks = (int)std::min<int64_t>(mnb_ceil_div(n, 256), MNB_NUM_SMS * 8);
-  codes_decode_kernel<<<blocks, 256, 0, S(stream)>>>(codes, dec, n, channels, hw, x);
+  codes_decode_kernel<XT><<<blocks, 256, 0, S(stream)>>>(codes, dec, n, channels, hw, x);
   MNB_LAUNCHED(1);
   return 0;
 }
+
+extern "C" int mnb_codes_decode(const int16_t* codes, const float* dec, int32_t batch, int32_t channels, int32_t hw, float* x,
+                                mnb_stream_t stream) {
+  return codes_decode<int16_t>(codes, dec, batch, channels, hw, x, stream);
+}
+
+extern "C" int mnb_codes_decode8(const int8_t* codes, const float* dec, int32_t batch, int32_t channels, int32_t hw, float* x,
+                                 mnb_stream_t stream) {
+  return codes_decode<int8_t>(codes, dec, batch, channels, hw, x, stream);
+}
diff --git a/micronet_b200/csrc/mnb_pk.cu b/micronet_b200/csrc/mnb_pk.cu
--- a/micronet_b200/csrc/mnb_pk.cu
+++ b/micronet_b200/csrc/mnb_pk.cu
@@ -750,6 +750,7 @@
   float gain;
   float* out;
   int16_t* codes;
+  int8_t* codes8;
   float* dec;
   uint4* post_out;
   mnb_act_qparams post_q;
@@ -955,6 +956,18 @@
           for (int i = 0; i < NR; ++i) acc[mt][i] = __int2float_rn(__float_as_int(acc[mt][i]));
         }
       }
+      if constexpr (!SEG && !I8 && !XPOST) {
+        if (p.codes8 && mg == 0 && y == 0 && warp == 4 && lane < 4) {
+#pragma unroll
+          for (int j = 0; j < NR / 4; ++j) {
+#pragma unroll
+            for (int e = 0; e < 2; ++e) {
+              const int n = 8 * j + 2 * lane + e;
+              if (n < n_cnt) p.dec[2 * p.NOUT + n_base + n] = (float)(__float2int_rn(acc[0][4 * j + e]) & 1);
+            }
+          }
+        }
+      }
       int mt_cur = -1;
       bool valid = false;
       int64_t orow = 0;
@@ -982,6 +995,13 @@
           }
         }
         if (!valid || n0 >= n_cnt || (p.dbg & 1)) return;
+        if (!SEG && !I8 && !XPOST && p.codes8) {
+          int8_t* cp = p.codes8 + orow + (int64_t)n0 * plane;
+#pragma unroll
+          for (int k = 0; k < 16; ++k, cp += plane)
+            if (n0 + k < n_cnt) *cp = (int8_t)(__float2int_rn(r[k]) >> 1);
+          return;
+        }
         if (!SEG && !I8 && p.codes) {
           int16_t* cp = p.codes + orow + (int64_t)n0 * plane;
 #pragma unroll
@@ -1703,6 +1723,15 @@
                                    out_shuffle_groups, ch_scale, terms, dx, dy_packed, stream);
 }
 
+extern "C" int mnb_bn_sign_bwd_pack_codes8(const float* g, const uint32_t* pass_bits, const int8_t* codes, const float* dec,
+                                           int32_t batch, int32_t channels, int32_t hw, const float* mean, const float* invstd,
+                                           const float* gamma, const float* dgamma, const float* dbeta, int32_t out_shuffle_groups,
+                                           const float* ch_scale, int32_t terms, float* dx, void* dy_packed, mnb_stream_t stream) {
+  MNB_REQUIRE(dec, "NULL decode triple");
+  return bn_sign_bwd_pack<int8_t>(g, pass_bits, codes, dec, batch, channels, hw, mean, invstd, gamma, dgamma, dbeta,
+                                  out_shuffle_groups, ch_scale, terms, dx, dy_packed, stream);
+}
+
 template <typename XT>
 static int bn_sign_pool_bwd_pack(const float* g, const uint32_t* pass_bits, const uint8_t* argmax, const XT* x, const float* dec,
                                  int32_t batch, int32_t channels, int32_t H, int32_t W, const float* mean, const float* invstd,
@@ -1746,6 +1775,16 @@
                                         dbeta, out_shuffle_groups, ch_scale, terms, dy_packed, stream);
 }
 
+extern "C" int mnb_bn_sign_pool_bwd_pack_codes8(const float* g, const uint32_t* pass_bits, const uint8_t* argmax,
+                                                const int8_t* codes, const float* dec, int32_t batch, int32_t channels, int32_t H,
+                                                int32_t W, const float* mean, const float* invstd, const float* gamma,
+                                                const float* dgamma, const float* dbeta, int32_t out_shuffle_groups,
+                                                const float* ch_scale, int32_t terms, void* dy_packed, mnb_stream_t stream) {
+  MNB_REQUIRE(dec, "NULL decode triple");
+  return bn_sign_pool_bwd_pack<int8_t>(g, pass_bits, argmax, codes, dec, batch, channels, H, W, mean, invstd, gamma, dgamma,
+                                       dbeta, out_shuffle_groups, ch_scale, terms, dy_packed, stream);
+}
+
 extern "C" int mnb_quant_add_pack_fwd(const float* a, const float* b, int32_t batch, int32_t channels, int32_t h, int32_t w,
                                       const mnb_act_qparams* qp, int32_t relu, float* out, const mnb_pk_post* post,
                                       mnb_stream_t stream) {
@@ -1850,15 +1889,21 @@
 static int pk_conv_impl(const mnb_conv_shape* s, int32_t mode, const void* a_pk, int32_t terms_a, const void* w_img,
                         int32_t terms_w, const float* n_scale, const float* a_scale, float a_scale_const,
                         const float* bias, const uint8_t* bits8, float gain, float* out, const mnb_pk_post* post,
-                        int32_t* err_flag, mnb_stream_t stream, int cpu = 8, int16_t* codes = nullptr, float* dec = nullptr) {
+                        int32_t* err_flag, mnb_stream_t stream, int cpu = 8, int16_t* codes = nullptr, float* dec = nullptr,
+                        int8_t* codes8 = nullptr) {
   using namespace pk;
-  MNB_REQUIRE(s && a_pk && w_img && (out || post || codes) && err_flag, "NULL pk_conv pointer");
+  MNB_REQUIRE(s && a_pk && w_img && (out || post || codes || codes8) && err_flag, "NULL pk_conv pointer");
   Plan pl;
   if (int e = make_plan(s, mode, terms_a, terms_w, pl, cpu)) return e;
   if (codes) {
     MNB_REQUIRE(mode == 0 && cpu == 8 && !out && !post && !bits8 && dec, "pk conv: int16 codes are a plain forward output");
     if (pl.segmented || terms_a != 1 || terms_w != 1)
       return unsupported("int16 codes need one activation piece, one weight piece and a non-segmented plan");
+  }
+  if (codes8) {
+    MNB_REQUIRE(mode == 0 && cpu == 8 && !out && !post && !bits8 && !codes && dec, "pk conv: int8 codes are a plain forward output");
+    if (pl.segmented || terms_a != 1 || terms_w != 1)
+      return unsupported("int8 codes need one activation piece, one weight piece and a non-segmented plan");
   }
   if (post) {
     const int nbn = (post->bn_mean != nullptr) + (post->bn_invstd != nullptr) + (post->bn_gamma != nullptr) + (post->bn_beta != nullptr);
@@ -1933,7 +1978,7 @@
   p.ng = pl.ng; p.Nt = pl.Nt; p.NOUT = pl.NOUT; p.C8O = ceil_div(pl.NOUT, cpu); p.smem_bytes = pl.smem_bytes; p.off_stg = pl.off_stg;
   p.mode = mode;
   p.n_scale = n_scale; p.a_scale = a_scale; p.a_scale_const = a_scale_const; p.bias = bias; p.bits8 = bits8; p.gain = gain;
-  p.out = out; p.err = err_flag; p.codes = codes; p.dec = dec;
+  p.out = out; p.err = err_flag; p.codes = codes; p.codes8 = codes8; p.dec = dec;
   if (post) {
     p.post_out = reinterpret_cast<uint4*>(post->out_pk); p.post_q = *post->q; p.post_relu = post->relu; p.post_split = post->phase_split;
     p.post_mean = post->bn_mean; p.post_invstd = post->bn_invstd; p.post_gamma = post->bn_gamma; p.post_beta = post->bn_beta;
@@ -1995,6 +2040,23 @@
                     s->ker_h, s->ker_w, level_bound);
   return pk_conv_impl(s, 0, a_pk, terms_a, w_img, terms_w, n_scale, a_scale, a_scale_const, bias, nullptr, 1.f, nullptr, nullptr,
                       err_flag, stream, 8, codes, dec);
+}
+
+extern "C" int mnb_pk_conv_codes8(const mnb_conv_shape* s, const void* a_pk, int32_t terms_a, const void* w_img, int32_t terms_w,
+                                  const float* n_scale, const float* a_scale, float a_scale_const, const float* bias,
+                                  int32_t level_bound, int8_t* codes, float* dec, int32_t* err_flag, mnb_stream_t stream) {
+  MNB_REQUIRE(s && codes && dec, "NULL pk_conv_codes8 pointer");
+  MNB_REQUIRE(level_bound >= 1 && s->groups >= 1, "pk_conv_codes8: level bound %d", level_bound);
+  if (s->pad_h != 0 || s->pad_w != 0 || level_bound != 1)
+    return mnb_fail(MNB_E_UNSUPPORTED, "pk_conv_codes8: int8 codes need padding 0 and weight levels in {-1, 0, 1} (padding %d x %d, "
+                    "level bound %d)", s->pad_h, s->pad_w, level_bound);
+  if ((int64_t)(s->in_c / s->groups) * s->ker_h * s->ker_w > 255)
+    return mnb_fail(MNB_E_UNSUPPORTED, "pk_conv_codes8: sums of %d x %d x %d terms may exceed the int8 codes' range",
+                    s->in_c / s->groups, s->ker_h, s->ker_w);
+  if (terms_a != 1 || terms_w != 1)
+    return mnb_fail(MNB_E_UNSUPPORTED, "pk_conv_codes8: int8 codes need one activation piece and one weight piece");
+  return pk_conv_impl(s, 0, a_pk, terms_a, w_img, terms_w, n_scale, a_scale, a_scale_const, bias, nullptr, 1.f, nullptr, nullptr,
+                      err_flag, stream, 8, nullptr, dec, codes);
 }
 
 
diff --git a/micronet_b200/csrc/mnb_quant.cu b/micronet_b200/csrc/mnb_quant.cu
--- a/micronet_b200/csrc/mnb_quant.cu
+++ b/micronet_b200/csrc/mnb_quant.cu
@@ -748,6 +748,14 @@
                                  mean_invstd, scratch, stream);
 }
 
+extern "C" int mnb_bn_batch_stats_codes8(const int8_t* codes, const float* dec, int32_t batch, int32_t channels, int32_t hw,
+                                         double eps, double momentum, float* running_mean, float* running_var,
+                                         int64_t* num_batches_tracked, float* mean_invstd, void* scratch, mnb_stream_t stream) {
+  MNB_REQUIRE(dec, "NULL decode triple");
+  return bn_batch_stats<int8_t>(codes, dec, batch, channels, hw, eps, momentum, running_mean, running_var, num_batches_tracked,
+                                mean_invstd, scratch, stream);
+}
+
 extern "C" int mnb_channel_stats_bwd(const float* x, const float* mean, const float* dmean, const float* dvar,
                                      int32_t batch, int32_t channels, int32_t hw, float* dx,
                                      mnb_stream_t stream) {
diff --git a/micronet_b200/functional.py b/micronet_b200/functional.py
--- a/micronet_b200/functional.py
+++ b/micronet_b200/functional.py
@@ -257,8 +257,10 @@
     if codes is not None:
         b, c = t.shape[0], t.shape[1]
         out = torch.empty(t.shape, dtype=torch.float32, device=t.device)
-        L.check(L.load().mnb_codes_decode(codes[0].data_ptr(), codes[1].data_ptr(), b, c, t.numel() // (b * c), out.data_ptr(),
-                                          L.stream()), "codes_decode")
+        lib = L.load()
+        fn = lib.mnb_codes_decode8 if codes[0].dtype == torch.int8 else lib.mnb_codes_decode
+        L.check(fn(codes[0].data_ptr(), codes[1].data_ptr(), b, c, t.numel() // (b * c), out.data_ptr(), L.stream()),
+                "codes_decode")
         return out
     if not getattr(t, "_mnb_plane_only", False):
         return t
@@ -313,10 +315,16 @@
             a_const = 1.0 / float(2 ** spec.bits - 1)
     rc = L.E_UNSUPPORTED
     if codes_out and w_int is not None and ta == 1 and tw == 1:
-        codes = torch.empty(y.shape, dtype=torch.int16, device=y.device)
-        dec = torch.empty(2 * y.shape[1], dtype=torch.float32, device=y.device)
-        rc = _timed("fwd_pk", sh, lambda: PK.conv_codes(sh, x_pk, w_img, codes, dec, n_scale=w_scale, a_scale=a_scale,
-                                                        a_scale_const=a_const, bias=bias))
+        forms = [(torch.int16, 2, PK.conv_codes)]
+        if PK.codes8_fit(sh.in_c, sh.groups, (sh.ker_h, sh.ker_w), (sh.pad_h, sh.pad_w)):
+            forms.insert(0, (torch.int8, 3, PK.conv_codes8))
+        for dtype, rows, conv_fn in forms:
+            codes = torch.empty(y.shape, dtype=dtype, device=y.device)
+            dec = torch.empty(rows * y.shape[1], dtype=torch.float32, device=y.device)
+            rc = _timed("fwd_pk", sh, lambda: conv_fn(sh, x_pk, w_img, codes, dec, n_scale=w_scale, a_scale=a_scale,
+                                                      a_scale_const=a_const, bias=bias))
+            if rc != L.E_UNSUPPORTED:
+                break
         if rc == 0:
             y._mnb_codes = (codes, dec)
     if rc == L.E_UNSUPPORTED:
diff --git a/micronet_b200/fused.py b/micronet_b200/fused.py
--- a/micronet_b200/fused.py
+++ b/micronet_b200/fused.py
@@ -14,7 +14,8 @@
 def _xargs(lib, name, x, codes):
     if codes is None:
         return getattr(lib, name), (x.data_ptr(),)
-    return getattr(lib, name + "_codes"), (codes[0].data_ptr(), codes[1].data_ptr())
+    suffix = "_codes8" if codes[0].dtype == torch.int8 else "_codes"
+    return getattr(lib, name + suffix), (codes[0].data_ptr(), codes[1].data_ptr())
 
 
 class BNSignFn(Function):
diff --git a/micronet_b200/pk.py b/micronet_b200/pk.py
--- a/micronet_b200/pk.py
+++ b/micronet_b200/pk.py
@@ -78,6 +78,18 @@
 def codes_fit(in_channels, groups, kernel_size, level_bound=1):
     r, s = (kernel_size, kernel_size) if isinstance(kernel_size, int) else kernel_size
     return (in_channels // groups) * r * s * level_bound <= 32767
+
+
+def conv_codes8(sh, a_pk, w_img, codes, dec, n_scale=None, a_scale=None, a_scale_const=1.0, bias=None, level_bound=1):
+    return L.load().mnb_pk_conv_codes8(C.byref(sh), a_pk.data_ptr(), 1, w_img.data_ptr(), 1, L.ptr(n_scale), L.ptr(a_scale),
+                                       float(a_scale_const), L.ptr(bias), int(level_bound), codes.data_ptr(), dec.data_ptr(),
+                                       L.tc_err_flag(codes.device).data_ptr(), L.stream())
+
+
+def codes8_fit(in_channels, groups, kernel_size, padding=0, level_bound=1):
+    r, s = (kernel_size, kernel_size) if isinstance(kernel_size, int) else kernel_size
+    ph, pw = (padding, padding) if isinstance(padding, int) else padding
+    return ph == 0 and pw == 0 and level_bound == 1 and (in_channels // groups) * r * s <= 255
 
 
 def consumer_plane(b, c, h, w, device):
```

Measured after the change: 38530 (median of 6 runs). 1.01x the previous value.
